# alphafox02/iridium-sniffer

Hardware: AMD Instinct MI355X
Metric: IQ Msamples/s end-to-end (detect->demod), 10 MHz cf32 (higher is better)
Workload: dtype f32

## Files before the change

### iridium-sniffer_amd/csrc/api.cpp

```cpp
#include <stdarg.h>
#include "pipeline.hpp"

namespace irdmh {

extern "C" int irdm_set_option(irdm_pipeline_t *p, const char *key, int value)
{
    if (!p || !key) return -1;
    if (!strcmp(key, "keep_frame_samples")) { p->keep_frame_samples = value; return 0; }
    if (!strcmp(key, "packed_records")) { p->packed_records = value; return 0; }
    if (!strcmp(key, "parsed_records")) { p->parsed_records = value; return 0; }
    if (!strcmp(key, "frame_records")) { p->frame_records = value; return 0; }
    if (!strcmp(key, "chunk_marks")) { p->chunk_marks = value ? 1 : 0; if (!value) p->q_marks.clear(); return 0; }
    if (!strcmp(key, "decode_frames")) { p->decode_frames = value; return 0; }
    if (!strcmp(key, "decode_ida")) { p->decode_ida = value; return 0; }
    if (!strcmp(key, "detect_only")) { p->detect_only = value; return 0; }
    if (!strcmp(key, "fir_order") || !strcmp(key, "simd_order")) { p->fir_order = value ? 1 : 0; return 0; }
    if (!strcmp(key, "host_cfo")) { p->dev_cfo = p->dev_cfo_ok && value == 0; return 0; }
    if (!strcmp(key, "scan_mode")) { p->scan_mode = value; return 0; }
    if (!strcmp(key, "kernel_clock")) { p->kernel_clock = value != 0; return 0; }
    if (!strcmp(key, "rot_prebuild")) {
        if (value) return p->rot_pre_runs ? 0 : rot_prebuild(p);
        return p->rot_pre_runs ? rot_arena_reset(p, (long long)std::min(p->P.n, 1024) * p->rot_runs) : 0;
    }
    if (!strcmp(key, "band_timeline")) { p->band_tune.timeline = value != 0; return 0; }
    if (!strcmp(key, "fir_generic")) { p->fir_generic = value != 0; return 0; }
    if (!strcmp(key, "post_generic")) { p->post_generic = value != 0; return 0; }
    if (!strcmp(key, "k1_lists")) { p->k1_lists = value; return 0; }
    if (!strcmp(key, "band_first")) { p->band_first = value < 0 ? 0 : value > kBandRounds ? kBandRounds : value; return 0; }
    if (!strcmp(key, "band_spec")) { p->band_spec_opt = value != 0; return 0; }
    if (!strcmp(key, "band_selfcheck")) { p->band_tune.selfcheck = value; return 0; }
    if (!strcmp(key, "rot_pool_rows")) {
        if (value < 1 || value > p->P.n) return -1;
        return rot_arena_reset(p, (long long)value * p->rot_runs);
    }
    if (!strcmp(key, "scratch_outputs")) {
        if (value < 16) return -1;
        for (int i = 0; i < p->n_bc; i++)
            if (p->bc[i].n != 0) return -1;
        IRDM_HIP_CHECK(hipDeviceSynchronize());
        for (int i = 0; i < p->n_bc; i++) {
            BatchCtx &b = p->bc[i];
            float2 *d2 = dev_alloc<float2>((size_t)value), *l2 = dev_alloc<float2>(lpf_alloc((size_t)value));
            if (!d2 || !l2) return -1;
            (void)hipFree(b.d_dec);
            (void)hipFree(b.d_lpf);
            b.d_dec = d2;
            b.d_lpf = l2;
            b.dec_cap = (size_t)value;
            if (!b.owns_buffers) { p->d_dec = d2; p->d_lpf = l2; }
        }
        return 0;
    }
    return -1;
}

extern "C" int64_t irdm_get_stat(const irdm_pipeline_t *p, const char *key)
{
    if (!p || !key) return -1;
    if (!strcmp(key, "scan_fast_chunks")) return (int64_t)p->stat_fast_chunks;
    if (!strcmp(key, "scan_fallbacks")) return (int64_t)p->stat_fallbacks;
    if (!strncmp(key, "host_us_", 8) && key[8] >= '0' && key[8] <= '9') return (int64_t)p->host_us[key[8] - '0'];
    if (!strcmp(key, "band_chunks")) return (int64_t)p->stat_band_chunks;
    if (!strcmp(key, "band_extra")) return (int64_t)p->stat_band_extra;
    if (!strcmp(key, "scan_chained")) return (int64_t)p->stat_chained;
    if (!strcmp(key, "scan_chain_undone")) return (int64_t)p->stat_chain_undone;
    if (!strcmp(key, "k1_lists")) return (int64_t)p->stat_k1_lists;
    if (!strcmp(key, "band_rounds")) return (int64_t)p->stat_band_rounds;
    if (!strcmp(key, "band_retries")) return (int64_t)p->stat_band_retries;
    if (!strcmp(key, "band_aborts")) return (int64_t)p->stat_band_aborts;
    if (!strncmp(key, "tl_dur_", 7)) { const int i = atoi(key + 7); return i >= 0 && i < 32 ? (int64_t)p->stat_tl_dur[i] : -1; }
    if (!strncmp(key, "tl_gap_", 7)) { const int i = atoi(key + 7); return i >= 0 && i < 32 ? (int64_t)p->stat_tl_gap[i] : -1; }
    if (!strncmp(key, "tl_n_", 5)) { const int i = atoi(key + 5); return i >= 0 && i < 32 ? (int64_t)p->stat_tl_n[i] : -1; }
    if (!strncmp(key, "plan_tp_", 8)) {
        const int i = atoi(key + 8);
        return i >= 0 && i < 16 ? (int64_t)p->stat_plan_tp[i] : -1;
    }
    if (!strcmp(key, "rot_rows")) return (int64_t)p->rot_rows_used;
    if (!strcmp(key, "rot_prebuilt_runs")) return (int64_t)p->rot_pre_runs;
    if (!strcmp(key, "rot_rows_cap")) return (int64_t)(p->rot_blocks_cap / p->rot_runs);
    if (!strcmp(key, "rot_blocks")) return (int64_t)p->rot_blocks_used;
    if (!strcmp(key, "rot_blocks_cap")) return (int64_t)p->rot_blocks_cap;
    if (!strcmp(key, "rot_grows")) return (int64_t)p->stat_rot_grows;
    if (!strcmp(key, "rot_builds")) return (int64_t)p->stat_rot_builds;
    if (!strcmp(key, "rot_runs")) return (int64_t)p->stat_rot_rows;
    if (!strcmp(key, "rot_ckpts")) return (int64_t)p->stat_rot_ckpts;
    if (!strcmp(key, "band_steps")) return (int64_t)p->stat_band_steps;
    if (!strcmp(key, "scratch_outputs")) return (int64_t)p->bc[0].dec_cap;
    if (!strcmp(key, "scratch_grows")) return (int64_t)p->stat_scratch_grows;
    if (!strcmp(key, "tiles_grows")) return (int64_t)p->stat_tiles_grows;
    if (!strcmp(key, "ring_waits")) return (int64_t)p->stat_ring_waits;
    if (!strcmp(key, "spec_passes")) return (int64_t)p->stat_spec_passes;
    if (!strcmp(key, "spec_scans")) return (int64_t)p->stat_spec_scans;
    if (!strcmp(key, "sum_restarts")) return (int64_t)p->stat_sum_restarts;
    if (!strcmp(key, "scratch_peak")) return (int64_t)p->stat_scratch_peak;
    if (!strcmp(key, "band_last_flags")) return (int64_t)p->last_band_flags;
    if (!strcmp(key, "scan_dense_frames")) return (int64_t)p->stat_dense_frames;
    return -1;
}

extern "C" int irdm_kernel_clock(irdm_pipeline_t *p, int which, double *sum_ms, uint64_t *launches, double *last_ms, int reset)
{
    if (!p || !p->d_kclk || which < 0 || which > 1) return -1;
    pipeline_enter(p);
    if (hipDeviceSynchronize() != hipSuccess) return -1;
    std::vector<unsigned long long> h((size_t)(6 + kMaxBc - 3) * kKClkWords);
    if (hipMemcpy(h.data(), p->d_kclk, sizeof(unsigned long long) * h.size(), hipMemcpyDeviceToHost) != hipSuccess) return -1;
    unsigned long long ticks = 0, n = 0, last = 0;
    std::vector<int> recs;
    if (which == 1) recs = { 3, 4, 5 };
    else
        for (int c = 0; c < kMaxBc; c++) recs.push_back(c < 3 ? c : 3 + c);
    for (int r : recs) {
        ticks += h[(size_t)r * kKClkWords + 128];
        n += h[(size_t)r * kKClkWords + 129];
        if (h[(size_t)r * kKClkWords + 130] > last) last = h[(size_t)r * kKClkWords + 130];
    }
    if (sum_ms) *sum_ms = (double)ticks * 1e-5;
    if (launches) *launches = n;
    if (last_ms) *last_ms = (double)last * 1e-5;
    if (reset) {
        for (int r : recs) {
            unsigned long long z[3] = { 0, 0, 0 };
            if (hipMemcpy(p->d_kclk + (size_t)r * kKClkWords + 128, z, sizeof(z), hipMemcpyHostToDevice) != hipSuccess) return -1;
        }
    }
    return 0;
}

extern "C" int irdm_last_timings(const irdm_pipeline_t *p, float *ms_out, int n)
{
    if (!p || !ms_out) return -1;
    for (int i = 0; i < n && i < 6; i++) ms_out[i] = p->last_ms[i];
    return n < 6 ? n : 6;
}

extern "C" int irdm_format_raw(const irdm_demod_t *f, const char *file_info, uint64_t *t0_io, char *buf,
                               size_t cap)
{
    if (!f || !t0_io || !buf) return -1;
    char auto_info[64];
    if (*t0_io == 0) *t0_io = (f->timestamp / 1000000000ULL) * 1000000000ULL;
    const uint64_t t0 = *t0_io;
    if (!file_info || !file_info[0]) {
        snprintf(auto_info, sizeof(auto_info), "i-%llu-t1", (unsigned long long)(t0 / 1000000000ULL));
        file_info = auto_info;
    }
    const double ts_ms = (double)(f->timestamp - t0) / 1000000.0;
    const int freq_hz = (int)(f->center_frequency + 0.5);
    const int payload = f->n_payload_symbols < 0 ? 0 : f->n_payload_symbols;
    int pos = snprintf(buf, cap, "RAW: %s %012.4f %010d N:%05.2f%+06.2f I:%011llu %3d%% %.5f %3d ", file_info,
                       ts_ms, freq_hz, f->magnitude, f->noise, (unsigned long long)f->id, f->confidence,
                       f->level, payload);
    if (pos < 0 || (size_t)pos + (size_t)f->n_bits + 2 > cap) return -1;
    for (int i = 0; i < f->n_bits; i++) buf[pos++] = (char)('0' + f->bits[i]);
    buf[pos++] = '\n';
    buf[pos] = 0;
    return pos;
}

extern "C" int irdm_format_raw_packed(const irdm_demod_packed_t *f, const char *file_info, uint64_t *t0_io, char *buf,
                                      size_t cap)
{
    if (!f || !t0_io || !buf) return -1;
    char auto_info[64];
    if (*t0_io == 0) *t0_io = (f->timestamp / 1000000000ULL) * 1000000000ULL;
    const uint64_t t0 = *t0_io;
    if (!file_info || !file_info[0]) {
        snprintf(auto_info, sizeof(auto_info), "i-%llu-t1", (unsigned long long)(t0 / 1000000000ULL));
        file_info = auto_info;
    }
    const double ts_ms = (double)(f->timestamp - t0) / 1000000.0;
    const int freq_hz = (int)(f->center_frequency + 0.5);
    const int payload = f->n_payload_symbols < 0 ? 0 : f->n_payload_symbols;
    int pos = snprintf(buf, cap, "RAW: %s %012.4f %010d N:%05.2f%+06.2f I:%011llu %3d%% %.5f %3d ", file_info,
                       ts_ms, freq_hz, f->magnitude, f->noise, (unsigned long long)f->id, f->confidence,
                       f->level, payload);
    const int nb = f->n_bits < 0 ? 0 : (f->n_bits > IRDM_MAX_BITS ? IRDM_MAX_BITS : f->n_bits);
    if (pos < 0 || (size_t)pos + (size_t)nb + 2 > cap) return -1;
    for (int i = 0; i < nb; i++) buf[pos++] = (char)('0' + ((f->bits[i >> 3] >> (7 - (i & 7))) & 1));
    buf[pos++] = '\n';
    buf[pos] = 0;
    return pos;
}

extern "C" long long irdm_format_raw_packed_batch(const irdm_demod_packed_t *f, int n, const char *file_info, uint64_t *t0_io,
                                                  char *buf, size_t cap)
{
    if (!f || n < 0 || !t0_io || !buf) return -1;
    size_t pos = 0;
    for (int i = 0; i < n; i++) {
        const int len = irdm_format_raw_packed(&f[i], file_info, t0_io, buf + pos, cap - pos);
        if (len < 0) return -1;
        pos += (size_t)len;
    }
    return (long long)pos;
}

extern "C" void irdm_ida_unpack(const irdm_ida_packed_t *ida, const irdm_demod_packed_t *f, irdm_ida_t *out)
{
    if (!ida || !f || !out) return;
    IdaOut d;
    memset(&d, 0, sizeof(d));
    d.ok = ida->ok;
    d.ft = ida->ft; d.lcw_ft = ida->lcw_ft; d.lcw_code = ida->lcw_code; d.ec_lcw = ida->ec_lcw;
    d.lcw3_val = ida->lcw3_val;
    d.da_ctr = ida->da_ctr; d.da_len = ida->da_len; d.cont = ida->cont; d.crc_ok = ida->crc_ok;
    d.stored_crc = ida->stored_crc; d.computed_crc = ida->computed_crc;
    d.fixederrs = ida->fixederrs; d.payload_len = ida->payload_len; d.bch_len = ida->bch_len;
    memcpy(d.payload, ida->payload, sizeof(d.payload));
    for (int i = 0; i < 256; i++) d.bch_stream[i] = (uint8_t)((ida->bch_stream[i >> 3] >> (7 - (i & 7))) & 1);
    irdm_demod_t fr;
    memset(&fr, 0, offsetof(irdm_demod_t, bits));
    fr.id = f->id;
    fr.direction = f->direction;
    fr.timestamp = f->timestamp;
    fr.center_frequency = f->center_frequency;
    fr.magnitude = f->magnitude;
    fr.noise = f->noise;
    fr.level = f->level;
    fr.confidence = f->confidence;
    fr.n_payload_symbols = f->n_payload_symbols;
    *out = finish_ida(d, fr);
}

extern "C" void irdm_frame_unpack(const irdm_frame_packed_t *fr, const irdm_demod_packed_t *f, irdm_decoded_t *out)
{
    if (!fr || !f || !out) return;
    DecodedOut d;
    memset(&d, 0, sizeof(d));
    d.type = fr->type;
    d.sat_id = fr->sat_id;
    d.beam_id = fr->beam_id;
    for (int k = 0; k < 3; k++) d.pos_xyz[k] = fr->pos_xyz[k];
    d.n_pages = fr->n_pages;
    for (int k = 0; k < 12; k++) { d.page_tmsi[k] = fr->page_tmsi[k]; d.page_msc[k] = fr->page_msc[k]; }
    d.timeslot = fr->timeslot;
    d.sv_blocking = fr->sv_blocking;
    d.bc_type = fr->bc_type;
    d.iri_time = fr->iri_time;
    d.bch_len = fr->bch_len;
    *out = finish_decoded(d, f->id, f->timestamp, f->center_frequency);
}

namespace {

struct LineBuf {
    char *buf;
    size_t cap, pos = 0;
    bool bad = false;
    void printf(const char *fmt, ...) __attribute__((format(printf, 2, 3)))
    {
        if (bad) return;
        va_list ap;
        va_start(ap, fmt);
        const int n = vsnprintf(buf + pos, cap - pos, fmt, ap);
        va_end(ap);
        if (n < 0 || (size_t)n >= cap - pos) bad = true;
        else pos += (size_t)n;
    }
    void put(char c)
    {
        if (bad || pos + 1 >= cap) { bad = true; return; }
        buf[pos++] = c;
        buf[pos] = 0;
    }
};

}

extern "C" int irdm_format_ida(const irdm_ida_t *b, uint64_t *t0_io, char *buf, size_t cap)
{
    if (!b || !t0_io || !buf || cap == 0) return -1;
    if (*t0_io == 0) *t0_io = (b->timestamp / 1000000000ULL) * 1000000000ULL;
    const uint64_t t0 = *t0_io;
    LineBuf o{ buf, cap };
    buf[0] = 0;
    char parsed_info[64];
    snprintf(parsed_info, sizeof(parsed_info), "p-%llu", (unsigned long long)(t0 / 1000000000ULL));
    const double ts_ms = (double)(b->timestamp - t0) / 1000000.0;
    const int freq_hz = (int)(b->frequency + 0.5);
    const double leveldb = (b->level > 0) ? 20.0 * log10(b->level) : -99.99;
    const double noise = b->noise, snr = b->magnitude;
    const char *dir = b->direction == 2 ? "UL" : "DL";
    const int syms = b->n_symbols < 0 ? 0 : b->n_symbols;
    o.printf("IDA: %s %014.4f %010d %3d%% %06.2f|%07.2f|%05.2f %3d %s ", parsed_info, ts_ms, freq_hz, b->confidence,
             leveldb, noise, snr, syms, dir);
    o.printf("%.*s", (int)sizeof(b->lcw_header), b->lcw_header);
    const uint8_t *bs = b->bch_stream;
    const int bch_len = b->bch_len;
    if (bch_len >= 20) {
        o.printf("%c%c%c", '0' + bs[0], '0' + bs[1], '0' + bs[2]);
        o.printf(" cont=%c", '0' + bs[3]);
        o.printf(" %c", '0' + bs[4]);
        o.printf(" ctr=%c%c%c", '0' + bs[5], '0' + bs[6], '0' + bs[7]);
        o.printf(" %c%c%c", '0' + bs[8], '0' + bs[9], '0' + bs[10]);
        o.printf(" len=%02d", b->da_len);
        o.printf(" 0:%c%c%c%c", '0' + bs[16], '0' + bs[17], '0' + bs[18], '0' + bs[19]);
        o.printf(" [");
        bool all_zero = true;
        if (b->da_len > 0)
            for (int i = b->da_len + 1; i < 20; i++)
                if (b->payload[i] != 0) { all_zero = false; break; }
        const int nbytes = b->da_len > 0 && all_zero ? b->da_len : 20;
        for (int i = 0; i < nbytes; i++) {
            if (i > 0) o.put(nbytes == 20 && i == b->da_len && b->da_len > 0 && b->da_len < 20 ? '!' : '.');
            o.printf("%02x", b->payload[i]);
        }
        o.printf("]");
        for (int i = nbytes * 3; i < 60; i++) o.put(' ');
        if (b->da_len > 0) {
            o.printf(" %04x/%04x", b->stored_crc, b->computed_crc);
            o.printf(b->crc_ok ? " CRC:OK" : " CRC:no");
        } else {
            o.printf("  ---   ");
        }
        const int shown = bch_len < 256 ? bch_len : 256;
        if (bch_len > 9 * 20 + 16) {
            o.put(' ');
            for (int i = 9 * 20 + 16; i < shown; i++) o.put((char)('0' + bs[i]));
        } else {
            o.printf(" 0000");
        }
        if (b->da_len > 0 && bch_len >= 9 * 20) {
            o.printf(" SBD: ");
            for (int i = 0; i < 20; i++) {
                int byte = 0;
                for (int k = 0; k < 8; k++) byte = (byte << 1) | bs[1 * 20 + i * 8 + k];
                o.put(byte >= 32 && byte < 127 ? (char)byte : '.');
            }
        }
    }
    o.put('\n');
    return o.bad ? -1 : (int)o.pos;
}

extern "C" long long irdm_format_parsed_packed_batch(const irdm_demod_packed_t *f, const irdm_ida_packed_t *idas, int n,
                                                     const char *file_info, uint64_t *t0_io, char *buf, size_t cap)
{
    if (!f || !idas || n < 0 || !t0_io || !buf) return -1;
    size_t pos = 0;
    for (int i = 0; i < n; i++) {
        int len;
        if (idas[i].ok) {
            irdm_ida_t b;
            irdm_ida_unpack(&idas[i], &f[i], &b);
            len = irdm_format_ida(&b, t0_io, buf + pos, cap - pos);
        } else {
            len = irdm_format_raw_packed(&f[i], file_info, t0_io, buf + pos, cap - pos);
        }
        if (len < 0) return -1;
        pos += (size_t)len;
    }
    return (long long)pos;
}

extern "C" int irdm_save_burst(const irdm_frame_info_t *info, const float *samples, const char *dir)
{
    if (!info || !samples || !dir || info->drop_reason != 0 || info->num_samples <= 0) return -1;
    struct stat st;
    memset(&st, 0, sizeof(st));
    if (stat(dir, &st) == -1) {
        if (mkdir(dir, 0755) == -1 && errno != EEXIST) {
            fprintf(stderr, "Warning: failed to create burst save directory: %s\n", strerror(errno));
            return -1;
        }
    }
    const char *dir_str = info->demod_direction == 1 ? "DL" : info->demod_direction == 2 ? "UL" : "UN";
    char base[512];
    snprintf(base, sizeof(base), "%s/%020lu_%011.0f_%lu_%s", dir, (unsigned long)info->timestamp,
             info->center_frequency, (unsigned long)info->id, dir_str);
    char path[520];
    snprintf(path, sizeof(path), "%s.cf32", base);
    FILE *f = fopen(path, "wb");
    if (!f) {
        fprintf(stderr, "Warning: failed to save burst IQ: %s\n", strerror(errno));
        return -1;
    }
    fwrite(samples, 2 * sizeof(float), (size_t)info->num_samples, f);
    fclose(f);
    snprintf(path, sizeof(path), "%s.meta", base);
    f = fopen(path, "w");
    if (!f) return -1;
    fprintf(f, "burst_id: %lu\n", (unsigned long)info->id);
    fprintf(f, "timestamp_ns: %lu\n", (unsigned long)info->timestamp);
    fprintf(f, "center_freq_hz: %.0f\n", info->center_frequency);
    fprintf(f, "sample_rate_hz: %.0f\n", info->sample_rate);
    fprintf(f, "samples_per_symbol: %.2f\n", info->samples_per_symbol);
    fprintf(f, "direction: %s\n", dir_str);
    fprintf(f, "magnitude_db: %.2f\n", info->magnitude);
    fprintf(f, "noise_dbfs_hz: %.2f\n", info->noise);
    fprintf(f, "num_samples: %zu\n", (size_t)info->num_samples);
    fprintf(f, "uw_start_offset: %.2f\n", info->uw_start);
    fclose(f);
    return 0;
}

extern "C" long long irdm_format_raw_batch(const irdm_demod_t *f, int n, const char *file_info, uint64_t *t0_io,
                                           char *buf, size_t cap)
{
    if (!f || n < 0 || !t0_io || !buf) return -1;
    size_t pos = 0;
    for (int i = 0; i < n; i++) {
        const int len = irdm_format_raw(&f[i], file_info, t0_io, buf + pos, cap - pos);
        if (len < 0) return -1;
        pos += (size_t)len;
    }
    return (long long)pos;
}

extern "C" const char *irdm_version(void) { return "irdm_hip 0.1 (gfx950)"; }

}
```

### iridium-sniffer_amd/csrc/band_core.hpp

```cpp
#pragma once
#include <stdint.h>
#include "types.hpp"

#if defined(__HIPCC__)
#define IRDM_HD __host__ __device__ __forceinline__
#else
#define IRDM_HD inline
#endif

namespace irdm {

constexpr int kBandSlots = 24;
constexpr int kBandRecCap = 1024;
constexpr int kBandMaxTotal = 8192;

enum : uint32_t {
    BAND_F_SLOTS = 1,
    BAND_F_RECS = 2,
    BAND_F_LIST = 4,
    BAND_F_STALE = 8,
    BAND_F_SQUELCH = 16,
    BAND_F_AGREE = 32,
    BAND_F_ITER = 64,
    BAND_F_TOTAL = 128,
    BAND_F_GONECAP = 256,
    BAND_F_SNAP = 512,
    BAND_F_CHAIN = 2048,
    BAND_F_CHECK = 4096,
    BAND_F_COOP = 1024,
};

struct BandParams {
    int32_t n, nw64;
    int32_t log_n;
    int32_t n_frames, occ_words;
    int32_t hw;
    int32_t pre_len, post_len, max_len, max_bursts;
    int32_t band_w, n_bands;
    int32_t gap;
    int32_t list_cap;
    float thr;
    uint64_t idx0;
    int32_t serial = 0;
    int32_t selfcheck = 0;
    int32_t tl_sel = -1;
    int32_t chained = 0;
    int32_t sum_restart = 1;
    int32_t spec_in = 0;
};

struct BandRec {
    int64_t start, last_active, stop;
    int32_t cf;
    int32_t cb;
    float rel, base;
    int32_t flags;
    int32_t seq;
};

IRDM_HD uint32_t band_float_bits(float v)
{
    uint32_t u;
    __builtin_memcpy(&u, &v, 4);
    return u;
}

IRDM_HD bool band_rec_same(const BandRec &a, const BandRec &b)
{
    return a.start == b.start && a.last_active == b.last_active && a.stop == b.stop && a.cf == b.cf &&
           a.cb == b.cb && a.seq == b.seq && (a.flags & 2) == (b.flags & 2) &&
           band_float_bits(a.rel) == band_float_bits(b.rel) && band_float_bits(a.base) == band_float_bits(b.base);
}

struct BandIO {
    const uint64_t *cross;
    const uint64_t *occ;
    const float *relq;
    const float *snap;
    const int32_t *slot_post;
    const ActiveBurst *act_in;
    int32_t n_act_in;
    BandRec *recs;
    uint32_t *rec_count;
    uint64_t *busy, *forced;
    uint32_t *conc;
    uint32_t *flags;
};

struct BandSlots {
    int64_t *start, *la;
    int32_t *cb, *cf, *seq;
    float *rel, *base;
    int stride;
};

#if defined(__HIP_DEVICE_COMPILE__)
IRDM_HD void band_or64(uint64_t *p, uint64_t v) { atomicOr(reinterpret_cast<unsigned long long *>(p), (unsigned long long)v); }
IRDM_HD void band_or32(uint32_t *p, uint32_t v) { atomicOr(p, v); }
IRDM_HD uint32_t band_add32(uint32_t *p, uint32_t v) { return atomicAdd(p, v); }
#else
IRDM_HD void band_or64(uint64_t *p, uint64_t v) { *p |= v; }
IRDM_HD void band_or32(uint32_t *p, uint32_t v) { *p |= v; }
IRDM_HD uint32_t band_add32(uint32_t *p, uint32_t v) { uint32_t o = *p; *p = o + v; return o; }
#endif

template <int NW>
IRDM_HD void bm_set_range(uint64_t (&m)[NW], int a, int b)
{
#pragma unroll
    for (int k = 0; k < NW; k++) {
        int lo = a - 64 * k, hi = b - 64 * k;
        if (lo < 0) lo = 0;
        if (hi > 63) hi = 63;
        if (lo <= hi) m[k] |= (~0ull >> (63 - hi)) & (~0ull << lo);
    }
}

template <int NW>
IRDM_HD int bm_test(const uint64_t (&m)[NW], int r)
{
    uint64_t w = 0;
#pragma unroll
    for (int k = 0; k < NW; k++)
        if (k == (r >> 6)) w = m[k];
    return (int)((w >> (r & 63)) & 1);
}

template <int NW>
IRDM_HD bool bm_any(const uint64_t (&m)[NW])
{
    uint64_t w = 0;
#pragma unroll
    for (int k = 0; k < NW; k++) w |= m[k];
    return w != 0;
}

IRDM_HD int band_next_occ(const uint64_t *occ, int a, int b, int n_frames)
{
    if (a < 0) a = 0;
    if (b >= n_frames) b = n_frames - 1;
    while (a <= b) {
        const int w = a >> 6;
        uint64_t v = occ[w] & (~0ull << (a & 63));
        if (v) {
            const int f = 64 * w + __builtin_ctzll(v);
            return f <= b ? f : 0x7fffffff;
        }
        a = 64 * (w + 1);
    }
    return 0x7fffffff;
}

IRDM_HD uint64_t band_segment_starts(const uint64_t *occ, int blk, int gap, bool carried)
{
    const uint64_t cur = occ[blk], prev = blk > 0 ? occ[blk - 1] : 0;
    uint64_t smear = 0;
    for (int d = 1; d <= gap; d++) smear |= (cur << d) | (prev >> (64 - d));
    if (blk == 0 && carried) smear |= gap >= 64 ? ~0ull : ((1ull << gap) - 1);
    return cur & ~smear;
}

template <int NW>
struct BandWalker {
    const BandParams &P;
    const BandIO &io;
    BandSlots S;
    int band, e0, word0;
    int own_lo, own_hi, rep_lo, rep_hi;
    uint64_t M[NW], elig[NW];
    uint32_t valid;
    int last_occ;
    int acc_blk;
    uint32_t acc_max;
    int n_events = 0;

    IRDM_HD BandWalker(const BandParams &p, const BandIO &i, BandSlots s, int b) : P(p), io(i), S(s), band(b)
    {
        const int H = P.band_w / 2;
        e0 = band * P.band_w - H;
        word0 = e0 >> 6;
        own_lo = H;
        own_hi = H + P.band_w;
        rep_lo = own_lo - P.hw;
        rep_hi = own_hi + P.hw;
#pragma unroll
        for (int k = 0; k < NW; k++) M[k] = elig[k] = 0;
        uint64_t dc[NW];
#pragma unroll
        for (int k = 0; k < NW; k++) dc[k] = 0;
        bm_set_range<NW>(elig, P.hw - e0, P.n - P.hw - 1 - e0);
        bm_set_range<NW>(dc, P.n / 2 - 3 - e0, P.n / 2 + 3 - e0);
#pragma unroll
        for (int k = 0; k < NW; k++) elig[k] &= ~dc[k];
        valid = 0;
        last_occ = -1;
        acc_blk = -1;
        acc_max = 0;
    }

    IRDM_HD void rebuild_mask()
    {
#pragma unroll
        for (int k = 0; k < NW; k++) M[k] = 0;
        for (uint32_t v = valid; v; v &= v - 1) {
            const int i = __builtin_ctz(v);
            const int r = S.cb[i * S.stride] - e0;
            bm_set_range<NW>(M, r - P.hw, r + P.hw);
        }
    }

    IRDM_HD void emit(int i, int64_t stop, int lng)
    {
        const int r = S.cb[i * S.stride] - e0;
        if (r < rep_lo || r >= rep_hi) return;
        const uint32_t at = band_add32(&io.rec_count[band], 1);
        if (at >= (uint32_t)kBandRecCap) {
            band_or32(io.flags, BAND_F_RECS);
            return;
        }
        BandRec g;
        g.start = S.start[i * S.stride];
        g.last_active = S.la[i * S.stride];
        g.stop = stop;
        g.cf = S.cf[i * S.stride];
        g.cb = S.cb[i * S.stride];
        g.rel = S.rel[i * S.stride];
        g.base = S.base[i * S.stride];
        g.flags = ((r >= own_lo && r < own_hi) ? 1 : 0) | (lng ? 2 : 0);
        g.seq = S.seq[i * S.stride];
        io.recs[(size_t)band * kBandRecCap + at] = g;
    }

    IRDM_HD uint32_t owned_count() const
    {
        uint32_t c = 0;
        for (uint32_t v = valid; v; v &= v - 1) {
            const int r = S.cb[__builtin_ctz(v) * S.stride] - e0;
            c += (r >= own_lo && r < own_hi) ? 1 : 0;
        }
        return c;
    }

    IRDM_HD void account(int a, int b, uint32_t c)
    {
        if (c == 0 || a > b) return;
        for (int blk = a >> 6; blk <= (b >> 6); blk++) {
            const int lo = blk == (a >> 6) ? (a & 63) : 0, hi = blk == (b >> 6) ? (b & 63) : 63;
            band_or64(&io.busy[blk], (~0ull >> (63 - hi)) & (~0ull << lo));
            if (blk != acc_blk) {
                flush_conc();
                acc_blk = blk;
                acc_max = c;
            } else if (c > acc_max) {
                acc_max = c;
            }
        }
    }

    IRDM_HD void flush_conc()
    {
        if (acc_blk >= 0 && acc_max > 0) band_add32(&io.conc[acc_blk], acc_max);
        acc_blk = -1;
        acc_max = 0;
    }

    IRDM_HD int load_carried()
    {
        int n = 0;
        for (int i = 0; i < io.n_act_in; i++) {
            const int r = io.act_in[i].center_bin - e0;
            if (r < 0 || r >= 64 * NW) continue;
            if (n >= kBandSlots) {
                band_or32(io.flags, BAND_F_SLOTS);
                break;
            }
            S.start[n * S.stride] = (int64_t)io.act_in[i].start;
            S.la[n * S.stride] = (int64_t)io.act_in[i].last_active;
            S.cb[n * S.stride] = io.act_in[i].center_bin;
            S.cf[n * S.stride] = -1;
            S.seq[n * S.stride] = i;
            S.rel[n * S.stride] = io.act_in[i].peak_rel;
            S.base[n * S.stride] = io.act_in[i].base_sum;
            valid |= 1u << n;
            n++;
        }
        rebuild_mask();
        return n;
    }

    IRDM_HD int min_expiry() const
    {
        int64_t best = 0x7fffffff;
        for (uint32_t v = valid; v; v &= v - 1) {
            const int i = __builtin_ctz(v);
            const int64_t num = S.la[i * S.stride] + (int64_t)P.post_len - (int64_t)P.idx0;
            const int64_t ef = num <= 0 ? 0 : (num + P.n - 1) >> P.log_n;
            if (ef < best) best = ef;
        }
        return (int)best;
    }

    IRDM_HD int next_event(int f)
    {
        const uint64_t *occ = io.occ + (size_t)band * P.occ_words;
        if (valid == 0) return band_next_occ(occ, f + 1, last_occ + P.gap, P.n_frames);
        const int ef = min_expiry();
        const int nf = band_next_occ(occ, f + 1, ef, P.n_frames);
        return nf < ef ? nf : ef;
    }

    IRDM_HD void process(int f)
    {
        const int64_t index = (int64_t)P.idx0 + (int64_t)f * P.n;
        const uint64_t *occ = io.occ + (size_t)band * P.occ_words;
        const bool occupied = (occ[f >> 6] >> (f & 63)) & 1;
        uint64_t cw[NW];
#pragma unroll
        for (int k = 0; k < NW; k++) {
            const int w = word0 + k;
            cw[k] = (occupied && w >= 0 && w < P.nw64) ? io.cross[(size_t)f * P.nw64 + w] : 0;
        }
        if (occupied) last_occ = f;

        if (valid && bm_any<NW>(cw)) {
            uint64_t hit[NW];
#pragma unroll
            for (int k = 0; k < NW; k++) {
                hit[k] = cw[k] | (cw[k] << 1) | (cw[k] >> 1);
                if (k > 0) hit[k] |= cw[k - 1] >> 63;
                if (k < NW - 1) hit[k] |= cw[k + 1] << 63;
            }
            for (uint32_t v = valid; v; v &= v - 1) {
                const int i = __builtin_ctz(v);
                if (bm_test<NW>(hit, S.cb[i * S.stride] - e0)) S.la[i * S.stride] = index;
            }
        }
        uint64_t pk[NW];
#pragma unroll
        for (int k = 0; k < NW; k++) pk[k] = cw[k] & ~M[k] & elig[k];

        bool deleted = false;
        for (uint32_t v = valid; v; v &= v - 1) {
            const int i = __builtin_ctz(v);
            const int64_t la = S.la[i * S.stride];
            const bool lng = P.max_len > 0 && (la - S.start[i * S.stride] > (int64_t)P.max_len);
            if (la + (int64_t)P.post_len <= index || lng) {
                const int r = S.cb[i * S.stride] - e0;
                if (lng && r >= own_lo && r < own_hi) band_or64(&io.forced[f >> 6], 1ull << (f & 63));
                emit(i, index, lng ? 1 : 0);
                valid &= ~(1u << i);
                deleted = true;
            }
        }
        if (deleted) rebuild_mask();

        while (bm_any<NW>(pk)) {
            float best = -1.0f;
            int best_r = -1;
#pragma unroll
            for (int k = 0; k < NW; k++) {
                uint64_t w = pk[k];
                const float *row = io.relq + (size_t)f * P.n + (e0 + 64 * k);
                while (w) {
                    const int j0 = __builtin_ctzll(w);
                    w &= w - 1;
                    const int j1 = w ? __builtin_ctzll(w) : j0;
                    w &= w ? w - 1 : 0;
                    const int j2 = w ? __builtin_ctzll(w) : j1;
                    w &= w ? w - 1 : 0;
                    const int j3 = w ? __builtin_ctzll(w) : j2;
                    w &= w ? w - 1 : 0;
                    const float v0 = row[j0], v1 = row[j1], v2 = row[j2], v3 = row[j3];
                    if (v0 > best) { best = v0; best_r = 64 * k + j0; }
                    if (v1 > best) { best = v1; best_r = 64 * k + j1; }
                    if (v2 > best) { best = v2; best_r = 64 * k + j2; }
                    if (v3 > best) { best = v3; best_r = 64 * k + j3; }
                }
            }
            if (best_r < 0) break;
            int slot = __builtin_ctz(~valid);
            if (slot >= kBandSlots) {
                band_or32(io.flags, BAND_F_SLOTS);
                break;
            }
            const int cbin = e0 + best_r;
            S.start[slot * S.stride] = index - (int64_t)P.pre_len;
            S.la[slot * S.stride] = index - (int64_t)P.pre_len;
            S.cb[slot * S.stride] = cbin;
            S.cf[slot * S.stride] = f;
            S.seq[slot * S.stride] = 0;
            S.rel[slot * S.stride] = best;
            S.base[slot * S.stride] = io.snap[(size_t)io.slot_post[f] * P.n + cbin];
            valid |= 1u << slot;
            bm_set_range<NW>(M, best_r - P.hw, best_r + P.hw);
#pragma unroll
            for (int k = 0; k < NW; k++) pk[k] &= ~M[k];
        }
    }

    IRDM_HD void run(int f_start, bool carried)
    {
        int f;
        if (carried) {
            last_occ = -1;
            const uint32_t c0 = owned_count();
            f = next_event(-1);
            account(0, (f < P.n_frames ? f : P.n_frames) - 1, c0);
        } else {
            f = f_start;
        }
        while (f < P.n_frames) {
            process(f);
            n_events++;
            const uint32_t c = owned_count();
            const int nf = next_event(f);
            account(f, (nf < P.n_frames ? nf : P.n_frames) - 1, c);
            if (valid == 0 && nf == 0x7fffffff) break;
            f = nf;
        }
        flush_conc();
        for (uint32_t v = valid; v; v &= v - 1) emit(__builtin_ctz(v), -1, 0);
    }
};

}
```

### iridium-sniffer_amd/csrc/create.cpp

```cpp
#include "pipeline.hpp"

namespace irdmh {

void pipeline_free(irdm_pipeline *p)
{
    if (!p) return;
    void *ptrs[] = { p->d_window, p->d_hist, p->d_sum, p->d_mag, p->d_tw, p->d_tw4096, p->d_tw2048,
                     p->d_dl_fft, p->d_ul_fft, p->d_rot_incr, p->d_state, p->d_gone,
                     p->d_cand_a, p->d_cand_b, p->d_ring, p->d_stage, p->d_in_taps, p->d_noise_taps,
                     p->d_start_taps, p->d_rrc_taps, p->d_cfo_window, p->d_work, p->d_tiles, p->d_dec,
                     p->d_lpf, p->d_rrc_ws, p->d_frames, p->d_demod_ws, p->d_probe, p->d_demod, p->d_decoded, p->d_syn_ra,
                     p->d_syn_hdr, p->d_nbits, p->d_ida, p->d_syn_da, p->d_syn_l1, p->d_syn_l2, p->d_syn_l3, p->d_dirs,
                     p->d_fir_off, p->d_mag2, p->d_mag3, p->k1_pre[1], p->k1_pre[2], p->k1_counts[1], p->k1_counts[2], p->k1_entries[1], p->k1_entries[2],
                     p->k1_pre[0] != p->d_pre ? p->k1_pre[0] : nullptr, p->k1_counts[0] != p->d_counts ? p->k1_counts[0] : nullptr,
                     p->k1_entries[0] != p->d_entries ? p->k1_entries[0] : nullptr, p->d_counts, p->d_entries, p->d_goff, p->d_compact, p->d_pre, p->d_sum_bak, p->d_hist_bak, p->d_state_bak,
                     p->d_status, p->d_mc_ops, p->d_mc_done, p->d_band, p->d_smin, p->d_kclk, p->d_state_spec };
    for (void *q : ptrs)
        if (q) (void)hipFree(q);
    for (int s = 0; s < 2; s++) {
        if (p->h_pin_set[s]) (void)hipHostFree(p->h_pin_set[s]);
        if (p->hp_gone_set[s]) (void)hipHostFree(p->hp_gone_set[s]);
        if (p->ev_end_set[s]) (void)hipEventDestroy(p->ev_end_set[s]);
        for (auto &e : p->ev_sk_set[s])
            if (e) (void)hipEventDestroy(e);
    }
    if (p->cfo_thread.joinable()) {
        {
            std::lock_guard<std::mutex> lk(p->cfo_mu);
            p->cfo_quit = true;
        }
        p->cfo_cv.notify_one();
        p->cfo_thread.join();
    }
    for (int i = 0; i < kMaxBc; i++) {
        BatchCtx &b = p->bc[i];
        if (b.ev_cfo) (void)hipEventDestroy(b.ev_cfo);
        if (b.ev_rot) (void)hipEventDestroy(b.ev_rot);
        for (auto &e : b.ev)
            if (e) (void)hipEventDestroy(e);
        if (b.hp_flag) (void)hipHostFree(b.hp_flag);
        if (b.hp_rot_new) (void)hipHostFree(b.hp_rot_new);
        if (b.d_rot_new) (void)hipFree(b.d_rot_new);
        if (b.hp_work) (void)hipHostFree(b.hp_work);
        if (b.hp_tiles) (void)hipHostFree(b.hp_tiles);
        if (b.hp_demod) (void)hipHostFree(b.hp_demod);
        if (b.hp_packed) (void)hipHostFree(b.hp_packed);
        if (b.hp_ida) (void)hipHostFree(b.hp_ida);
        if (b.hp_frame) (void)hipHostFree(b.hp_frame);
        if (b.owns_buffers) {
            void *own[] = { b.d_work, b.d_tiles, b.d_dec, b.d_lpf, b.d_rrc_ws, b.d_frames, b.d_demod_ws, b.d_demod,
                            b.d_decoded, b.d_ida };
            for (void *q : own)
                if (q) (void)hipFree(q);
            if (b.stream) (void)hipStreamDestroy(b.stream);
        }
    }
    if (p->ev_ring) (void)hipEventDestroy(p->ev_ring);
    for (auto &f : p->fs) {
        if (f.ev_start) (void)hipEventDestroy(f.ev_start);
        if (f.ev_k1) (void)hipEventDestroy(f.ev_k1);
        if (f.ev_copy) (void)hipEventDestroy(f.ev_copy);
    }
    if (p->hp_gate) (void)hipHostFree(p->hp_gate);
    if (p->d_rot_table) (void)hipFree(p->d_rot_table);
    for (float2 *q : p->rot_retired) (void)hipFree(q);
    for (float2 *q : p->scratch_retired) (void)hipFree(q);
    for (void *q : p->tiles_retired) (void)hipFree(q);
    for (void *q : p->tiles_host_retired) (void)hipHostFree(q);
    if (p->d_rot_slot) (void)hipFree(p->d_rot_slot);
    if (p->stream_rot_pre) { (void)hipStreamSynchronize(p->stream_rot_pre); (void)hipStreamDestroy(p->stream_rot_pre); }
    if (p->ev_rot_pre) (void)hipEventDestroy(p->ev_rot_pre);
    if (p->d_rot_pre_news) (void)hipFree(p->d_rot_pre_news);
    if (p->stream_spec) (void)hipStreamDestroy(p->stream_spec);
    if (p->ev_sums1) (void)hipEventDestroy(p->ev_sums1);
    if (p->ev_spec_done) (void)hipEventDestroy(p->ev_spec_done);
    if (p->d_band_spec) (void)hipFree(p->d_band_spec);
    for (auto &e : p->ev)
        if (e) (void)hipEventDestroy(e);
    if (p->sstream && p->sstream != p->stream) (void)hipStreamDestroy(p->sstream);
    if (p->ev_scan_in) (void)hipEventDestroy(p->ev_scan_in);
    if (p->ev_scan_out) (void)hipEventDestroy(p->ev_scan_out);
    if (p->fstream && p->fstream != p->stream) (void)hipStreamDestroy(p->fstream);
    if (p->stream2) (void)hipStreamDestroy(p->stream2);
    if (p->stream) (void)hipStreamDestroy(p->stream);
    delete p;
}

extern "C" void irdm_destroy(irdm_pipeline_t *p) { pipeline_free(p); }


bool chain_stream_create(irdm_pipeline *, hipStream_t *out, int prio)
{
    return hipStreamCreateWithPriority(out, hipStreamNonBlocking, prio) == hipSuccess;
}

extern "C" irdm_pipeline_t *irdm_create(const irdm_config_t *cfg)
{
    if (!cfg || cfg->sample_rate <= 0) return nullptr;
    int ndev = 0;
    if (hipGetDeviceCount(&ndev) != hipSuccess || ndev == 0) {
        fprintf(stderr, "irdm_hip: no HIP device -- there is no CPU fallback in this library\n");
        return nullptr;
    }
    if (hipSetDevice(cfg->device) != hipSuccess) return nullptr;
    const bool dbg = getenv("IRDM_CREATE_DEBUG") != nullptr;
    size_t mem_free0 = 0, mem_total = 0;
    if (dbg) (void)hipMemGetInfo(&mem_free0, &mem_total);
    auto t_now = [] {
        struct timespec ts;
        clock_gettime(CLOCK_MONOTONIC, &ts);
        return ts.tv_sec * 1e3 + ts.tv_nsec * 1e-6;
    };
    const double t_create0 = t_now();
    auto mark = [&](const char *what) {
        if (!dbg) return;
        size_t fr = 0, tot = 0;
        (void)hipMemGetInfo(&fr, &tot);
        fprintf(stderr, "irdm_create: %-28s %8.2f ms  %8.1f MB on the device\n", what, t_now() - t_create0,
                ((double)mem_free0 - (double)fr) / 1e6);
    };

    irdm_pipeline *p = new (std::nothrow) irdm_pipeline();
    if (!p) return nullptr;
    p->cfg = *cfg;
    const int fs = cfg->sample_rate;

    DetParams &P = p->P;
    P.log_n = (int)round(log2(fs / 1000.0));
    P.n = 1 << P.log_n;
    P.pre_len = 2 * P.n;
    P.post_len = (int)(fs * 16e-3);
    const int burst_width_hz = 40000;
    P.width = burst_width_hz / (fs / P.n);
    P.max_bursts = (int)((fs / (float)burst_width_hz) * 0.8f);
    P.max_len = (int)(fs * 0.09);
    const float tdb = cfg->threshold_db > 0 ? cfg->threshold_db : 16.0f;
    P.threshold = powf(10.0f, tdb / 10.0f) / kHistory / 1.72f;
    if (P.n < kScanThreads || P.n > 16384 || P.max_bursts + P.n / (P.width > 0 ? P.width : 1) + 8 > kMaxActive) {
        fprintf(stderr, "irdm_hip: unsupported sample rate %d (fft_size %d)\n", fs, P.n);
        delete p;
        return nullptr;
    }
    p->feed_block = cfg->feed_block > 0 ? cfg->feed_block : 32768;
    if (p->feed_block % P.n != 0) {
        fprintf(stderr, "irdm_hip: feed_block %d must be a multiple of fft_size %d\n", p->feed_block, P.n);
        delete p;
        return nullptr;
    }
    p->dev_fmt = cfg->format;
    p->bps = p->dev_fmt == 2 ? 8 : (p->dev_fmt == 1 ? 4 : 2);
    p->max_chunk = cfg->max_chunk_samples ? cfg->max_chunk_samples : ((size_t)64 << 20);
    p->max_chunk = (p->max_chunk + p->feed_block - 1) / p->feed_block * p->feed_block;
    p->burst_cap = cfg->max_bursts_per_chunk > 0 ? cfg->max_bursts_per_chunk : 4096;
    p->gone_cap = p->burst_cap;
    p->start_time_ns = cfg->start_time_ns;
    if (p->start_time_ns == 0) {
        struct timespec ts;
        clock_gettime(CLOCK_REALTIME, &ts);
        p->start_time_ns = ts.tv_sec * 1000000000ULL + ts.tv_nsec;
    }

    p->ref_ring = (uint64_t)P.max_len + P.pre_len + P.post_len + (uint64_t)P.n * 4;
    if (p->ref_ring < (uint64_t)2 * fs) p->ref_ring = (uint64_t)2 * fs;
    p->l_cap = (size_t)P.max_len + P.post_len + P.pre_len + 2 * (size_t)P.n;
    p->depth = cfg->pipeline_depth > 0 ? std::min(cfg->pipeline_depth, kMaxBc - 1) : 0;
    p->k1_first = 1;
    p->k1_lists = 1;
    p->band_first = 0;
    p->band_auto = kBandFirst;
    p->ring_len = p->ref_ring + p->l_cap + p->feed_block;
    if (p->depth) p->ring_len += (size_t)(p->depth + 2 + kLookAhead) * p->max_chunk;
    p->ring_len = (p->ring_len + 15) / 16 * 16;
    if (p->depth) p->ring_len = (p->ring_len + p->max_chunk - 1) / p->max_chunk * p->max_chunk;
    p->n_ckpt = (int)(p->l_cap / kRotSeg) + 2;

    p->out_rate = 10 * 25000;
    p->sps = (float)p->out_rate / 25000;
    p->search_depth = p->out_rate;
    p->pre_start = (int)(100 * 1e-6f * p->out_rate);
    p->decim = (int)roundf((float)fs / p->out_rate);
    if (p->decim < 1) p->decim = 1;
    p->dec_stride = (int)(p->l_cap / p->decim) + 8;

    std::vector<float> in_taps = design_lpf(1.0f, 10000000.0f, p->out_rate * 0.4f, p->out_rate * 0.2f);
    std::vector<float> noise_taps = design_lpf(1.0f, (float)p->out_rate, 40000.0f / 2.0f, 40000.0f);
    int box = (int)(p->sps * 2);
    if (box < 3) box = 3;
    std::vector<float> start_taps = design_box(box);
    std::vector<float> rrc = design_rrc(1.0f, (float)p->out_rate, 25000.0f, 0.4f, 51);
    std::vector<float> rc = design_rc((float)p->out_rate, 25000.0f, 0.4f, 51);
    std::vector<float> cfo_window = design_blackman(kCfoN);
    if ((int)in_taps.size() != kFirTaps) {
        delete p;
        return nullptr;
    }
    p->in_ntaps = (int)in_taps.size();
    p->noise_ntaps = (int)noise_taps.size();
    p->start_ntaps = (int)start_taps.size();
    p->rrc_ntaps = (int)rrc.size();
    std::vector<cfloat> dl = design_sync_template(rc, kCorrN, p->sps, false, &p->dl_len);
    std::vector<cfloat> ul = design_sync_template(rc, kCorrN, p->sps, true, &p->ul_len);

    std::vector<float> window = design_blackman(P.n);
    for (int i = 0; i < P.n; i++) window[i] /= 0.42f;
    std::vector<cfloat> tw = design_twiddles(P.n), tw4096 = design_twiddles(kCfoTotal),
                        tw2048 = design_twiddles(kCorrN);
    std::vector<cfloat> rot_incr = design_rotator_incr(P.n);

    mark("host designs");
    int prio_lo = 0, prio_hi = 0;
    (void)hipDeviceGetStreamPriorityRange(&prio_lo, &prio_hi);
    bool ok = true;
    p->stream2 = nullptr;
    if (p->depth) {
        int prio_k1 = prio_hi < prio_lo - 1 ? prio_hi + 1 : prio_hi;
        if (const char *e = getenv("IRDM_K1_PRIO")) prio_k1 = atoi(e);
        ok = hipStreamCreateWithPriority(&p->stream, hipStreamNonBlocking, prio_hi) == hipSuccess &&
             hipStreamCreateWithPriority(&p->fstream, hipStreamNonBlocking, prio_k1) == hipSuccess &&
             chain_stream_create(p, &p->stream2, prio_lo);
        p->bstream = p->stream2;
    } else {
        ok = hipStreamCreateWithFlags(&p->stream, hipStreamNonBlocking) == hipSuccess;
        p->bstream = p->stream;
        p->fstream = p->stream;
    }
    p->sstream = p->stream;
    p->bstream_prio = prio_lo;
    p->ev_scan_in = p->ev_scan_out = nullptr;
    p->has_pending = false;
    p->pend_c1 = 0;
    p->h_pin = nullptr;
    for (int s = 0; s < 2; s++) {
        p->h_pin_set[s] = nullptr;
        p->hp_gone_set[s] = nullptr;
        p->ev_end_set[s] = nullptr;
        for (auto &e : p->ev_sk_set[s]) ok = ok && hipEventCreate(&e) == hipSuccess;
        ok = ok && hipEventCreateWithFlags(&p->ev_end_set[s], hipEventDisableTiming) == hipSuccess;
        ok = ok && hipHostMalloc(reinterpret_cast<void **>(&p->h_pin_set[s]), sizeof(int) * 128, hipHostMallocDefault) == hipSuccess;
        if (ok) memset(p->h_pin_set[s], 0, sizeof(int) * 128);
    }
    p->out_sel = 0;
    p->chain_pending = false;
    p->settle_clean = true;
    p->h_pin = p->h_pin_set[0];
    p->ev_sk[0] = p->ev_sk_set[0][0];
    p->ev_sk[1] = p->ev_sk_set[0][1];
    p->ev_end = p->ev_end_set[0];
    for (auto &e : p->ev) ok = ok && hipEventCreate(&e) == hipSuccess;
#define UP(dst, vec) ok = ok && ((dst = reinterpret_cast<decltype(dst)>(dev_upload((vec).data(), (vec).size()))) != nullptr)
#define AL(dst, T, count) ok = ok && ((dst = dev_alloc<T>(count)) != nullptr)
    UP(p->d_window, window);
    UP(p->d_tw, tw);
    UP(p->d_tw4096, tw4096);
    UP(p->d_tw2048, tw2048);
    UP(p->d_dl_fft, dl);
    UP(p->d_ul_fft, ul);
    UP(p->d_rot_incr, rot_incr);
    UP(p->d_in_taps, in_taps);
    UP(p->d_noise_taps, noise_taps);
    UP(p->d_start_taps, start_taps);
    UP(p->d_rrc_taps, rrc);
    UP(p->d_cfo_window, cfo_window);
    {
        const int row = fir_tile_row(p->decim);
        std::vector<int> off(kFirTaps);
        for (int k = 0; k < kFirTaps; k++) off[k] = ((k % p->decim) * row + k / p->decim) * (int)sizeof(float2);
        UP(p->d_fir_off, off);
    }
    mark("streams, uploads");
    AL(p->d_hist, float, (size_t)kHistory * P.n);
    AL(p->d_sum, float, (size_t)P.n);
    AL(p->d_mag, float, p->max_chunk);
    if (p->depth) AL(p->d_mag2, float, p->max_chunk);
    if (p->depth) AL(p->d_mag3, float, p->max_chunk);
    AL(p->d_state, DetState, 1);
    AL(p->d_gone, GoneBurst, (size_t)p->gone_cap);
    AL(p->d_cand_a, PeakCand, (size_t)P.n);
    AL(p->d_cand_b, PeakCand, (size_t)P.n);
    mark("detector buffers");
    p->d_rot_table = nullptr;
    AL(p->d_work, BurstWork, (size_t)p->burst_cap);
    p->tiles_cap = (size_t)p->burst_cap * 64;
    AL(p->d_tiles, FirTile, (p->tiles_cap + 1) * kFirTileUnits);
    p->cfo_quit = false;
    p->scratch_init = std::max<size_t>((size_t)p->burst_cap * p->dec_stride / 16, (size_t)4 * p->dec_stride);
    AL(p->d_dec, float2, p->scratch_init);
    AL(p->d_lpf, float2, lpf_alloc(p->scratch_init));
    AL(p->d_rrc_ws, float2, (size_t)p->burst_cap * kFrameNeed);
    AL(p->d_frames, float2, (size_t)p->burst_cap * kMaxFrameSamples);
    AL(p->d_demod_ws, float2, (size_t)p->burst_cap * 2 * kMaxSymbols);
    AL(p->d_demod, DemodOut, (size_t)p->burst_cap);
    AL(p->d_decoded, DecodedOut, (size_t)p->burst_cap);
    AL(p->d_nbits, int, (size_t)p->burst_cap);
    {
        auto rem = [](unsigned poly, unsigned v) {
            if (!v) return 0u;
            const int pb = 32 - __builtin_clz(poly);
            for (int i = 31; i >= pb - 1; i--)
                if (v & (1u << i)) v ^= poly << (i - pb + 1);
            return v;
        };
        auto build = [&](unsigned poly, int nbits, int max_err, int size) {
            std::vector<int2> t((size_t)size, make_int2(-1, 0));
            for (int b1 = 0; b1 < nbits; b1++) {
                const unsigned v = 1u << b1, r = rem(poly, v);
                if (r < (unsigned)size) t[r] = make_int2(1, (int)v);
            }
            if (max_err >= 2)
                for (int b1 = 0; b1 < nbits; b1++)
                    for (int b2 = b1 + 1; b2 < nbits; b2++) {
                        const unsigned v = (1u << b1) | (1u << b2), r = rem(poly, v);
                        if (r < (unsigned)size && t[r].x < 0) t[r] = make_int2(2, (int)v);
                    }
            return t;
        };
        std::vector<int2> ra = build(1207u, 31, 2, 1024), hdr = build(29u, 7, 1, 16);
        UP(p->d_syn_ra, ra);
        UP(p->d_syn_hdr, hdr);
        std::vector<int2> da = build(3545u, 31, 2, 2048), l1 = build(29u, 7, 1, 16), l2 = build(465u, 14, 1, 256),
                          l3 = build(41u, 26, 2, 32);
        UP(p->d_syn_da, da);
        UP(p->d_syn_l1, l1);
        UP(p->d_syn_l2, l2);
        UP(p->d_syn_l3, l3);
        AL(p->d_ida, IdaOut, (size_t)p->burst_cap);
        AL(p->d_dirs, int, (size_t)p->burst_cap);
    }
    AL(p->d_probe, float2, p->l_cap);
    {
        const size_t max_frames = p->max_chunk / P.n;
        AL(p->d_counts, unsigned, max_frames);
        AL(p->d_entries, ListEntry, max_frames * (size_t)std::max(kListCap, band_list_cap(P.n)));
        AL(p->d_goff, unsigned, max_frames + 1);
        AL(p->d_compact, ListEntry, max_frames * kListCap);
        AL(p->d_pre, float, (size_t)P.n);
        p->k1_pre[0] = p->d_pre;
        p->k1_counts[0] = p->d_counts;
        p->k1_entries[0] = p->d_entries;
        for (int i = 0; i < kFeedSlots && p->depth; i++) {
            AL(p->k1_pre[i], float, (size_t)P.n);
            AL(p->k1_counts[i], unsigned, max_frames);
            AL(p->k1_entries[i], ListEntry, max_frames * (size_t)std::max(kListCap, band_list_cap(P.n)));
        }
        AL(p->d_sum_bak, float, (size_t)P.n);
        AL(p->d_hist_bak, float, (size_t)kHistory * P.n);
        AL(p->d_state_bak, DetState, 1);
        AL(p->d_status, int, 64);
        p->mc_ops_cap = (int)(4 * max_frames + 64);
        AL(p->d_mc_ops, unsigned long long, (size_t)p->mc_ops_cap);
        AL(p->d_mc_done, unsigned, 32 * 16);
    }
    mark("per-burst scratch, lists");
    ok = ok && hipHostMalloc(reinterpret_cast<void **>(&p->hp_gate), 64, hipHostMallocMapped | hipHostMallocCoherent) == hipSuccess &&
         hipHostGetDevicePointer(reinterpret_cast<void **>(&p->hp_gate_dev), p->hp_gate, 0) == hipSuccess;
    if (ok) memset(p->hp_gate, 0, 64);
    AL(p->d_kclk, unsigned long long, (size_t)(6 + kMaxBc - 3) * kKClkWords);
    if (ok) {
        std::vector<unsigned long long> init((size_t)(6 + kMaxBc - 3) * kKClkWords, 0ull);
        for (int r = 0; r < 6 + kMaxBc - 3; r++)
            for (int i = 0; i < 64; i++) init[(size_t)r * kKClkWords + i] = ~0ull;
        ok = hipMemcpy(p->d_kclk, init.data(), sizeof(unsigned long long) * init.size(), hipMemcpyHostToDevice) == hipSuccess;
    }
    p->band_ok = band_scan_supported(P, nullptr, 1, 0) != 0;
    if (p->band_ok) {
        AL(p->d_smin, float, (size_t)P.n);
        if (ok) ok = hipMalloc(&p->d_band, band_work_bytes(P.n, p->max_chunk)) == hipSuccess;
        if (ok) band_work_carve(&p->band, p->d_band, P.n, p->max_chunk);
        if (ok) ok = hipMemset(p->band.bar, 0, 256) == hipSuccess;
        if (ok && p->depth) {
            const size_t sb = band_work_bytes(P.n, p->max_chunk, true);
            ok = hipMalloc(&p->d_band_spec, sb) == hipSuccess;
            if (ok) band_work_carve(&p->band_spec, p->d_band_spec, P.n, p->max_chunk, true);
            if (ok) ok = hipMemset(p->band_spec.ctl, 0, sizeof(BandCtl)) == hipSuccess && hipMemset(p->band_spec.bar, 0, 256) == hipSuccess &&
                         hipMemset(p->band_spec.rec_count, 0, 4 * 64) == hipSuccess && hipMemset(p->band_spec.flags, 0, 256) == hipSuccess;
            AL(p->d_state_spec, DetState, 1);
            if (ok) ok = hipMemset(p->d_state_spec, 0, sizeof(DetState)) == hipSuccess;
            ok = ok && hipStreamCreateWithPriority(&p->stream_spec, hipStreamNonBlocking, prio_hi) == hipSuccess &&
                 hipEventCreateWithFlags(&p->ev_sums1, hipEventDisableTiming) == hipSuccess &&
                 hipEventCreateWithFlags(&p->ev_spec_done, hipEventDisableTiming) == hipSuccess;
        }
    }
    mark("band scan workspace");
    if (ok) ok = hipMalloc(&p->d_ring, p->ring_len * p->bps) == hipSuccess;
    mark("history ring");
    p->n_bc = p->depth ? std::min(p->depth + 1, kMaxBc) : 1;
    for (int i = 0; i < p->n_bc && ok; i++) {
        BatchCtx &b = p->bc[i];
        b.owner = p;
        b.n = 0;
        b.cfo_seq = 0;
        b.owns_buffers = i > 0;
        b.tiles_cap = p->tiles_cap;
        b.dec_cap = p->scratch_init;
        if (i == 0) {
            b.stream = p->bstream;
            b.d_work = p->d_work; b.d_tiles = p->d_tiles; b.d_dec = p->d_dec; b.d_lpf = p->d_lpf;
            b.d_rrc_ws = p->d_rrc_ws; b.d_frames = p->d_frames; b.d_demod_ws = p->d_demod_ws; b.d_demod = p->d_demod;
            b.d_decoded = p->d_decoded; b.d_ida = p->d_ida;
        } else {
            ok = ok && chain_stream_create(p, &b.stream, p->bstream_prio);
            AL(b.d_work, BurstWork, (size_t)p->burst_cap);
            AL(b.d_tiles, FirTile, (b.tiles_cap + 1) * kFirTileUnits);
            AL(b.d_dec, float2, p->scratch_init);
            AL(b.d_lpf, float2, lpf_alloc(p->scratch_init));
            AL(b.d_rrc_ws, float2, (size_t)p->burst_cap * kFrameNeed);
            AL(b.d_frames, float2, (size_t)p->burst_cap * kMaxFrameSamples);
            AL(b.d_demod_ws, float2, (size_t)p->burst_cap * 2 * kMaxSymbols);
            AL(b.d_demod, DemodOut, (size_t)p->burst_cap);
            AL(b.d_decoded, DecodedOut, (size_t)p->burst_cap);
            AL(b.d_ida, IdaOut, (size_t)p->burst_cap);
        }
        ok = ok && hipHostMalloc(reinterpret_cast<void **>(&b.hp_work), sizeof(BurstWork) * (size_t)p->burst_cap,
                                 hipHostMallocMapped | hipHostMallocCoherent) == hipSuccess &&
             hipHostGetDevicePointer(reinterpret_cast<void **>(&b.hp_work_dev), b.hp_work, 0) == hipSuccess;
        ok = ok && hipHostMalloc(reinterpret_cast<void **>(&b.hp_tiles), sizeof(FirTile) * b.tiles_cap, hipHostMallocDefault) == hipSuccess;
        ok = ok && hipHostMalloc(reinterpret_cast<void **>(&b.hp_demod), sizeof(DemodOut) * (size_t)p->burst_cap, hipHostMallocDefault) == hipSuccess;
        ok = ok && hipHostMalloc(reinterpret_cast<void **>(&b.hp_packed), sizeof(DemodPacked) * (size_t)p->burst_cap, hipHostMallocDefault) == hipSuccess;
        ok = ok && hipHostMalloc(reinterpret_cast<void **>(&b.hp_ida), sizeof(IdaPacked) * (size_t)p->burst_cap, hipHostMallocDefault) == hipSuccess;
        ok = ok && hipHostMalloc(reinterpret_cast<void **>(&b.hp_frame), sizeof(FramePacked) * (size_t)p->burst_cap, hipHostMallocDefault) == hipSuccess;
        ok = ok && hipHostMalloc(reinterpret_cast<void **>(&b.hp_flag), 64, hipHostMallocMapped | hipHostMallocCoherent) == hipSuccess &&
             hipHostGetDevicePointer(reinterpret_cast<void **>(&b.hp_flag_dev), b.hp_flag, 0) == hipSuccess;
        if (ok) memset(b.hp_flag, 0, 64);
        ok = ok && hipHostMalloc(reinterpret_cast<void **>(&b.hp_rot_new), sizeof(int4) * (size_t)p->burst_cap, hipHostMallocMapped) == hipSuccess &&
             hipHostGetDevicePointer(reinterpret_cast<void **>(&b.hp_rot_new_dev), b.hp_rot_new, 0) == hipSuccess;
        AL(b.d_rot_new, int4, (size_t)p->burst_cap);
        ok = ok && hipEventCreateWithFlags(&b.ev_cfo, hipEventDisableTiming) == hipSuccess;
        ok = ok && hipEventCreateWithFlags(&b.ev_rot, hipEventDisableTiming) == hipSuccess;
        for (auto &e : b.ev) ok = ok && hipEventCreate(&e) == hipSuccess;
        b.h_cfreq.assign((size_t)p->burst_cap, 0.0);
    }
    p->hp_gone_cap = p->gone_cap;
    for (int s = 0; s < 2; s++)
        ok = ok && hipHostMalloc(reinterpret_cast<void **>(&p->hp_gone_set[s]), sizeof(GoneBurst) * (size_t)p->hp_gone_cap, hipHostMallocDefault) == hipSuccess;
    p->hp_gone = p->hp_gone_set[0];
    ok = ok && hipEventCreateWithFlags(&p->ev_ring, hipEventDisableTiming) == hipSuccess;
    for (auto &f : p->fs)
        ok = ok && hipEventCreate(&f.ev_start) == hipSuccess && hipEventCreate(&f.ev_k1) == hipSuccess &&
             hipEventCreateWithFlags(&f.ev_copy, hipEventDisableTiming) == hipSuccess;
    p->chunk_no = 0;
#undef UP
#undef AL
    if (!ok) {
        fprintf(stderr, "irdm_hip: device allocation failed\n");
        pipeline_free(p);
        return nullptr;
    }
    mark("batch contexts");
    ok = hipMemset(p->d_hist, 0, sizeof(float) * (size_t)kHistory * P.n) == hipSuccess &&
         hipMemset(p->d_sum, 0, sizeof(float) * P.n) == hipSuccess &&
         hipMemset(p->d_state, 0, sizeof(DetState)) == hipSuccess &&
         hipMemset(p->d_ring, 0, p->ring_len * p->bps) == hipSuccess;
    ok = ok && hipDeviceSynchronize() == hipSuccess;
    mark("memsets, sync");
    p->rot_runs = (p->n_ckpt + kRotRun - 1) / kRotRun;
    p->rot_blocks_cap = std::min(P.n, 1024) * p->rot_runs;
    p->rot_blocks_used = 0;
    p->rot_rows_used = 0;
    p->rot_len_h.assign((size_t)P.n, 0);
    p->rot_want.assign((size_t)P.n, 0);
    ok = ok && (p->d_rot_table = dev_alloc<float2>((size_t)p->rot_blocks_cap * kRotRun)) != nullptr;
    ok = ok && (p->d_rot_slot = dev_alloc<int>((size_t)P.n * p->rot_runs)) != nullptr;
    ok = ok && hipMemset(p->d_rot_slot, 0xff, sizeof(int) * (size_t)P.n * p->rot_runs) == hipSuccess;
    p->rot_build_ctx.assign((size_t)P.n, -1);
    p->rot_build_gen.assign((size_t)P.n, 0);
#ifndef IRDM_HIP_EMULATED
    if (ok && p->depth >= 1 && !getenv("IRDM_NO_ROT_PREBUILD")) (void)rot_prebuild(p);
#endif
    mark("rotator row pool");
    if (!ok) {
        fprintf(stderr, "irdm_hip: device initialisation failed\n");
        pipeline_free(p);
        return nullptr;
    }
    p->h_gone.resize(p->gone_cap);
    p->total_samples = p->begun_samples = 0;
    p->begin_no = p->end_no = 0;
    p->tagged = 0;
    p->stream_closed = false;
    p->last_frames = 0;
    p->last_chunk = nullptr;
    p->keep_frame_samples = 0;
    p->chunk_marks = 0;
    p->scan_mode = 0;
    p->mc_updaters = 7;
    {
        hipDeviceProp_t prop;
        const bool have = hipGetDeviceProperties(&prop, cfg->device) == hipSuccess;
        p->mc_auto = have && prop.multiProcessorCount >= 64;
        if (p->scan_cus == 0) p->scan_cus = have ? prop.multiProcessorCount : 1;
    }
    p->stat_fast_chunks = p->stat_fallbacks = p->stat_dense_frames = 0;
    p->stat_band_chunks = p->stat_band_rounds = p->stat_band_retries = p->stat_band_aborts = 0;
    p->last_band_flags = 0;
    p->fl_mode = 0;
    p->fl_done = 0;
    p->host_primed = 0;
    p->host_hist_idx = 0;
    p->dev_cfo = true;
    {
        auto same = [](float off) {
            const cfloat h = fine_rotator_incr(off);
            const float phase_inc = -2.0f * (float)M_PI * off;
            float re, im;
            if (libm_cexpf_i<true>(phase_inc, &re, &im) != 0) return false;
            const float hr = h.real(), hi = h.imag();
            return memcmp(&re, &hr, 4) == 0 && memcmp(&im, &hi, 4) == 0;
        };
        bool all = true;
        for (int i = 0; i < (1 << 18) && all; i++) all = same(-0.26f + 0.52f * (float)i / (float)(1 << 18));
        const float edges[] = { 0.0f, -0.0f, 1e-45f, -1e-45f, 1e-39f, 3e-5f, -3e-5f, 0.125f, -0.125f, 0.25f, -0.25f, 0.2499999f, 0.1250001f };
        for (float e : edges) all = all && same(e);
        if (!all) {
            fprintf(stderr, "irdm_hip: this host's cexpf differs from the restated glibc routine: the fine-CFO step stays on the host\n");
            p->dev_cfo = false;
        }
    }
    p->dev_cfo_ok = p->dev_cfo;
    mark("libm self-check");
    p->cfo_thread = std::thread(cfo_helper_main, p);
    mark("done");
    return p;
}

extern "C" int irdm_sincosf_probe(int device, const float *x, size_t n, float *re, float *im)
{
    if (!x || !re || !im) return -1;
    if (!n) return 0;
    IRDM_HIP_CHECK(hipSetDevice(device));
    float *d = nullptr;
    IRDM_HIP_CHECK(hipMalloc(&d, 3 * n * sizeof(float)));
    int rc = hipMemcpy(d, x, n * sizeof(float), hipMemcpyHostToDevice) == hipSuccess ? 0 : -1;
    if (!rc) rc = launch_sincosf_probe(d, n, d + n, d + 2 * n, nullptr);
    if (!rc) rc = hipMemcpy(re, d + n, n * sizeof(float), hipMemcpyDeviceToHost) == hipSuccess ? 0 : -1;
    if (!rc) rc = hipMemcpy(im, d + 2 * n, n * sizeof(float), hipMemcpyDeviceToHost) == hipSuccess ? 0 : -1;
    (void)hipFree(d);
    return rc;
}

extern "C" uint64_t irdm_tagged_bursts(const irdm_pipeline_t *p) { return p ? p->tagged : 0; }
extern "C" size_t irdm_max_chunk_samples(const irdm_pipeline_t *p) { return p ? p->max_chunk : 0; }
extern "C" size_t irdm_bytes_per_sample(const irdm_pipeline_t *p) { return p ? p->bps : 0; }
extern "C" size_t irdm_required_overlap(const irdm_pipeline_t *p)
{
    if (!p) return 0;
    return (size_t)(p->ref_ring + (uint64_t)p->P.max_len + (uint64_t)p->P.post_len + (uint64_t)p->P.pre_len + 2 * (uint64_t)p->P.n);
}
extern "C" int irdm_wait_ingest(irdm_pipeline_t *p)
{
    if (!p) return -1;
    pipeline_enter(p);
    IRDM_HIP_CHECK(hipStreamSynchronize(p->fstream));
    return 0;
}
extern "C" uint64_t irdm_sample_count(const irdm_pipeline_t *p) { return p ? p->total_samples : 0; }
extern "C" int irdm_fft_size(const irdm_pipeline_t *p) { return p ? p->P.n : -1; }
extern "C" uint64_t irdm_start_time_ns(const irdm_pipeline_t *p) { return p ? p->start_time_ns : 0; }

extern "C" int irdm_set_stream_origin(irdm_pipeline_t *p, double center_frequency, uint64_t start_time_ns)
{
    if (!p || p->begin_no != p->end_no) return -1;
    p->cfg.center_frequency = center_frequency;
    if (start_time_ns) p->start_time_ns = start_time_ns;
    return 0;
}

}
```

### iridium-sniffer_amd/csrc/kernels.hpp

```cpp
#pragma once
#include <hip/hip_runtime.h>
#include "types.hpp"

namespace irdm {

int launch_fft_mag_lists(int log_n, int fmt, const void *iq, const float *window, const float2 *tw, float *mag,
                         int n_frames, const float *pre, unsigned *counts, ListEntry *entries, int cap,
                         hipStream_t stream, unsigned long long *kclk, int order);
int launch_prefilter_threshold(const float *sum, float thr, float *pre, int n, hipStream_t stream);
int launch_fft_mag(int log_n, int fmt, const void *iq, const float *window, const float2 *tw,
                   float *mag, int n_frames, hipStream_t stream, unsigned long long *kclk, int order);
int launch_detect_scan(const DetParams &P, DetState *st, float *sum, float *hist, const float *mag,
                       int n_frames, GoneBurst *gone, int gone_cap, PeakCand *cand_a,
                       PeakCand *cand_b, hipStream_t stream);

int launch_prefilter(const float *sum, float thr, float *pre, const float *mag, int n,
                     unsigned *counts, ListEntry *entries, unsigned *goff, ListEntry *compact,
                     int n_frames, hipStream_t stream);
int launch_detect_scan_fast(const DetParams &P, DetState *st, float *sum, float *hist, const float *mag,
                            int n_frames, const unsigned *counts, const unsigned *goff,
                            const ListEntry *compact, const float *pre, GoneBurst *gone, int gone_cap,
                            int *status, unsigned long long *mc_ops, int mc_ops_cap, unsigned *mc_done,
                            int mc_updaters, hipStream_t stream);

constexpr int kBandRounds = 5;
constexpr int kBandFirst = 3;
struct BandRec;
struct BandParams;
struct BandCtl {
    int32_t status;
    int32_t rounds;
    uint32_t flags;
    int32_t n_upd, n_snap, agree_fail, mismatch, first_mismatch;
    int32_t n_gone, n_total, committed, h0;
    int32_t k_restart, restart_slot;
    int32_t n_restarts, pad1;
    uint32_t tp[16];
};
struct SumStep {
    uint32_t nw_off;
    uint32_t ol_off;
    uint32_t snap_off;
    uint32_t pad;
};
struct BandWork {
    BandCtl *ctl;
    uint8_t *uq, *uf;
    int32_t *cnt_before, *tmp, *upd_frame, *old_row, *snap_after, *need, *snap_slot, *slot_pre, *slot_post;
    SumStep *steps;
    uint64_t *cross;
    float *relq, *snap;
    int snap_cap;
    uint64_t *occ, *busy, *forced;
    uint32_t *conc;
    BandRec *recs;
    uint32_t *rec_count;
    float *sum_new;
    uint32_t *tot;
    uint64_t *ids;
    uint32_t *flags;
    uint32_t *rank;
    unsigned long long *tl;
    unsigned *bar;
};
struct BandTune {
    int selfcheck = 0;
    int timeline = 0;
    int sum_restart = 1;
};
int band_list_cap(int n);
int band_scan_supported(const DetParams &D, BandParams *out, int n_frames, uint64_t idx0);
size_t band_work_bytes(int n, size_t max_chunk, bool spec = false);
int band_work_carve(BandWork *W, void *base, int n, size_t max_chunk, bool spec = false);
int launch_band_spec(const DetParams &D, BandWork S, DetState *st_spec, const float *sum_src, int n_frames, uint64_t idx0,
                     const unsigned *counts, const ListEntry *entries, int have_prev, hipStream_t stream, const BandTune &tune);
int launch_band_scan(const DetParams &D, BandWork W, DetState *st, float *sum, float *hist, const float *mag,
                     int n_frames, uint64_t idx0, const unsigned *counts, const ListEntry *entries, const float *pre,
                     float *smin, GoneBurst *gone, int gone_cap, int round_begin, int round_end, GoneBurst *hp_gone,
                     uint32_t *hp_hdr, void *hp_ctl, int hp_cap, int chained, int tl_sel, hipStream_t stream,
                     const BandTune &tune, const uint32_t *gate_flag = nullptr, uint32_t gate_seq = 0, uint32_t *gate_err = nullptr,
                     const void *gate_src = nullptr, size_t gate_bytes = 0,
                     const BandWork *spec = nullptr, hipEvent_t sums_done = nullptr);
constexpr int kBandTlSlots = 32;
int launch_prefilter_lists(const float *sum, float thr, float *pre, const float *smin, const float *mag, int n,
                           unsigned *counts, ListEntry *entries, int n_frames, int cap, hipStream_t stream);

struct SampleSource {
    const void *chunk;
    uint64_t chunk_start;
    uint64_t chunk_end;
    const void *ring;
    uint64_t ring_len;
    uint64_t ref_ring;
    int fmt;
};

int launch_rotator_rows(const float2 *incr, float2 *table, int n_runs, const int4 *news, int n_new, int *runs, hipStream_t stream);
int fir_tile_row(int decim);
int fir_reg_supported(int decim);
int fir_fma_tile_out(int decim);
int fir_reg_tile_out(int decim);
int launch_fir_fma(const SampleSource &src, const FirGeom *geom, int n_tiles, int decim, const float *taps,
                   const float2 *rot_table, float2 *dec, hipStream_t stream, unsigned long long *kclk = nullptr);
int launch_fir_reg(const SampleSource &src, const FirGeom *geom, int n_tiles, int decim, const float *taps,
                   const float2 *rot_table, float2 *dec, hipStream_t stream, unsigned long long *kclk = nullptr);
int fir_tile_out(int decim, int aligned, int generic, int order);
int fir_needs_tile_list(int decim, int aligned, int generic);
int launch_fir_decimate(const SampleSource &src, const BurstWork *work, int n_bursts, FirTile *tiles, size_t tiles_cap,
                        int n_tiles, int decim, const float *taps, const int *tap_off, const float2 *rot_incr,
                        const float2 *rot_table, int n_ckpt, float2 *dec,
                        hipStream_t stream, unsigned long long *kclk,
                        const int *rot_slot, int order, int generic);
int launch_kclk_fold(unsigned long long *kclk, hipStream_t stream);
int launch_gone_export(const DetState *st, const GoneBurst *gone, int cap, GoneBurst *hp_gone, uint32_t *hp_hdr,
                       const void *ctl, void *hp_ctl, int ctl_bytes, hipStream_t stream);
int launch_copy_to_host(void *dst, const void *src, size_t bytes, hipStream_t stream);
int launch_copy2_to_host(void *dst_a, const void *src_a, size_t bytes_a, void *dst_b, const void *src_b, size_t bytes_b,
                         hipStream_t stream);
int launch_copy_words(void *dst, const void *src, size_t bytes, hipStream_t stream);
int launch_wait_host_flag(const uint32_t *flag, uint32_t seq, uint32_t *err, hipStream_t stream);
int launch_gather_burst(const SampleSource &src, uint64_t start, uint64_t avail_end, int n,
                        float2 *out, hipStream_t stream);
int launch_downmix_post1(BurstWork *work, int n_bursts, int max_dec_len, float2 *dec,
                         float2 *lpf, float *box, const float *noise_taps, int noise_ntaps,
                         const float *start_taps, int start_ntaps, int search_depth, int pre_start,
                         const float *cfo_window, const float2 *tw4096, BurstWork *hp_work, hipStream_t stream,
                         unsigned long long *kclk,
                         int order, int generic);
struct CfoStep {
    int on_device;
    int n_fft, sample_rate, out_rate;
    double center_frequency;
};
int launch_downmix_post2(BurstWork *work, int n_bursts, const float2 *lpf,
                         const float *rrc_taps, int rrc_ntaps, const float2 *tw2048,
                         const float2 *dl_fft, const float2 *ul_fft, int dl_len, int ul_len,
                         float sps, float2 *rrc_ws, float2 *frames, const BurstWork *hp_work, const CfoStep &cfo,
                         hipStream_t stream, int order, int generic);
int launch_sincosf_probe(const float *x, size_t n, float *re, float *im, hipStream_t stream);

int launch_ida_decode(const DemodOut *frames, int n_frames, const int2 *syn_da, const int2 *syn_l1, const int2 *syn_l2,
                      const int2 *syn_l3, int use_llr, const int *n_bits, const int *direction, IdaOut *out,
                      hipStream_t stream);
int launch_frame_decode(const DemodOut *frames, int n_frames, const int2 *syn_ra, const int2 *syn_hdr, int use_llr,
                        const int *n_bits, DecodedOut *out, hipStream_t stream);
int launch_ida_packed(const DemodOut *frames, int n_frames, const int2 *syn_da, const int2 *syn_l1, const int2 *syn_l2,
                      const int2 *syn_l3, IdaPacked *hp_ida, hipStream_t stream);
int launch_frame_packed(const DemodOut *frames, int n_frames, const int2 *syn_ra, const int2 *syn_hdr, FramePacked *hp_frame,
                        hipStream_t stream);
int launch_demod(const BurstWork *work, int n_bursts, const float2 *frames, int use_gardner,
                 float sps, float2 *ws, DemodOut *out, hipStream_t stream, DemodPacked *hp_packed = nullptr,
                 BurstWork *hp_work = nullptr, int keep_bits = 0);

}
```

### iridium-sniffer_amd/csrc/pipeline.hpp

```cpp
#pragma once
#include <math.h>
#include <stdlib.h>
#include <string.h>
#include <time.h>
#include <errno.h>
#include <sys/stat.h>
#include <algorithm>
#include <deque>
#include <new>
#include <vector>
#include <thread>
#include <mutex>
#include <condition_variable>
#include "../../include/irdm_hip.h"
#include "common.hpp"
#include "host_design.hpp"
#include "kernels.hpp"
#include "libm_port.hpp"
#include "band_core.hpp"
#include "types.hpp"

using namespace irdm;

namespace irdmh {

template <typename T>
inline T *dev_alloc(size_t count)
{
    void *p = nullptr;
    if (hipMalloc(&p, count * sizeof(T)) != hipSuccess) return nullptr;
    return static_cast<T *>(p);
}

template <typename T>
inline T *dev_upload(const T *src, size_t count)
{
    T *p = dev_alloc<T>(count);
    if (!p) return nullptr;
    if (hipMemcpy(p, src, count * sizeof(T), hipMemcpyHostToDevice) != hipSuccess) {
        (void)hipFree(p);
        return nullptr;
    }
    return p;
}

inline int ilog2(int n)
{
    int l = 0;
    while ((1 << l) < n) l++;
    return (1 << l) == n ? l : -1;
}

}


struct irdm_pipeline;

constexpr int kMaxBc = 6;
static inline size_t lpf_alloc(size_t cap) { return cap + cap / 2 + 8; }
static inline float *box_of(float2 *lpf, size_t cap) { return reinterpret_cast<float *>(lpf + cap); }
constexpr int kFeedSlots = 3;
constexpr unsigned kLookAhead = 1;

struct BatchCtx {
    irdm_pipeline *owner;
    hipStream_t stream;
    hipEvent_t ev[4];
    hipEvent_t ev_cfo;
    hipEvent_t ev_rot;
    BurstWork *d_work;
    FirTile *d_tiles;
    size_t tiles_cap;
    float2 *d_dec, *d_lpf, *d_rrc_ws, *d_frames, *d_demod_ws;
    size_t dec_cap;
    DemodOut *d_demod;
    DecodedOut *d_decoded;
    IdaOut *d_ida;
    BurstWork *hp_work, *hp_work_dev;
    FirTile *hp_tiles;
    DemodOut *hp_demod;
    DemodPacked *hp_packed;
    IdaPacked *hp_ida;
    FramePacked *hp_frame;
    uint32_t *hp_flag, *hp_flag_dev;
    int4 *hp_rot_new, *hp_rot_new_dev, *d_rot_new;
    uint32_t cfo_seq;
    bool packed;
    bool parsed;
    bool framed;
    bool cfo_on_device;
    std::vector<double> h_cfreq;
    std::vector<irdm_burst_t> recs;
    int n;
    uint64_t chunk_no;
    uint64_t ring_lo = 0, ring_hi = 0;
    bool owns_buffers;
    float ms[3];
};

struct irdm_pipeline {
    irdm_config_t cfg;
    DetParams P;
    int dev_fmt;
    size_t bps;
    int feed_block, decim, out_rate;
    float peak_signal_db;
    bool dev_cfo;
    bool dev_cfo_ok;
    float sps;
    uint64_t ref_ring, ring_len;
    size_t l_cap;
    int n_ckpt, dec_stride, burst_cap, gone_cap;
    size_t max_chunk;
    int search_depth, pre_start;
    int in_ntaps, noise_ntaps, start_ntaps, rrc_ntaps, dl_len, ul_len;

    hipStream_t stream;
    hipStream_t bstream;
    hipStream_t stream2;
    int bstream_prio;
    hipStream_t sstream;
    hipEvent_t ev_scan_in, ev_scan_out;
    int band_spec_opt = 1;
    void *d_band_spec = nullptr;
    BandWork band_spec = {};
    DetState *d_state_spec = nullptr;
    hipStream_t stream_spec = nullptr;
    hipEvent_t ev_sums1 = nullptr;
    hipEvent_t ev_spec_done = nullptr;
    uint64_t spec_for_no = ~0ull;
    int spec_frames = 0;
    uint64_t stat_spec_passes = 0, stat_spec_scans = 0, stat_sum_restarts = 0;
    uint32_t seq_counter = 0;
    uint32_t fl_seq = 0;
    uint32_t chain_seq = 0;
    uint64_t chain_no = 0;
    int fir_order = 1;
    int fir_generic = 0;
    int post_generic = 0;
    irdm::BandTune band_tune;
    hipEvent_t ev_sk[2];
    hipEvent_t ev[10];

    float *d_window, *d_hist, *d_sum, *d_mag;
    float2 *d_tw, *d_tw4096, *d_tw2048, *d_dl_fft, *d_ul_fft, *d_rot_incr, *d_rot_table;
    DetState *d_state;
    GoneBurst *d_gone;
    PeakCand *d_cand_a, *d_cand_b;
    void *d_ring, *d_stage;
    float *d_in_taps, *d_noise_taps, *d_start_taps, *d_rrc_taps, *d_cfo_window;
    int *d_fir_off;
    BurstWork *d_work;
    FirTile *d_tiles;
    size_t tiles_cap;
    float2 *d_dec, *d_lpf, *d_rrc_ws, *d_frames, *d_demod_ws, *d_probe;
    DemodOut *d_demod;
    DecodedOut *d_decoded;
    int2 *d_syn_ra, *d_syn_hdr;
    int *d_nbits;
    int decode_frames, decode_ida, detect_only;
    IdaOut *d_ida;
    int2 *d_syn_da, *d_syn_l1, *d_syn_l2, *d_syn_l3;
    int *d_dirs;
    std::vector<IdaOut> h_ida;
    std::deque<irdm_ida_t> q_ida;
    std::vector<DecodedOut> h_decoded;
    std::deque<irdm_decoded_t> q_decoded;
    unsigned *d_counts, *d_goff;
    ListEntry *d_entries, *d_compact;
    float *d_pre, *d_sum_bak, *d_hist_bak;
    DetState *d_state_bak;
    int *d_status;
    unsigned long long *d_mc_ops;
    unsigned *d_mc_done;
    int mc_ops_cap, mc_updaters, mc_auto;
    int scan_cus;
    int scan_mode;
    uint64_t stat_fast_chunks, stat_fallbacks, stat_dense_frames;
    int host_primed, host_hist_idx;
    void *d_band;
    BandWork band;
    float *d_smin;
    bool band_ok;
    int fl_mode;
    int fl_done;
    uint64_t stat_plan_tp[16] = {};
    uint64_t stat_tl_dur[32] = {}, stat_tl_gap[32] = {}, stat_tl_n[32] = {};
    uint64_t stat_band_chunks, stat_band_rounds, stat_band_retries, stat_band_aborts, stat_band_extra, stat_chain_undone, stat_chained;
    uint32_t last_band_flags;

    std::vector<GoneBurst> h_gone;
    std::vector<GoneBurst> pend_gone;
    bool has_pending;
    uint64_t pend_c1, pend_no, fl_no;
    int depth;
    int *h_pin;
    int deferred_emitted;
    bool caller_ordered;
    int k1_first;
    bool fl_active, fl_sparse;
    bool fl_band_ran;
    const float *fl_mag, *d_mag_last;
    int fl_frames;
    uint64_t fl_c1, fl_c0;
    hipStream_t fstream;
    float *d_mag2;
    std::vector<BurstWork> h_work;
    BatchCtx bc[kMaxBc];
    int n_bc;
    std::thread cfo_thread;
    std::mutex cfo_mu;
    std::condition_variable cfo_cv;
    std::deque<BatchCtx *> cfo_jobs;
    bool cfo_quit;
    GoneBurst *hp_gone;
    int hp_gone_cap;
    int *h_pin_set[2];
    GoneBurst *hp_gone_set[2];
    hipEvent_t ev_sk_set[2][2], ev_end_set[2], ev_end;
    int out_sel;
    bool chain_pending;
    int chain_sel, chain_band_first;
    bool settle_clean;
    hipEvent_t ev_ring;
    uint64_t chunk_no;
    struct FeedSlot {
        const void *iq;
        uint64_t c0, c1;
        float *mag;
        int frames;
        bool in_ring;
        bool lists;
        hipEvent_t ev_start, ev_k1, ev_copy;
    } fs[kFeedSlots];
    float *k1_pre[kFeedSlots];
    unsigned *k1_counts[kFeedSlots];
    ListEntry *k1_entries[kFeedSlots];
    int k1_lists;
    int band_first;
    int band_auto, fl_band_first;
    const FeedSlot *fl_feed;
    uint64_t stat_k1_lists;
    uint64_t begin_no, end_no;
    uint64_t begun_samples;
    float *d_mag3;
    double host_us[10];
    std::vector<FirTile> h_tiles;
    std::vector<DemodOut> h_demod;
    std::vector<float> h_frames;

    std::deque<irdm_burst_t> q_bursts;
    std::deque<irdm_frame_info_t> q_frames;
    std::deque<std::vector<float>> q_frame_samples;
    std::deque<irdm_demod_t> q_demods;
    std::deque<irdm_demod_packed_t> q_packed;
    int packed_records;
    int parsed_records;
    std::deque<irdm_ida_packed_t> q_ida_packed;
    int frame_records;
    std::deque<irdm_frame_packed_t> q_frame_packed;
    std::deque<irdm_chunk_mark_t> q_marks;
    int chunk_marks;

    uint64_t total_samples, tagged, start_time_ns;
    bool stream_closed;
    int last_frames;
    const void *last_chunk;
    uint64_t last_chunk_start, last_chunk_end;
    std::vector<irdm_burst_t> last_bursts;
    float last_ms[6];
    int keep_frame_samples;
    int *d_rot_slot = nullptr;
    int rot_runs = 0;
    int rot_rows_used = 0;
    int rot_blocks_used = 0, rot_blocks_cap = 0;
    std::vector<int> rot_len_h, rot_want, rot_touched;
    std::vector<int> rot_build_ctx;
    std::vector<uint32_t> rot_build_gen;
    uint32_t rot_gen[kMaxBc] = {}, rot_done_gen[kMaxBc] = {};
    std::vector<float2 *> rot_retired;
    uint64_t stat_rot_builds = 0, stat_rot_rows = 0, stat_rot_ckpts = 0, stat_rot_grows = 0, stat_band_steps = 0;
    hipStream_t stream_rot_pre = nullptr;
    hipEvent_t ev_rot_pre = nullptr;
    int4 *d_rot_pre_news = nullptr;
    bool rot_pre_pending = false;
    int rot_pre_runs = 0;
    size_t scratch_init = 0;
    std::vector<float2 *> scratch_retired;
    std::vector<void *> tiles_retired, tiles_host_retired;
    uint64_t stat_scratch_grows = 0, stat_scratch_peak = 0, stat_tiles_grows = 0, stat_ring_waits = 0;
    uint32_t *hp_gate = nullptr, *hp_gate_dev = nullptr;
    uint32_t gate_seq = 0;
    bool gate_armed = false;
    bool gate_open_pending = false;
    const void *gate_src = nullptr;
    unsigned long long *d_kclk = nullptr;
    int kernel_clock = 0;
    unsigned long long *kclk_rec(int i) const { return kernel_clock && d_kclk ? d_kclk + (size_t)i * kKClkWords : nullptr; }
    unsigned long long *kclk_fir(int c) const { return kclk_rec(c < 3 ? c : 3 + c); }
};


static inline void pipeline_enter(const irdm_pipeline *p) { (void)hipSetDevice(p->cfg.device); }

namespace irdmh {

template <typename T>
static int drain(std::deque<T> &q, T *out, int max)
{
    int n = 0;
    while (n < max && !q.empty()) {
        out[n++] = q.front();
        q.pop_front();
    }
    return n;
}

void pipeline_free(irdm_pipeline *p);
bool chain_stream_create(irdm_pipeline *, hipStream_t *out, int prio);

SampleSource make_source(const irdm_pipeline *p, const void *chunk, uint64_t c0, uint64_t c1);
int ring_guard(irdm_pipeline *p, uint64_t a0, uint64_t a1, hipStream_t st);
int ring_update(irdm_pipeline *p, const void *d_iq, uint64_t c0, uint64_t c1, hipStream_t st);
irdm_decoded_t finish_decoded(const DecodedOut &d, uint64_t id, uint64_t timestamp, double frequency);
int lcw_field(const char *b, int from, int to);
void format_lcw_header(int ft, int lcw_ft, int lcw_code, uint32_t lcw3_val, char *out, size_t outsz);
irdm_ida_t finish_ida(const IdaOut &d, const irdm_demod_t &f);
void cfreq_from_records(BatchCtx &b);
void fine_cfo_host(BatchCtx &b);
void cfo_helper_main(irdm_pipeline *p);
int rot_arena_reset(irdm_pipeline *p, long long blocks);
int rot_prebuild(irdm_pipeline *p);
int rot_rows_prepare(irdm_pipeline *p, BatchCtx &b, int nb, hipStream_t st);
int bursts_enqueue(irdm_pipeline *p, BatchCtx &b, const SampleSource &src, const GoneBurst *gone_list, int nb);
int bursts_finish(irdm_pipeline *p, BatchCtx &b);
int bursts_finish_records(irdm_pipeline *p, BatchCtx &b);
int process_bursts(irdm_pipeline *p, BatchCtx &b, const SampleSource &src, const GoneBurst *gone_list, int n_gone);

int hist_fence(irdm_pipeline *);
uint32_t next_scan_seq(irdm_pipeline *p);
int scan_hop_in(irdm_pipeline *p);
int scan_hop_out(irdm_pipeline *p);
int scan_dense(irdm_pipeline *p, const float *mag, int n_frames, bool timed);
int scan_pick(const irdm_pipeline *p);
int scan_snapshot(irdm_pipeline *p);
int scan_restore(irdm_pipeline *p);
int scan_band_enqueue_at(irdm_pipeline *p, const float *mag, int n_frames, int done, int retry, bool more_rounds,
                                uint64_t c0, const irdm_pipeline::FeedSlot *feed, int sel, int first, int chained,
                                uint32_t seq, uint64_t chunk_no, bool use_spec = false);
int scan_band_enqueue(irdm_pipeline *p, const float *mag, int n_frames, int done, int retry, bool more_rounds = false);
int scan_legacy_enqueue(irdm_pipeline *p, const float *mag, int n_frames, int done, bool sparse);
int scan_export(irdm_pipeline *p);
void scan_select_outputs(irdm_pipeline *p, int sel);
int scan_chain_try(irdm_pipeline *p, irdm_pipeline::FeedSlot &f, uint64_t no);
int spec_enqueue(irdm_pipeline *p, irdm_pipeline::FeedSlot &nx, uint64_t no);
int scan_launch(irdm_pipeline *p, const float *mag, int n_frames, uint64_t c1);
int scan_finish(irdm_pipeline *p, int *n_gone_out);
int settle(irdm_pipeline *p);
int quiesce(irdm_pipeline *p);
int deferred_enqueue(irdm_pipeline *p);
int deferred_finish(irdm_pipeline *p, BatchCtx &b);

}
```

### iridium-sniffer_amd/csrc/scan_band.hip

```cpp
#include <atomic>
#include <mutex>
#include "common.hpp"
#include "types.hpp"
#include "kernels.hpp"
#include "band_core.hpp"
#include "band_wave.hpp"

namespace irdm {

namespace {

__device__ __forceinline__ bool band_void(const BandParams &P, const BandWork &W)
{
    return __hip_atomic_load(W.bar + 5, __ATOMIC_RELAXED, __HIP_MEMORY_SCOPE_AGENT) == (unsigned)P.serial;
}

struct TlScope {
    unsigned long long *lo, *hi;
    __device__ __forceinline__ TlScope(const BandParams &P, const BandWork &W, int slot) : lo(nullptr), hi(nullptr)
    {
        if (P.tl_sel >= 0 && (threadIdx.x & 63) == 0 && slot >= 0 && slot < kBandTlSlots) {
            lo = W.tl + (size_t)P.tl_sel * 2 * kBandTlSlots + slot;
            hi = lo + kBandTlSlots;
            atomicMin(lo, (unsigned long long)wall_clock64());
        }
    }
    __device__ __forceinline__ void leave()
    {
        if (hi) atomicMax(hi, (unsigned long long)wall_clock64());
        hi = nullptr;
    }
    __device__ __forceinline__ ~TlScope() { leave(); }
};

constexpr int kPlanThreads = 1024;
constexpr int kSumDepth = 32;

template <int NT>
__device__ int block_scan(const int32_t *in, int32_t *out, int len, int32_t *s_part)
{
    const int tid = threadIdx.x, lane = tid & 63, wave = tid >> 6;
    const int per = (len + NT - 1) / NT;
    const int lo = tid * per, hi = min(lo + per, len);
    int s = 0;
    for (int i = lo; i < hi; i++) s += in[i];
    int incl = s;
    for (int d = 1; d < 64; d <<= 1) {
        const int v = __shfl_up(incl, d);
        if (lane >= d) incl += v;
    }
    if (lane == 63) s_part[wave] = incl;
    __syncthreads();
    int wave_base = 0, total = 0;
    for (int w = 0; w < NT / 64; w++) {
        const int v = s_part[w];
        if (w < wave) wave_base += v;
        total += v;
    }
    int run = wave_base + incl - s;
    for (int i = lo; i < hi; i++) {
        const int v = in[i];
        out[i] = run;
        run += v;
    }
    __syncthreads();
    return total;
}

__device__ bool boundary_agrees(const BandParams &P, const BandWork &W, int i, int lane)
{
    const int X = (i + 1) * P.band_w;
    const BandRec *A = W.recs + (size_t)i * kBandRecCap, *B = W.recs + (size_t)(i + 1) * kBandRecCap;
    const int na = min((int)W.rec_count[i], kBandRecCap), nb = min((int)W.rec_count[i + 1], kBandRecCap);
    int bad = 0, ca = 0, cb = 0;
    for (int a = lane; a < na; a += 64) {
        if (A[a].cb < X - P.hw || A[a].cb >= X + P.hw) continue;
        ca++;
        bool found = false;
        for (int b = 0; b < nb && !found; b++) found = B[b].cb == A[a].cb && band_rec_same(A[a], B[b]);
        if (!found) bad = 1;
    }
    for (int b = lane; b < nb; b += 64)
        if (B[b].cb >= X - P.hw && B[b].cb < X + P.hw) cb++;
    for (int d = 32; d; d >>= 1) {
        ca += __shfl_xor(ca, d);
        cb += __shfl_xor(cb, d);
        bad |= __shfl_xor(bad, d);
    }
    return !(bad || ca != cb);
}

struct ZoneEnt {
    uint32_t cb, start_lo, idx;
};
constexpr int kZoneCap = 32;
constexpr size_t kZoneLdsBytes = 64 * kZoneCap * (sizeof(ZoneEnt) + sizeof(uint32_t)) + 128 * sizeof(uint32_t);

__device__ void boundaries_agree_lds(const BandParams &P, const BandWork &W, uint8_t *lds, int *s_fail, int nt)
{
    ZoneEnt *zb = reinterpret_cast<ZoneEnt *>(lds);
    uint32_t *za = reinterpret_cast<uint32_t *>(zb + 64 * kZoneCap);
    uint32_t *zc = za + 64 * kZoneCap;
    const int tid = threadIdx.x, gl = tid & 15;
    for (int t = tid; t < 128; t += nt) zc[t] = 0;
    __syncthreads();
    for (int i = tid >> 4; i + 1 < P.n_bands; i += nt >> 4) {
        const int X = (i + 1) * P.band_w;
        const BandRec *A = W.recs + (size_t)i * kBandRecCap, *B = W.recs + (size_t)(i + 1) * kBandRecCap;
        const int na = min((int)W.rec_count[i], kBandRecCap), nb = min((int)W.rec_count[i + 1], kBandRecCap);
        const int nmax = max(na, nb);
        for (int k = gl; k < nmax; k += 16) {
            const int cba = k < na ? A[k].cb : -0x40000000;
            const int cbb = k < nb ? B[k].cb : -0x40000000;
            const uint32_t stb = k < nb ? (uint32_t)B[k].start : 0u;
            if (cba >= X - P.hw && cba < X + P.hw) {
                const uint32_t at = atomicAdd(&zc[2 * i], 1u);
                if (at < (uint32_t)kZoneCap) za[i * kZoneCap + at] = (uint32_t)k;
            }
            if (cbb >= X - P.hw && cbb < X + P.hw) {
                const uint32_t at = atomicAdd(&zc[2 * i + 1], 1u);
                if (at < (uint32_t)kZoneCap) zb[i * kZoneCap + at] = ZoneEnt{ (uint32_t)cbb, stb, (uint32_t)k };
            }
        }
    }
    __syncthreads();
    int bad = 0;
    for (int i = tid >> 4; i + 1 < P.n_bands; i += nt >> 4) {
        const int X = (i + 1) * P.band_w;
        const BandRec *A = W.recs + (size_t)i * kBandRecCap, *B = W.recs + (size_t)(i + 1) * kBandRecCap;
        const int na = min((int)W.rec_count[i], kBandRecCap), nb = min((int)W.rec_count[i + 1], kBandRecCap);
        const int ca = (int)zc[2 * i], cb = (int)zc[2 * i + 1];
        if (ca != cb) {
            bad = 1;
        } else if (ca > kZoneCap) {
            for (int a = gl; a < na; a += 16) {
                if (A[a].cb < X - P.hw || A[a].cb >= X + P.hw) continue;
                bool found = false;
                for (int b = 0; b < nb && !found; b++) found = B[b].cb == A[a].cb && band_rec_same(A[a], B[b]);
                if (!found) bad = 1;
            }
        } else {
            for (int k = gl; k < ca; k += 16) {
                const BandRec ra = A[za[i * kZoneCap + k]];
                bool found = false;
                for (int j = 0; j < cb && !found; j++) {
                    const ZoneEnt e = zb[i * kZoneCap + j];
                    if (e.cb == (uint32_t)ra.cb && e.start_lo == (uint32_t)ra.start) found = band_rec_same(ra, B[e.idx]);
                }
                if (!found) bad = 1;
            }
        }
    }
    if (bad) atomicOr(s_fail, 1);
}

__device__ __forceinline__ SumStep make_step(const BandParams &P, int uf, int old, int slot)
{
    SumStep s;
    const uint32_t row = (uint32_t)P.n * 4u;
    s.nw_off = (uint32_t)uf * row;
    s.ol_off = (uint32_t)(old < 0 ? -old - 1 : old) * row;
    s.snap_off = slot >= 0 ? (uint32_t)slot * row : ~0u;
    s.pad = 0;
    return s;
}
__device__ __forceinline__ SumStep noop_step()
{
    SumStep s;
    s.nw_off = 0;
    s.ol_off = 0;
    s.snap_off = ~0u;
    s.pad = 0;
    return s;
}

struct PlanShared {
    int32_t part[kPlanThreads / 64 + 1];
    int mismatch, first, status, agree_fail;
    unsigned flags;
    int kstar;
};

constexpr int kPlanLdsFrames = 8192;
constexpr size_t kPlanLdsBytes = ((2 * kPlanLdsFrames + 2 + 15) & ~15) + sizeof(int32_t) * (2 * kPlanLdsFrames + 2);
static_assert(kZoneLdsBytes <= kPlanLdsBytes, "the boundary test's lists live in the plan's LDS before the plan needs it");

template <int NT>
__device__ void band_plan_body(const BandParams &P, const BandWork &W, const unsigned *__restrict__ counts,
                               DetState *__restrict__ st, int round, PlanShared &sh, uint8_t *lds,
                               const uint64_t *u_busy = nullptr, const uint64_t *u_forced = nullptr)
{
    const bool first = round == 0 || (P.spec_in && round == 1);
    if (!(P.spec_in && round == 1) || u_busy == nullptr) {
        u_busy = W.busy;
        u_forced = W.forced;
    }
    constexpr int kPlanThreads = NT;
    int32_t *s_part = sh.part;
    int &s_mismatch = sh.mismatch, &s_first = sh.first, &s_status = sh.status, &s_agree_fail = sh.agree_fail;
    unsigned &s_flags = sh.flags;
    const int tid = threadIdx.x;
    BandCtl *ctl = W.ctl;
    if (first) {
        if (tid == 0) {
            const unsigned prev = W.bar[4];
            s_status = (P.chained && prev != 1u) ? 1 : 0;
            if (s_status) __hip_atomic_store(W.bar + 5, (unsigned)P.serial, __ATOMIC_RELAXED, __HIP_MEMORY_SCOPE_AGENT);
            else W.bar[4] = 0;
        }
        __syncthreads();
        if (s_status) return;
        __syncthreads();
    } else if (band_void(P, W)) {
        return;
    }
    if (first) {
        if (tid < (int)(sizeof(BandCtl) / 4)) reinterpret_cast<uint32_t *>(ctl)[tid] = 0;
        if (tid == 0) {
            *W.flags = 0;
            st->n_gone = 0;
        }
        __syncthreads();
        if (round != 0 && tid == 0) ctl->h0 = st->hist_idx;
    }
    if (ctl->status != 0) return;
    const int F = P.n_frames;
    const uint64_t t_begin = wall_clock64();
    uint32_t *tp = ctl->tp + (round == 1 ? 0 : 8);
    auto stamp = [&](int i) {
        if (tid == 0 && round >= 1) tp[i] = (uint32_t)(wall_clock64() - t_begin);
    };

    if (tid == 0) {
        s_mismatch = 0;
        s_first = 0x7fffffff;
        s_flags = 0;
        s_status = 0;
        s_agree_fail = 0;
    }
    __syncthreads();
    if (round == 0) {
        int any = 0;
        for (int f = tid; f < F; f += kPlanThreads) {
            const unsigned c = counts[f];
            W.uq[f] = 0;
            W.uf[f] = 0;
            W.cnt_before[f] = 0;
            const int slot = c > 0 ? 0 : -1;
            W.slot_pre[f] = slot;
            W.slot_post[f] = slot;
            any |= c > 0 ? 1 : 0;
            if (c > (unsigned)P.list_cap) atomicOr(&s_flags, BAND_F_LIST);
        }
        if (any) atomicOr(&s_mismatch, 1);
        for (int i = tid; i < P.n_bands * P.occ_words; i += kPlanThreads) W.occ[i] = 0;
        for (int i = tid; i < P.occ_words; i += kPlanThreads) {
            W.busy[i] = 0;
            W.forced[i] = 0;
            W.conc[i] = 0;
        }
        for (int i = tid; i < P.n_bands; i += kPlanThreads) W.rec_count[i] = 0;
        for (int k = tid; k < 2 * kSumDepth + 1; k += kPlanThreads) W.steps[k] = noop_step();
        __syncthreads();
        if (tid == 0) {
            const int some = s_mismatch;
            ctl->h0 = st->hist_idx;
            W.need[0] = some;
            W.snap_slot[0] = some ? 0 : -1;
            ctl->n_upd = 0;
            ctl->n_snap = some;
            ctl->rounds = 1;
            if (s_flags) {
                ctl->flags = s_flags;
                ctl->status = 2;
            }
        }
        return;
    } else if (first) {
        for (int f = tid; f < F; f += kPlanThreads)
            if (counts[f] > (unsigned)P.list_cap) atomicOr(&s_flags, BAND_F_LIST);
        __syncthreads();
        if (s_flags) {
            if (tid == 0) {
                ctl->flags = s_flags;
                ctl->rounds = 1;
                ctl->status = 2;
            }
            return;
        }
        for (int f = tid; f < F; f += kPlanThreads) {
            W.uq[f] = ((u_busy[f >> 6] >> (f & 63)) & 1) ? 0 : 1;
            W.uf[f] = (uint8_t)((u_forced[f >> 6] >> (f & 63)) & 1);
        }
        if (P.selfcheck & 32) {
            __syncthreads();
            if (tid == 0 && F >= 8) W.uq[(3 * F) / 4] ^= 1;
            __syncthreads();
        }
    } else {
        for (int f = tid; f < F; f += kPlanThreads) {
            const int q = ((W.busy[f >> 6] >> (f & 63)) & 1) ? 0 : 1;
            const int fc = (int)((W.forced[f >> 6] >> (f & 63)) & 1);
            if (q != W.uq[f] || fc != W.uf[f]) {
                atomicAdd(&s_mismatch, 1);
                atomicMin(&s_first, f);
            }
        }
        for (int b = tid; b < P.occ_words; b += kPlanThreads)
            if (W.conc[b] >= (unsigned)P.max_bursts) atomicOr(&s_flags, BAND_F_SQUELCH);
        __syncthreads();
        stamp(0);
        if (P.selfcheck & 2) {
            for (int i = 1; i < P.n_bands; i++) {
                BandRec *B = W.recs + (size_t)i * kBandRecCap;
                const int X = i * P.band_w, nb = min((int)W.rec_count[i], kBandRecCap);
                for (int k = tid; k < nb; k += kPlanThreads)
                    if (B[k].cb >= X - P.hw && B[k].cb < X + P.hw) B[k].last_active += 1;
            }
            __syncthreads();
        }
        if (lds != nullptr) {
            boundaries_agree_lds(P, W, lds, &s_agree_fail, NT);
            if (P.selfcheck & 1) {
                __shared__ int s_other;
                if (tid == 0) s_other = 0;
                __syncthreads();
                for (int i = tid >> 6; i + 1 < P.n_bands; i += kPlanThreads / 64)
                    if (!boundary_agrees(P, W, i, tid & 63) && (tid & 63) == 0) atomicOr(&s_other, 1);
                __syncthreads();
                if (tid == 0 && s_other != s_agree_fail) atomicOr(&s_flags, BAND_F_CHECK);
            }
        } else {
            for (int i = tid >> 6; i + 1 < P.n_bands; i += kPlanThreads / 64)
                if (!boundary_agrees(P, W, i, tid & 63) && (tid & 63) == 0) atomicOr(&s_agree_fail, 1);
        }
        __syncthreads();
        stamp(1);
        if (tid == 0) {
            unsigned fl = s_flags | *W.flags;
            int status = 0;
            if (fl) {
                status = 2;
            } else if (s_mismatch == 0) {
                if (s_agree_fail) {
                    fl |= BAND_F_AGREE;
                    status = 2;
                } else {
                    status = 1;
                }
            } else if (round >= kBandRounds) {
                fl |= BAND_F_ITER;
                status = 2;
            }
            ctl->flags = fl;
            ctl->mismatch = s_mismatch;
            ctl->first_mismatch = s_first;
            ctl->rounds = round;
            ctl->status = status;
            s_status = status;
        }
        __syncthreads();
        if (s_status != 0) return;
        for (int f = tid; f < F; f += kPlanThreads) {
            W.uq[f] = ((W.busy[f >> 6] >> (f & 63)) & 1) ? 0 : 1;
            W.uf[f] = (uint8_t)((W.forced[f >> 6] >> (f & 63)) & 1);
        }
    }
    __syncthreads();
    if (round == 0 && s_flags) {
        if (tid == 0) {
            ctl->flags = s_flags;
            ctl->status = 2;
        }
        return;
    }

    if (lds != nullptr && F <= kPlanLdsFrames) {
        constexpr int FPT = kPlanLdsFrames / NT;
        uint8_t *s_need = lds;
        int32_t *s_slot = reinterpret_cast<int32_t *>(lds + ((2 * kPlanLdsFrames + 2 + 15) & ~15));
        const int f0 = tid * FPT;
        int uqb = 0, ufb = 0, cnz = 0, c_t = 0;
#pragma unroll
        for (int j = 0; j < FPT; j++) {
            const int f = f0 + j;
            if (f < F) {
                int q = ((u_busy[f >> 6] >> (f & 63)) & 1) ? 0 : 1;
                const int fc = (int)((u_forced[f >> 6] >> (f & 63)) & 1);
                if ((P.selfcheck & 32) && first && round == 1 && F >= 8 && f == (3 * F) / 4) q ^= 1;
                uqb |= q << j;
                ufb |= fc << j;
                cnz |= (counts[f] > 0 ? 1 : 0) << j;
                c_t += q + fc;
            }
        }
        __syncthreads();
        stamp(2);
        for (int i = tid; i < P.n_bands * P.occ_words; i += kPlanThreads) W.occ[i] = 0;
        for (int i = tid; i < P.occ_words; i += kPlanThreads) {
            W.busy[i] = 0;
            W.forced[i] = 0;
            W.conc[i] = 0;
        }
        for (int i = tid; i < P.n_bands; i += kPlanThreads) W.rec_count[i] = 0;
        const int lane = tid & 63, wave = tid >> 6;
        auto scan1 = [&](int v, int &total) {
            int incl = v;
            for (int d = 1; d < 64; d <<= 1) {
                const int o = __shfl_up(incl, d);
                if (lane >= d) incl += o;
            }
            if (lane == 63) s_part[wave] = incl;
            __syncthreads();
            int wb = 0, tot = 0;
            for (int w = 0; w < NT / 64; w++) {
                const int o = s_part[w];
                if (w < wave) wb += o;
                tot += o;
            }
            __syncthreads();
            total = tot;
            return wb + incl - v;
        };
        int n_upd = 0;
        const int base = scan1(c_t, n_upd);
        stamp(3);
        for (int k = tid; k <= n_upd + 1; k += kPlanThreads) s_need[k] = (P.sum_restart && k > 0 && (k & 63) == 0) ? 1 : 0;
        __syncthreads();
        {
            int k = base;
#pragma unroll
            for (int j = 0; j < FPT; j++) {
                const int f = f0 + j;
                if (f < F) {
                    const int q = (uqb >> j) & 1, fc = (ufb >> j) & 1;
                    if (f == s_first) sh.kstar = k;
                    if ((cnz >> j) & 1) {
                        s_need[k] = 1;
                        if (fc) s_need[k + 1] = 1;
                    }
                    if (fc) W.upd_frame[k++] = f;
                    if (q) W.upd_frame[k++] = f;
                }
            }
        }
        __syncthreads();
        stamp(4);
        const int kpt = (n_upd + 1 + NT - 1) / NT;
        const int k0 = tid * kpt, k1 = min(k0 + kpt, n_upd + 1);
        int nn = 0;
        for (int k = k0; k < k1; k++) nn += s_need[k];
        int n_snap = 0;
        int run = scan1(nn, n_snap);
        for (int k = k0; k < k1; k++) {
            const int nd = s_need[k];
            s_slot[k] = nd ? run : -1;
            run += nd;
        }
        if (tid == 0) W.snap_slot[0] = s_need[0] ? 0 : -1;
        __syncthreads();
        stamp(5);
        const int h0 = ctl->h0;
        for (int k = n_upd + tid; k < n_upd + 2 * kSumDepth + 1; k += kPlanThreads) W.steps[k] = noop_step();
        for (int k = tid; k < n_upd; k += kPlanThreads) {
            const int uf_k = W.upd_frame[k];
            const int old = k < kHistory ? -(((h0 + k) % kHistory) + 1) : W.upd_frame[k - kHistory];
            W.steps[k] = make_step(P, uf_k, old, s_slot[k + 1]);
        }
        {
            int k = base;
#pragma unroll
            for (int j = 0; j < FPT; j++) {
                const int f = f0 + j;
                if (f < F) {
                    const int q = (uqb >> j) & 1, fc = (ufb >> j) & 1, has = (cnz >> j) & 1;
                    const int pre = has ? s_slot[k] : -1;
                    W.slot_pre[f] = pre;
                    W.slot_post[f] = (has && fc) ? s_slot[k + 1] : pre;
                    k += q + fc;
                }
            }
        }
        __syncthreads();
        stamp(6);
        if (tid == 0) {
            ctl->n_upd = n_upd;
            ctl->n_snap = n_snap;
            ctl->rounds = round + 1;
            if (n_snap > W.snap_cap) {
                ctl->flags = BAND_F_SNAP;
                ctl->status = 2;
            }
            int kr = 0;
            if (P.sum_restart && !first && round >= 2 && s_first != 0x7fffffff && s_first < F) kr = (sh.kstar / 64) * 64;
            if (kr > n_upd) kr = (n_upd / 64) * 64;
            if (kr >= 64 && s_slot[kr] >= 0) {
                ctl->k_restart = kr;
                ctl->restart_slot = s_slot[kr];
                ctl->n_restarts++;
            } else {
                ctl->k_restart = 0;
                ctl->restart_slot = -1;
            }
        }
        return;
    }

    for (int i = tid; i < P.n_bands * P.occ_words; i += kPlanThreads) W.occ[i] = 0;
    for (int i = tid; i < P.occ_words; i += kPlanThreads) {
        W.busy[i] = 0;
        W.forced[i] = 0;
        W.conc[i] = 0;
    }
    for (int i = tid; i < P.n_bands; i += kPlanThreads) W.rec_count[i] = 0;

    for (int f = tid; f < F; f += kPlanThreads) W.tmp[f] = W.uq[f] + W.uf[f];
    __syncthreads();
    const int n_upd = block_scan<NT>(W.tmp, W.cnt_before, F, s_part);
    for (int k = tid; k <= n_upd; k += kPlanThreads) W.need[k] = 0;
    __syncthreads();
    for (int f = tid; f < F; f += kPlanThreads) {
        int k = W.cnt_before[f];
        if (counts[f] > 0) {
            W.need[k] = 1;
            if (W.uf[f]) W.need[k + 1] = 1;
        }
        if (W.uf[f]) W.upd_frame[k++] = f;
        if (W.uq[f]) W.upd_frame[k] = f;
    }
    __syncthreads();
    const int n_snap = block_scan<NT>(W.need, W.tmp, n_upd + 1, s_part);
    for (int k = tid; k <= n_upd; k += kPlanThreads) W.snap_slot[k] = W.need[k] ? W.tmp[k] : -1;
    __syncthreads();
    const int h0 = ctl->h0;
    for (int k = n_upd + tid; k < n_upd + 2 * kSumDepth + 1; k += kPlanThreads) W.steps[k] = noop_step();
    for (int k = tid; k < n_upd; k += kPlanThreads) {
        W.snap_after[k] = W.snap_slot[k + 1];
        W.old_row[k] = k < kHistory ? -(((h0 + k) % kHistory) + 1) : W.upd_frame[k - kHistory];
        W.steps[k] = make_step(P, W.upd_frame[k], W.old_row[k], W.snap_after[k]);
    }
    for (int f = tid; f < F; f += kPlanThreads) {
        const int k = W.cnt_before[f];
        const int pre = counts[f] > 0 ? W.snap_slot[k] : -1;
        W.slot_pre[f] = pre;
        W.slot_post[f] = (counts[f] > 0 && W.uf[f]) ? W.snap_slot[k + 1] : pre;
    }
    if (tid == 0) {
        ctl->n_upd = n_upd;
        ctl->n_snap = n_snap;
        ctl->rounds = round + 1;
        if (n_snap > W.snap_cap) {
            ctl->flags = BAND_F_SNAP;
            ctl->status = 2;
        }
    }
}

__device__ void band_commit_body(const BandParams &P, const BandWork &W, DetState *__restrict__ st,
                                 float *__restrict__ sum, GoneBurst *__restrict__ gone, int gone_cap,
                                 unsigned char *smem_raw);
template <int NT>
__global__ __launch_bounds__(NT) void band_plan_kernel(BandParams P, BandWork W, const unsigned *__restrict__ counts,
                                                       DetState *__restrict__ st, int round, float *__restrict__ sum,
                                                       GoneBurst *__restrict__ gone, int gone_cap, const float *__restrict__ pre,
                                                       float *__restrict__ smin_out, const uint64_t *u_busy,
                                                       const uint64_t *u_forced)
{
    IRDM_DETECTOR_PRIO();
    TlScope tl(P, W, 4 * round);
    __shared__ PlanShared sh;
    extern __shared__ __attribute__((aligned(16))) unsigned char plan_lds[];
    static_assert(kPlanLdsBytes >= (size_t)kBandMaxTotal * 10, "the fused commit sorts in the plan pass's LDS");
    band_plan_body<NT>(P, W, counts, st, round, sh, (P.selfcheck & 16) ? nullptr : plan_lds, u_busy, u_forced);
    if (round == 0 && pre != nullptr) {
        __syncthreads();
        if (!band_void(P, W) && W.ctl->status == 0) {
            const int slot0 = W.snap_slot[0];
            for (int b = (int)threadIdx.x; b < P.n; b += NT) {
                const float sv = sum[b];
                if (slot0 >= 0) W.snap[(size_t)slot0 * P.n + b] = sv;
                W.sum_new[b] = sv;
                smin_out[b] = sv;
                if (!(pre[b] <= 0.9f * P.thr * sv)) atomicOr(W.flags, BAND_F_STALE);
            }
        }
    }
    if (round >= 1 && !(P.selfcheck & 16)) {
        __syncthreads();
        if (!band_void(P, W) && W.ctl->status == 1) band_commit_body(P, W, st, sum, gone, gone_cap, plan_lds);
    }
}


__device__ __forceinline__ __amdgpu_buffer_rsrc_t band_rsrc(const void *p, size_t bytes)
{
    return __builtin_amdgcn_make_buffer_rsrc(const_cast<void *>(p), 0, (int)(bytes > 0x7fffffffu ? 0x7fffffffu : bytes), 0x00020000);
}

__device__ __forceinline__ void band_sum_body(const BandParams &P, const BandWork &W, const float *__restrict__ mag,
                                              const float *__restrict__ hist, const float *__restrict__ sum,
                                              const float *__restrict__ pre, float *__restrict__ smin_out,
                                              const SumStep *steps, float *snap, int b)
{
    const BandCtl *ctl = W.ctl;
    const int N = P.n;
    const int n = ctl->n_upd;
    const int k_begin = ctl->k_restart;
    float s = sum[b], smin = s;
    const int slot0 = W.snap_slot[0];
    if (k_begin > 0) {
        s = snap[(size_t)ctl->restart_slot * N + b];
        smin = __builtin_fminf(smin_out[b], s);
    } else if (slot0 >= 0) {
        snap[(size_t)slot0 * N + b] = s;
    }
    const size_t row = (size_t)N * 4;
    const __amdgpu_buffer_rsrc_t r_mag = band_rsrc(mag, (size_t)P.n_frames * row);
    const __amdgpu_buffer_rsrc_t r_hist = band_rsrc(hist, (size_t)kHistory * row);
    const __amdgpu_buffer_rsrc_t r_snap = band_rsrc(snap, (size_t)W.snap_cap * row);
    const int boff = b * 4;

    static_assert(kHistory % kSumDepth == 0, "a batch of steps must not straddle the history ring's length");
    static_assert(kSumDepth == 32, "two batches per 64 descriptors");
    static_assert(sizeof(SumStep) == 16, "a descriptor is one 16-byte load");
    const int lane = (int)(threadIdx.x & 63);
    const uint4 *steps4 = reinterpret_cast<const uint4 *>(steps);
    float nwA[kSumDepth], olA[kSumDepth], nwB[kSumDepth], olB[kSumDepth];
#define IRDM_SUM_LOAD(NWv, OLv, D, half, k0)                                                            \
    {                                                                                                   \
        const __amdgpu_buffer_rsrc_t r_old = (k0) < kHistory ? r_hist : r_mag;                          \
        _Pragma("unroll") for (int j = 0; j < kSumDepth; j++) {                                         \
            const int o_nw = __builtin_amdgcn_readlane((int)D.x, (half) * kSumDepth + j);               \
            const int o_ol = __builtin_amdgcn_readlane((int)D.y, (half) * kSumDepth + j);               \
            NWv[j] = __builtin_bit_cast(float, __builtin_amdgcn_raw_buffer_load_b32(r_mag, boff, o_nw, 0)); \
            OLv[j] = __builtin_bit_cast(float, __builtin_amdgcn_raw_buffer_load_b32(r_old, boff, o_ol, 0)); \
        }                                                                                               \
    }
#define IRDM_SUM_STEP(NWv, OLv, D, half)                                                                \
    {                                                                                                   \
        const float dd = s - OLv[j];       \
        s = dd + NWv[j];                                                                                \
        smin = __builtin_fminf(smin, s);                                                                      \
        if ((snaps >> ((half) * kSumDepth + j)) & 1)                                                    \
            __builtin_amdgcn_raw_buffer_store_b32(__builtin_bit_cast(int, s), r_snap, boff,             \
                                                  __builtin_amdgcn_readlane((int)D.z, (half) * kSumDepth + j), 0); \
    }
#define IRDM_SUM_CONSUME(NWv, OLv, D, half, k0)                                                         \
    {                                                                                                   \
        const unsigned long long snaps = __builtin_amdgcn_ballot_w64(D.z != ~0u);                       \
        if ((k0) + kSumDepth <= n) {                                                                    \
            _Pragma("unroll") for (int j = 0; j < kSumDepth; j++) IRDM_SUM_STEP(NWv, OLv, D, half)      \
        } else {                                                                                        \
            _Pragma("unroll") for (int j = 0; j < kSumDepth; j++)                                       \
                if ((k0) + j < n) IRDM_SUM_STEP(NWv, OLv, D, half)                                      \
        }                                                                                               \
    }
    uint4 d = steps4[k_begin + lane], dn = steps4[k_begin + 2 * kSumDepth + lane];
    IRDM_SUM_LOAD(nwA, olA, d, 0, k_begin)
    for (int k0 = k_begin; k0 < n; k0 += 2 * kSumDepth) {
        const bool more = k0 + 2 * kSumDepth < n;
        const uint4 dnn = steps4[k0 + 4 * kSumDepth + lane];
        IRDM_SUM_LOAD(nwB, olB, d, 1, k0 + kSumDepth)
        IRDM_SUM_CONSUME(nwA, olA, d, 0, k0)
        if (more) { IRDM_SUM_LOAD(nwA, olA, dn, 0, k0 + 2 * kSumDepth) }
        IRDM_SUM_CONSUME(nwB, olB, d, 1, k0 + kSumDepth)
        d = dn;
        dn = dnn;
    }
#undef IRDM_SUM_LOAD
#undef IRDM_SUM_CONSUME
#undef IRDM_SUM_STEP
    W.sum_new[b] = s;
    smin_out[b] = smin;
    if (!(pre[b] <= 0.9f * P.thr * smin)) atomicOr(W.flags, BAND_F_STALE);
}

__global__ __launch_bounds__(64) void band_sum_kernel(BandParams P, BandWork W, const float *__restrict__ mag,
                                                      const float *__restrict__ hist, const float *__restrict__ sum,
                                                      const float *__restrict__ pre, float *__restrict__ smin_out,
                                                      const SumStep *__restrict__ steps, float *__restrict__ snap)
{
    IRDM_DETECTOR_PRIO();
    TlScope tl(P, W, 4 * (W.ctl->rounds - 1) + 1);
    if (band_void(P, W) || W.ctl->status != 0) return;
    band_sum_body(P, W, mag, hist, sum, pre, smin_out, steps, snap, (int)blockIdx.x * 64 + (int)threadIdx.x);
}

constexpr int kWalkWaveGroups = 256;

template <int NW>
__global__ __launch_bounds__(256) void band_walk_wave_kernel(BandParams P, BandWork W, BandIO io, const DetState *__restrict__ st)
{
    IRDM_DETECTOR_PRIO();
    TlScope tl(P, W, 4 * (W.ctl->rounds - 1) + 3);
    if (band_void(P, W) || W.ctl->status != 0) return;
    io.act_in = st->act;
    io.n_act_in = (int32_t)wv_first((uint32_t)st->n_act);
    const int lane = threadIdx.x & 63;
    const int gw = (int)wv_first((uint32_t)(blockIdx.x * 4 + (threadIdx.x >> 6))), n_waves = (int)gridDim.x * 4;
    const int n_pairs = P.n_bands * P.occ_words;
    unsigned long long *tl_stat = nullptr;
    if (P.tl_sel >= 0)
        tl_stat = W.tl + (size_t)P.tl_sel * 2 * kBandTlSlots + kBandTlSlots + (W.ctl->rounds - 1 == 0 ? 26 : 28);
    int wave_events = 0;
    const unsigned long long t_wave = tl_stat ? wall_clock64() : 0;
    for (int p0 = gw; p0 < n_pairs; p0 += 64 * n_waves) {
        const int pl = p0 + lane * n_waves;
        bool work = false;
        if (pl < n_pairs) {
            const int band = pl / P.occ_words, blk = pl % P.occ_words;
            work = blk == 0 || band_segment_starts(io.occ + (size_t)band * P.occ_words, blk, P.gap, false) != 0;
        }
        uint64_t todo = __builtin_amdgcn_ballot_w64(work);
        while (todo) {
            const int j = __builtin_ctzll(todo);
            todo &= todo - 1;
            const int p = p0 + j * n_waves;
            const int band = p / P.occ_words, blk = p % P.occ_words;
            bool carried = false;
            int events = 0;
            if (blk == 0) {
                WaveWalker<NW> w(P, io, band, lane);
                if (w.load_carried() > 0) {
                    carried = true;
                    w.run(0, true);
                    events += w.n_events;
                }
            }
            uint64_t starts = wv_first64(band_segment_starts(io.occ + (size_t)band * P.occ_words, blk, P.gap, carried));
            while (starts) {
                const int q = __builtin_ctzll(starts);
                starts &= starts - 1;
                WaveWalker<NW> w(P, io, band, lane);
                w.run(64 * blk + q, false);
                events += w.n_events;
            }
            wave_events += events;
            if (tl_stat && lane == 0) {
                atomicMax(tl_stat, (unsigned long long)events);
                atomicAdd(tl_stat + 1, (unsigned long long)events);
            }
        }
    }
    if (tl_stat && lane == 0 && W.ctl->rounds - 1 != 0) {
        unsigned long long *x = W.tl + (size_t)P.tl_sel * 2 * kBandTlSlots + kBandTlSlots + 30;
        atomicMax(x, (unsigned long long)wave_events);
        atomicMax(x + 1, wall_clock64() - t_wave);
    }
}

__device__ __forceinline__ void band_cross_wave(const BandParams &P, const BandWork &W, unsigned c,
                                                const ListEntry *__restrict__ entries, int f, uint32_t *s_bits, int lane)
{
    const int N = P.n;
    for (int w = lane; w < N / 32; w += 64) s_bits[w] = 0;
    __builtin_amdgcn_fence(__ATOMIC_RELEASE, "wavefront");
    __builtin_amdgcn_wave_barrier();
    const float *srow = W.snap + (size_t)W.slot_pre[f] * N;
    const ListEntry *e = entries + (size_t)f * P.list_cap;
    float *rq = W.relq + (size_t)f * N;
    for (unsigned i = lane; i < c; i += 64) {
        const int bin = e[i].bin;
        const float base = srow[bin];
        const float rel = base > 0 ? e[i].mag / base : 0.0f;
        if (rel > P.thr) {
            atomicOr(&s_bits[bin >> 5], 1u << (bin & 31));
            rq[bin] = rel;
        }
    }
    __builtin_amdgcn_fence(__ATOMIC_ACQ_REL, "wavefront");
    __builtin_amdgcn_wave_barrier();
    uint32_t *out = reinterpret_cast<uint32_t *>(W.cross) + (size_t)f * (N / 32);
    for (int w = lane; w < N / 32; w += 64) out[w] = s_bits[w];
    if (lane < P.n_bands) {
        const int w0 = (lane * P.band_w - P.band_w / 2) / 32, nw = 2 * P.band_w / 32;
        uint32_t any = 0;
        for (int k = 0; k < nw; k++) {
            const int w = w0 + k;
            if (w >= 0 && w < N / 32) any |= s_bits[w];
        }
        if (any) atomicOr(reinterpret_cast<unsigned long long *>(&W.occ[(size_t)lane * P.occ_words + (f >> 6)]), 1ull << (f & 63));
    }
    __builtin_amdgcn_fence(__ATOMIC_ACQ_REL, "wavefront");
    __builtin_amdgcn_wave_barrier();
}

constexpr int kCrossGroups = 256;

__global__ __launch_bounds__(256) void band_cross_w_kernel(BandParams P, BandWork W, const unsigned *__restrict__ counts,
                                                           const ListEntry *__restrict__ entries)
{
    IRDM_DETECTOR_PRIO();
    TlScope tl(P, W, 4 * (W.ctl->rounds - 1) + 2);
    __shared__ uint32_t s_bits_all[4][16384 / 32];
    if (band_void(P, W) || W.ctl->status != 0) return;
    const int lane = threadIdx.x & 63, wave = threadIdx.x >> 6;
    const int gw = (int)blockIdx.x * 4 + wave, n_waves = (int)gridDim.x * 4;
    uint32_t *s_bits = s_bits_all[wave];
    for (int f0 = gw; f0 < P.n_frames; f0 += 64 * n_waves) {
        const int fl = f0 + lane * n_waves;
        const unsigned cl = fl < P.n_frames ? counts[fl] : 0u;
        uint64_t todo = __builtin_amdgcn_ballot_w64(cl != 0 && cl <= (unsigned)P.list_cap);
        while (todo) {
            const int j = __builtin_ctzll(todo);
            todo &= todo - 1;
            const unsigned c = (unsigned)__builtin_amdgcn_readlane((int)cl, j);
            band_cross_wave(P, W, c, entries, f0 + j * n_waves, s_bits, lane);
        }
    }
}


__global__ __launch_bounds__(256) void band_spec_prep_kernel(BandParams P, BandWork S, const unsigned *__restrict__ counts,
                                                              const float *__restrict__ sum_src, DetState *__restrict__ st_spec,
                                                              int have_prev)
{
    IRDM_DETECTOR_PRIO();
    const int tid = threadIdx.x, F = P.n_frames;
    __shared__ unsigned s_n;
    if (tid == 0) s_n = 0;
    __syncthreads();
    if (have_prev)
        for (int band = tid >> 4; band < P.n_bands; band += 256 / 16) {
            const int cnt = min((int)S.rec_count[band], kBandRecCap);
            for (int j = tid & 15; j < cnt; j += 16) {
                const BandRec &r = S.recs[(size_t)band * kBandRecCap + j];
                if (!(r.flags & 1) || r.stop >= 0) continue;
                const unsigned at = atomicAdd(&s_n, 1u);
                if (at < (unsigned)kMaxActive) {
                    ActiveBurst a;
                    a.id = 0; a.start = (uint64_t)r.start; a.last_active = (uint64_t)r.last_active;
                    a.center_bin = r.cb; a.peak_rel = r.rel; a.base_sum = r.base; a.pad = 0;
                    st_spec->act[at] = a;
                }
            }
        }
    __syncthreads();
    if (tid == 0) st_spec->n_act = (uint32_t)min(s_n, (unsigned)kMaxActive);
    if (tid < (int)(sizeof(BandCtl) / 4)) reinterpret_cast<uint32_t *>(S.ctl)[tid] = 0;
    for (int f = tid; f < F; f += 256) {
        const int slot = counts[f] > 0 ? 0 : -1;
        S.slot_pre[f] = slot;
        S.slot_post[f] = slot;
    }
    for (int i = tid; i < P.n_bands * P.occ_words; i += 256) S.occ[i] = 0;
    for (int i = tid; i < P.occ_words; i += 256) {
        S.busy[i] = 0;
        S.forced[i] = 0;
        S.conc[i] = 0;
    }
    for (int i = tid; i < P.n_bands; i += 256) S.rec_count[i] = 0;
    for (int b = tid; b < P.n; b += 256) S.snap[b] = sum_src[b];
    __syncthreads();
    if (tid == 0) {
        *S.flags = 0;
        S.ctl->rounds = 1;
        S.snap_slot[0] = 0;
    }
}

__device__ void lds_bitonic_sort(uint64_t *key, uint16_t *val, int np)
{
    for (int k = 2; k <= np; k <<= 1) {
        for (int j = k >> 1; j > 0; j >>= 1) {
            for (int i = threadIdx.x; i < np / 2; i += blockDim.x) {
                const int lo = ((i & ~(j - 1)) << 1) | (i & (j - 1)), hi = lo | j;
                const uint64_t a = key[lo], b = key[hi];
                if ((a > b) == ((lo & k) == 0)) {
                    key[lo] = b;
                    key[hi] = a;
                    const uint16_t va = val[lo];
                    val[lo] = val[hi];
                    val[hi] = va;
                }
            }
            __syncthreads();
        }
    }
}

__device__ void band_commit_body(const BandParams &P, const BandWork &W, DetState *__restrict__ st,
                                 float *__restrict__ sum, GoneBurst *__restrict__ gone, int gone_cap,
                                 unsigned char *smem_raw)
{
    const int kPlanThreads = (int)blockDim.x;
    uint64_t *s_key = reinterpret_cast<uint64_t *>(smem_raw);
    uint16_t *s_val = reinterpret_cast<uint16_t *>(s_key + kBandMaxTotal);
    uint32_t *rank_of = W.rank;
    __shared__ unsigned s_n, s_carried, s_gone;
    BandCtl *ctl = W.ctl;
    if (band_void(P, W) || ctl->status != 1 || ctl->committed) return;
    const int tid = threadIdx.x;
    if (tid == 0) {
        s_n = 0;
        s_carried = 0;
        s_gone = 0;
    }
    __syncthreads();
    for (int band = tid >> 4; band < P.n_bands; band += kPlanThreads / 16) {
        {
            const int cnt = min((int)W.rec_count[band], kBandRecCap);
            for (int j = tid & 15; j < cnt; j += 16) {
                const int i = band * kBandRecCap + j;
                const BandRec &r = W.recs[i];
                if (!(r.flags & 1)) continue;
                const unsigned at = atomicAdd(&s_n, 1u);
                if (at < (unsigned)kBandMaxTotal) W.tot[at] = i;
                if (r.cf < 0) atomicAdd(&s_carried, 1u);
                if (r.stop >= 0) atomicAdd(&s_gone, 1u);
            }
        }
    }
    __syncthreads();
    const int n = (int)s_n, n_carried = (int)s_carried, n_gone = (int)s_gone;
    if (n > kBandMaxTotal || n_gone > gone_cap) {
        if (tid == 0) {
            ctl->flags |= n > kBandMaxTotal ? BAND_F_TOTAL : BAND_F_GONECAP;
            ctl->n_gone = n_gone;
            ctl->status = 2;
        }
        return;
    }
    for (int t = tid; t < n; t += kPlanThreads) {
        const BandRec &r = W.recs[W.tot[t]];
        uint64_t key;
        if (r.cf < 0) {
            key = (uint64_t)r.seq;
        } else {
            uint32_t rb;
            __builtin_memcpy(&rb, &r.rel, 4);
            key = (1ull << 63) | ((uint64_t)r.cf << 46) | ((uint64_t)(0xffffffffu - rb) << 14) | (uint64_t)r.cb;
        }
        s_key[t] = key;
        s_val[t] = (uint16_t)t;
    }
    int np = 2;
    while (np < n) np <<= 1;
    for (int t = n + tid; t < np; t += kPlanThreads) {
        s_key[t] = ~0ull;
        s_val[t] = 0xffff;
    }
    __syncthreads();
    lds_bitonic_sort(s_key, s_val, np);
    for (int q = tid; q < n; q += kPlanThreads) rank_of[s_val[q]] = (uint32_t)q;
    __syncthreads();
    const uint64_t id0 = st->burst_id;
    for (int t = tid; t < n; t += kPlanThreads) {
        const BandRec &r = W.recs[W.tot[t]];
        W.ids[t] = r.cf < 0 ? st->act[r.seq].id : id0 + 10ull * (uint64_t)((int)rank_of[t] - n_carried);
    }
    for (int t = tid; t < n; t += kPlanThreads) {
        const BandRec &r = W.recs[W.tot[t]];
        s_key[t] = r.stop >= 0 ? (((uint64_t)((r.stop - (int64_t)P.idx0) >> P.log_n)) << 32) | rank_of[t]
                               : (1ull << 63) | rank_of[t];
        s_val[t] = (uint16_t)t;
    }
    for (int t = n + tid; t < np; t += kPlanThreads) {
        s_key[t] = ~0ull;
        s_val[t] = 0xffff;
    }
    __syncthreads();
    lds_bitonic_sort(s_key, s_val, np);
    for (int pos = tid; pos < n; pos += kPlanThreads) {
        const int t = s_val[pos];
        const BandRec &r = W.recs[W.tot[t]];
        const uint64_t id = W.ids[t];
        if (r.stop >= 0) {
            GoneBurst g;
            g.id = id; g.start = (uint64_t)r.start; g.stop = (uint64_t)r.stop; g.last_active = (uint64_t)r.last_active;
            g.center_bin = r.cb; g.peak_rel = r.rel; g.base_sum = r.base; g.pad = 0;
            gone[pos] = g;
        } else {
            ActiveBurst a;
            a.id = id; a.start = (uint64_t)r.start; a.last_active = (uint64_t)r.last_active;
            a.center_bin = r.cb; a.peak_rel = r.rel; a.base_sum = r.base; a.pad = 0;
            st->act[pos - n_gone] = a;
        }
    }
    for (int b = tid; b < P.n; b += kPlanThreads) sum[b] = W.sum_new[b];
    if (tid == 0) {
        const int F = P.n_frames;
        st->index += (uint64_t)F * (uint64_t)P.n;
        st->burst_id = id0 + 10ull * (uint64_t)(n - n_carried);
        st->hist_idx = (ctl->h0 + ctl->n_upd) % kHistory;
        st->squelch = st->squelch > F ? st->squelch - F : 0;
        st->n_act = n - n_gone;
        st->n_gone = (uint32_t)n_gone;
        ctl->n_gone = n_gone;
        ctl->n_total = n;
        ctl->committed = 1;
        W.bar[4] = 1;
    }
}

__global__ __launch_bounds__(kPlanThreads) void band_commit_kernel(BandParams P, BandWork W, DetState *__restrict__ st,
                                                                   float *__restrict__ sum, GoneBurst *__restrict__ gone,
                                                                   int gone_cap)
{
    IRDM_DETECTOR_PRIO();
    TlScope tl(P, W, 24);
    extern __shared__ __attribute__((aligned(16))) unsigned char smem_raw[];
    band_commit_body(P, W, st, sum, gone, gone_cap, smem_raw);
}

constexpr int kExportBlocks = 32;

__global__ __launch_bounds__(256) void band_history_kernel(BandParams P, BandWork W, const float *__restrict__ mag,
                                                           float *__restrict__ hist, const DetState *__restrict__ st,
                                                           const uint32_t *__restrict__ gone, int gone_cap,
                                                           uint32_t *__restrict__ hp_gone, uint32_t *__restrict__ hp_hdr,
                                                           uint32_t *__restrict__ hp_ctl)
{
    IRDM_DETECTOR_PRIO();
    TlScope tl(P, W, 25);
    const BandCtl *ctl = W.ctl;
    if (band_void(P, W)) {
        if (hp_ctl && blockIdx.x == 0 && threadIdx.x == 0) {
            __hip_atomic_store(hp_ctl + 2, (uint32_t)BAND_F_CHAIN, __ATOMIC_RELAXED, __HIP_MEMORY_SCOPE_SYSTEM);
            __hip_atomic_store(hp_ctl + 0, 2u, __ATOMIC_RELAXED, __HIP_MEMORY_SCOPE_SYSTEM);
            __threadfence_system();
        }
        return;
    }
    if (hp_hdr && blockIdx.x < kExportBlocks)
        gone_export_body(st, gone, gone_cap, hp_gone, hp_hdr, reinterpret_cast<const uint32_t *>(ctl), hp_ctl,
                         (int)(sizeof(BandCtl) / 4), kExportBlocks);
    if (ctl->status != 1 || !ctl->committed) return;
    const int k = ctl->n_upd - 1 - (int)blockIdx.x;
    if (k < 0) return;
    const float4 *src = reinterpret_cast<const float4 *>(mag + (size_t)W.upd_frame[k] * P.n);
    float4 *dst = reinterpret_cast<float4 *>(hist + (size_t)((ctl->h0 + k) % kHistory) * P.n);
    for (int i0 = threadIdx.x; i0 < P.n / 4; i0 += 8 * 256) {
        float4 v[8];
#pragma unroll
        for (int u = 0; u < 8; u++)
            if (i0 + 256 * u < P.n / 4) v[u] = src[i0 + 256 * u];
#pragma unroll
        for (int u = 0; u < 8; u++)
            if (i0 + 256 * u < P.n / 4) dst[i0 + 256 * u] = v[u];
    }
}

}

int band_list_cap(int n) { return n < kBandListCap ? n : kBandListCap; }

int band_scan_supported(const DetParams &D, BandParams *out, int n_frames, uint64_t idx0)
{
    BandParams P;
    P.n = D.n;
    P.log_n = 31 - __builtin_clz((unsigned)(D.n > 0 ? D.n : 1));
    P.nw64 = D.n / 64;
    P.n_frames = n_frames;
    P.occ_words = (n_frames + 63) / 64;
    P.hw = D.width / 2;
    P.pre_len = D.pre_len;
    P.post_len = D.post_len;
    P.max_len = D.max_len;
    P.max_bursts = D.max_bursts;
    P.band_w = P.hw <= 20 ? 128 : 256;
    P.n_bands = D.n / P.band_w;
    P.gap = (D.post_len + D.n - 1) / D.n;
    P.thr = D.threshold;
    P.idx0 = idx0;
    P.list_cap = band_list_cap(D.n);
    if (out) *out = P;
    if (D.n < 2048 || D.n > 16384 || D.n != (1 << P.log_n) || P.n_bands < 1 || P.n_bands > 64) return 0;
    if (P.hw < 1 || 2 * P.hw + 8 > P.band_w / 2) return 0;
    if (P.gap < 1 || P.gap >= 64) return 0;
    if (D.max_bursts <= 0 || D.max_bursts > kMaxActive - 64) return 0;
    return 1;
}

size_t band_work_bytes(int n, size_t max_chunk, bool spec)
{
    const size_t F = max_chunk / (size_t)n + 2;
    size_t b = 0;
    auto add = [&](size_t x) { b += (x + 255) & ~(size_t)255; };
    add(sizeof(BandCtl));
    add(F); add(F);
    add(4 * (F + 2)); add(4 * (2 * F + 4));
    add(4 * (2 * F + 4)); add(4 * (2 * F + 4)); add(4 * (2 * F + 4));
    add(sizeof(SumStep) * (2 * F + 4 + 3 * kSumDepth + 6 * kSumDepth));
    add(4 * (2 * F + 4)); add(4 * (2 * F + 4));
    add(4 * F); add(4 * F);
    add(F * (size_t)n / 8);
    add(F * (size_t)n * 4);
    add((spec ? 2 : F + 2 + F / 32 + 4) * (size_t)n * 4);
    add(64 * ((F + 63) / 64) * 8);
    add(((F + 63) / 64) * 8); add(((F + 63) / 64) * 8); add(((F + 63) / 64) * 4);
    add(sizeof(BandRec) * 64 * kBandRecCap); add(4 * 64);
    add(4 * (size_t)n); add(4 * kBandMaxTotal); add(8 * kBandMaxTotal); add(256);
    add(256); add(4 * kBandMaxTotal);
    add(8 * 4 * kBandTlSlots);
    return b;
}

int band_work_carve(BandWork *W, void *base, int n, size_t max_chunk, bool spec)
{
    const size_t F = max_chunk / (size_t)n + 2;
    unsigned char *p = static_cast<unsigned char *>(base);
    auto take = [&](size_t x) { void *q = p; p += (x + 255) & ~(size_t)255; return q; };
    W->ctl = static_cast<BandCtl *>(take(sizeof(BandCtl)));
    W->uq = static_cast<uint8_t *>(take(F));
    W->uf = static_cast<uint8_t *>(take(F));
    W->cnt_before = static_cast<int32_t *>(take(4 * (F + 2)));
    W->tmp = static_cast<int32_t *>(take(4 * (2 * F + 4)));
    W->upd_frame = static_cast<int32_t *>(take(4 * (2 * F + 4)));
    W->old_row = static_cast<int32_t *>(take(4 * (2 * F + 4)));
    W->snap_after = static_cast<int32_t *>(take(4 * (2 * F + 4)));
    W->steps = static_cast<SumStep *>(take(sizeof(SumStep) * (2 * F + 4 + 3 * kSumDepth + 6 * kSumDepth)));
    W->need = static_cast<int32_t *>(take(4 * (2 * F + 4)));
    W->snap_slot = static_cast<int32_t *>(take(4 * (2 * F + 4)));
    W->slot_pre = static_cast<int32_t *>(take(4 * F));
    W->slot_post = static_cast<int32_t *>(take(4 * F));
    W->cross = static_cast<uint64_t *>(take(F * (size_t)n / 8));
    W->relq = static_cast<float *>(take(F * (size_t)n * 4));
    W->snap = static_cast<float *>(take((spec ? 2 : F + 2 + F / 32 + 4) * (size_t)n * 4));
    W->snap_cap = (int)(spec ? 2 : F + 2 + F / 32 + 4);
    W->occ = static_cast<uint64_t *>(take(64 * ((F + 63) / 64) * 8));
    W->busy = static_cast<uint64_t *>(take(((F + 63) / 64) * 8));
    W->forced = static_cast<uint64_t *>(take(((F + 63) / 64) * 8));
    W->conc = static_cast<uint32_t *>(take(((F + 63) / 64) * 4));
    W->recs = static_cast<BandRec *>(take(sizeof(BandRec) * 64 * kBandRecCap));
    W->rec_count = static_cast<uint32_t *>(take(4 * 64));
    W->sum_new = static_cast<float *>(take(4 * (size_t)n));
    W->tot = static_cast<uint32_t *>(take(4 * kBandMaxTotal));
    W->ids = static_cast<uint64_t *>(take(8 * kBandMaxTotal));
    W->flags = static_cast<uint32_t *>(take(256));
    W->bar = static_cast<unsigned *>(take(256));
    W->rank = static_cast<uint32_t *>(take(4 * kBandMaxTotal));
    W->tl = static_cast<unsigned long long *>(take(8 * 4 * kBandTlSlots));
    return 0;
}

static unsigned next_launch_serial()
{
    static std::atomic<unsigned> launch_serial{ 0 };
    unsigned serial = launch_serial.fetch_add(1) + 1;
    if (serial == 0) serial = launch_serial.fetch_add(1) + 1;
    return serial;
}

int launch_band_spec(const DetParams &D, BandWork S, DetState *st_spec, const float *sum_src, int n_frames, uint64_t idx0,
                     const unsigned *counts, const ListEntry *entries, int have_prev, hipStream_t stream, const BandTune &tune)
{
    BandParams P;
    if (!band_scan_supported(D, &P, n_frames, idx0) || n_frames < 1) return -1;
    P.serial = (int32_t)next_launch_serial();
    P.selfcheck = tune.selfcheck & 8;
    BandIO io;
    io.cross = S.cross;
    io.occ = S.occ;
    io.relq = S.relq;
    io.snap = S.snap;
    io.slot_post = S.slot_post;
    io.act_in = nullptr;
    io.n_act_in = 0;
    io.recs = S.recs;
    io.rec_count = S.rec_count;
    io.busy = S.busy;
    io.forced = S.forced;
    io.conc = S.conc;
    io.flags = S.flags;
    hipLaunchKernelGGL(band_spec_prep_kernel, dim3(1), dim3(256), 0, stream, P, S, counts, sum_src, st_spec, have_prev);
    hipLaunchKernelGGL(band_cross_w_kernel, dim3(kCrossGroups), dim3(256), 0, stream, P, S, counts, entries);
    if (P.band_w == 128)
        hipLaunchKernelGGL((band_walk_wave_kernel<4>), dim3(kWalkWaveGroups), dim3(256), 0, stream, P, S, io, st_spec);
    else
        hipLaunchKernelGGL((band_walk_wave_kernel<8>), dim3(kWalkWaveGroups), dim3(256), 0, stream, P, S, io, st_spec);
    return hipGetLastError() == hipSuccess ? 0 : -1;
}

int launch_band_scan(const DetParams &D, BandWork W, DetState *st, float *sum, float *hist, const float *mag,
                     int n_frames, uint64_t idx0, const unsigned *counts, const ListEntry *entries, const float *pre,
                     float *smin, GoneBurst *gone, int gone_cap, int round_begin, int round_end, GoneBurst *hp_gone,
                     uint32_t *hp_hdr, void *hp_ctl, int hp_cap, int chained, int tl_sel, hipStream_t stream,
                     const BandTune &tune, const uint32_t *gate_flag, uint32_t gate_seq, uint32_t *gate_err, const void *gate_src,
                     size_t gate_bytes, const BandWork *spec, hipEvent_t sums_done)
{
    if (spec && round_begin != 1) return -1;
    const uint64_t *ub = spec ? spec->busy : nullptr, *uf = spec ? spec->forced : nullptr;
    bool sums_noted = sums_done == nullptr;
    BandParams P;
    if (!band_scan_supported(D, &P, n_frames, idx0) || n_frames < 1) return -1;
    P.serial = (int32_t)next_launch_serial();
    P.chained = chained;
    P.spec_in = spec ? 1 : 0;
    P.sum_restart = tune.sum_restart;
    P.selfcheck = tune.selfcheck;
    P.tl_sel = tune.timeline && tl_sel >= 0 && tl_sel < 2 ? tl_sel : -1;
    if (P.tl_sel >= 0 && (round_begin == 0 || spec)) {
        unsigned long long *half = W.tl + (size_t)P.tl_sel * 2 * kBandTlSlots;
        (void)hipMemsetAsync(half, 0xff, 8 * kBandTlSlots, stream);
        (void)hipMemsetAsync(half + kBandTlSlots, 0, 8 * kBandTlSlots, stream);
    }
    BandIO io;
    io.cross = W.cross;
    io.occ = W.occ;
    io.relq = W.relq;
    io.snap = W.snap;
    io.slot_post = W.slot_post;
    io.act_in = nullptr;
    io.n_act_in = 0;
    io.recs = W.recs;
    io.rec_count = W.rec_count;
    io.busy = W.busy;
    io.forced = W.forced;
    io.conc = W.conc;
    io.flags = W.flags;
    const size_t commit_lds = (size_t)kBandMaxTotal * (8 + 2);
    (void)hipFuncSetAttribute((const void *)band_commit_kernel, hipFuncAttributeMaxDynamicSharedMemorySize, (int)commit_lds);
    (void)hipFuncSetAttribute((const void *)band_plan_kernel<kPlanThreads>, hipFuncAttributeMaxDynamicSharedMemorySize, (int)kPlanLdsBytes);
    for (int round = round_begin; round <= round_end; round++) {
        if (round > round_begin || round_begin == 0 || spec) {
            const size_t plan_lds = (P.selfcheck & 16) ? 0 : kPlanLdsBytes;
            const float *pre0 = round == 0 ? pre : nullptr;
            hipLaunchKernelGGL(band_plan_kernel<kPlanThreads>, dim3(1), dim3(kPlanThreads), plan_lds, stream, P, W, counts, st, round, sum,
                               gone, gone_cap, pre0, smin, ub, uf);
        }
        if (round == round_end) break;
        if (gate_flag && round == (round_begin > 1 ? round_begin : 1)) {
            if (launch_wait_host_flag(gate_flag, gate_seq, gate_err, stream) != 0) return -1;
            if (hipMemcpyAsync(hist, gate_src, gate_bytes, hipMemcpyDeviceToDevice, stream) != hipSuccess) return -1;
        }
        if (round >= 1)
            hipLaunchKernelGGL(band_sum_kernel, dim3(P.n / 64), dim3(64), 0, stream, P, W, mag, hist, sum, pre, smin, W.steps, W.snap);
        if (!sums_noted && round >= 1) {
            if (hipEventRecord(sums_done, stream) != hipSuccess) return -1;
            sums_noted = true;
        }
        hipLaunchKernelGGL(band_cross_w_kernel, dim3(kCrossGroups), dim3(256), 0, stream, P, W, counts, entries);
        if (P.band_w == 128)
            hipLaunchKernelGGL((band_walk_wave_kernel<4>), dim3(kWalkWaveGroups), dim3(256), 0, stream, P, W, io, st);
        else
            hipLaunchKernelGGL((band_walk_wave_kernel<8>), dim3(kWalkWaveGroups), dim3(256), 0, stream, P, W, io, st);
    }
    if (P.selfcheck & 16)
        hipLaunchKernelGGL(band_commit_kernel, dim3(1), dim3(kPlanThreads), commit_lds, stream, P, W, st, sum, gone, gone_cap);
    static_assert(kHistory >= kExportBlocks, "the export rides on the history pass's first workgroups");
    hipLaunchKernelGGL(band_history_kernel, dim3(kHistory), dim3(256), 0, stream, P, W, mag, hist, st,
                       reinterpret_cast<const uint32_t *>(gone), hp_cap < gone_cap ? hp_cap : gone_cap,
                       reinterpret_cast<uint32_t *>(hp_gone), hp_hdr, static_cast<uint32_t *>(hp_ctl));
    return hipGetLastError() == hipSuccess ? 0 : -1;
}

}
```

### iridium-sniffer_amd/csrc/scan_host.cpp

```cpp
#include "pipeline.hpp"

namespace irdmh {

int hist_fence(irdm_pipeline *) { return 0; }

uint32_t next_scan_seq(irdm_pipeline *p)
{
    if (++p->seq_counter == 0) ++p->seq_counter;
    return p->seq_counter;
}

int scan_hop_in(irdm_pipeline *p)
{
    if (p->sstream == p->stream) return 0;
    IRDM_HIP_CHECK(hipEventRecord(p->ev_scan_in, p->stream));
    IRDM_HIP_CHECK(hipStreamWaitEvent(p->sstream, p->ev_scan_in, 0));
    return 0;
}

int scan_hop_out(irdm_pipeline *p)
{
    if (p->sstream == p->stream) return 0;
    IRDM_HIP_CHECK(hipEventRecord(p->ev_scan_out, p->sstream));
    IRDM_HIP_CHECK(hipStreamWaitEvent(p->stream, p->ev_scan_out, 0));
    return 0;
}

int scan_dense(irdm_pipeline *p, const float *mag, int n_frames, bool timed)
{
    if (hist_fence(p) != 0 || scan_hop_in(p) != 0) return -1;
    if (timed) IRDM_HIP_CHECK(hipEventRecord(p->ev_sk[0], p->sstream));
    if (launch_detect_scan(p->P, p->d_state, p->d_sum, p->d_hist, mag, n_frames, p->d_gone, p->gone_cap,
                           p->d_cand_a, p->d_cand_b, p->sstream) != 0)
        return -1;
    if (timed) IRDM_HIP_CHECK(hipEventRecord(p->ev_sk[1], p->sstream));
    if (scan_hop_out(p) != 0) return -1;
    p->stat_dense_frames += n_frames;
    return 0;
}

int scan_pick(const irdm_pipeline *p)
{
    if (p->scan_mode == 1) return 0;
    if ((p->scan_mode == 0 || p->scan_mode == 4) && p->band_ok) return 2;
    return p->P.n >= 2048 ? 1 : 0;
}

int scan_snapshot(irdm_pipeline *p)
{
    const DetParams &P = p->P;
    if (hist_fence(p) != 0) return -1;
    IRDM_HIP_CHECK(hipMemcpyAsync(p->d_sum_bak, p->d_sum, sizeof(float) * P.n, hipMemcpyDeviceToDevice, p->stream));
    IRDM_HIP_CHECK(hipMemcpyAsync(p->d_hist_bak, p->d_hist, sizeof(float) * (size_t)kHistory * P.n,
                                  hipMemcpyDeviceToDevice, p->stream));
    IRDM_HIP_CHECK(hipMemcpyAsync(p->d_state_bak, p->d_state, sizeof(DetState), hipMemcpyDeviceToDevice, p->stream));
    return 0;
}

int scan_restore(irdm_pipeline *p)
{
    const DetParams &P = p->P;
    if (hist_fence(p) != 0) return -1;
    IRDM_HIP_CHECK(hipMemcpyAsync(p->d_sum, p->d_sum_bak, sizeof(float) * P.n, hipMemcpyDeviceToDevice, p->stream));
    IRDM_HIP_CHECK(hipMemcpyAsync(p->d_hist, p->d_hist_bak, sizeof(float) * (size_t)kHistory * P.n,
                                  hipMemcpyDeviceToDevice, p->stream));
    IRDM_HIP_CHECK(hipMemcpyAsync(p->d_state, p->d_state_bak, sizeof(DetState), hipMemcpyDeviceToDevice, p->stream));
    return 0;
}

int scan_band_enqueue_at(irdm_pipeline *p, const float *mag, int n_frames, int done, int retry, bool more_rounds,
                                uint64_t c0, const irdm_pipeline::FeedSlot *feed, int sel, int first, int chained,
                                uint32_t seq, uint64_t chunk_no, bool use_spec)
{
    (void)seq; (void)chunk_no;
    const DetParams &P = p->P;
    const float *mag_rest = mag + (size_t)done * P.n;
    const uint64_t idx0 = c0 + (uint64_t)done * (uint64_t)P.n;
    const bool from_k1 = feed && feed->lists && done == 0;
    const int ls = from_k1 && p->depth ? (int)(feed - p->fs) : 0;
    float *pre = from_k1 ? p->k1_pre[ls] : p->d_pre;
    unsigned *counts = from_k1 ? p->k1_counts[ls] : p->d_counts;
    ListEntry *entries = from_k1 ? p->k1_entries[ls] : p->d_entries;
    int *pin = p->h_pin_set[sel];
    GoneBurst *hpg = p->hp_gone_set[sel];
    if (more_rounds) {
        return launch_band_scan(P, p->band, p->d_state, p->d_sum, p->d_hist, mag_rest, n_frames - done, idx0, counts, entries, pre,
                                p->d_smin, p->d_gone, p->gone_cap, first, kBandRounds, hpg,
                                reinterpret_cast<uint32_t *>(pin + 64), pin + 96, p->hp_gone_cap, 0, sel, p->stream, p->band_tune);
    }
    if (!from_k1 || retry) {
        if (launch_prefilter_lists(p->d_sum, P.threshold, pre, retry ? p->d_smin : nullptr, mag_rest, P.n, counts,
                                   entries, n_frames - done, band_list_cap(P.n), p->stream) != 0)
            return -1;
    } else {
        p->stat_k1_lists++;
    }
    IRDM_HIP_CHECK(hipEventRecord(p->ev_sk_set[sel][0], p->stream));
    const bool gate = p->gate_armed && !retry && p->hp_gate_dev;
    if (gate) {
        p->gate_armed = false;
        p->gate_open_pending = true;
    }
    if (launch_band_scan(P, p->band, p->d_state, p->d_sum, p->d_hist, mag_rest, n_frames - done, idx0, counts,
                         entries, pre, p->d_smin, p->d_gone, p->gone_cap, use_spec ? 1 : 0, first, hpg,
                         reinterpret_cast<uint32_t *>(pin + 64), pin + 96, p->hp_gone_cap, chained, sel, p->stream, p->band_tune,
                         gate ? p->hp_gate_dev : nullptr, p->gate_seq, gate ? p->hp_gate_dev + 1 : nullptr,
                         p->gate_src, sizeof(float) * (size_t)kHistory * P.n,
                         use_spec ? &p->band_spec : nullptr, p->ev_sums1) != 0)
        return -1;
    if (use_spec) p->stat_spec_scans++;
    IRDM_HIP_CHECK(hipEventRecord(p->ev_sk_set[sel][1], p->stream));
    return 0;
}

int scan_band_enqueue(irdm_pipeline *p, const float *mag, int n_frames, int done, int retry, bool more_rounds)
{
    if (!more_rounds && !retry) p->fl_band_first = p->band_first ? p->band_first : p->band_auto;
    return scan_band_enqueue_at(p, mag, n_frames, done, retry, more_rounds, p->fl_c0, p->fl_feed, p->out_sel, p->fl_band_first, 0,
                                p->fl_seq, p->fl_no);
}

int scan_legacy_enqueue(irdm_pipeline *p, const float *mag, int n_frames, int done, bool sparse)
{
    const DetParams &P = p->P;
    if (hist_fence(p) != 0) return -1;
    if (sparse) {
        IRDM_HIP_CHECK(hipMemsetAsync(p->d_status, 0, sizeof(int) * 64, p->stream));
        if (done < n_frames) {
            const float *mag_rest = mag + (size_t)done * P.n;
            if (launch_prefilter(p->d_sum, P.threshold, p->d_pre, mag_rest, P.n, p->d_counts, p->d_entries,
                                 p->d_goff, p->d_compact, n_frames - done, p->stream) != 0)
                return -1;
            const int upd = (p->scan_mode == 3 || (p->scan_mode != 2 && p->mc_auto))
                                ? std::min(p->mc_updaters, p->scan_cus - 1) : 0;
            const int mc_words = (int)std::min<size_t>((size_t)p->mc_ops_cap, 3 * (size_t)(n_frames - done) + 64);
            if (upd > 0) {
                IRDM_HIP_CHECK(hipMemsetAsync(p->d_mc_ops, 0, sizeof(unsigned long long) * (size_t)mc_words, p->stream));
                IRDM_HIP_CHECK(hipMemsetAsync(p->d_mc_done, 0, sizeof(unsigned) * 32 * 16, p->stream));
            }
            if (scan_hop_in(p) != 0) return -1;
            IRDM_HIP_CHECK(hipEventRecord(p->ev_sk[0], p->sstream));
            if (launch_detect_scan_fast(P, p->d_state, p->d_sum, p->d_hist, mag_rest, n_frames - done,
                                        p->d_counts, p->d_goff, p->d_compact, p->d_pre, p->d_gone,
                                        p->gone_cap, p->d_status, p->d_mc_ops, mc_words, p->d_mc_done, upd, p->sstream) != 0)
                return -1;
            IRDM_HIP_CHECK(hipEventRecord(p->ev_sk[1], p->sstream));
            if (scan_hop_out(p) != 0) return -1;
        }
        IRDM_HIP_CHECK(hipMemcpyAsync(p->h_pin, p->d_status, sizeof(int) * 64, hipMemcpyDeviceToHost, p->stream));
    } else if (done < n_frames) {
        if (scan_dense(p, mag + (size_t)done * P.n, n_frames - done, true) != 0) return -1;
    }
    return 0;
}

int scan_export(irdm_pipeline *p)
{
    const bool band = p->fl_mode == 2 && p->fl_band_ran;
    return launch_gone_export(p->d_state, p->d_gone, std::min(p->gone_cap, p->hp_gone_cap), p->hp_gone,
                              reinterpret_cast<uint32_t *>(p->h_pin + 64), band ? p->band.ctl : nullptr, p->h_pin + 96,
                              (int)sizeof(BandCtl), p->stream);
}

void scan_select_outputs(irdm_pipeline *p, int sel)
{
    p->out_sel = sel;
    p->h_pin = p->h_pin_set[sel];
    p->hp_gone = p->hp_gone_set[sel];
    p->ev_sk[0] = p->ev_sk_set[sel][0];
    p->ev_sk[1] = p->ev_sk_set[sel][1];
    p->ev_end = p->ev_end_set[sel];
}

int scan_chain_try(irdm_pipeline *p, irdm_pipeline::FeedSlot &f, uint64_t no)
{
    p->chain_pending = false;
    if (!p->fl_active || p->fl_mode != 2 || !p->fl_band_ran || !p->host_primed || scan_pick(p) != 2 ||
        f.frames < 1 || !f.lists)
        return 0;
    const int sel = p->out_sel ^ 1;
    IRDM_HIP_CHECK(hipStreamWaitEvent(p->stream, f.ev_k1, 0));
    memset(p->h_pin_set[sel] + 96, 0, sizeof(BandCtl));
    p->chain_band_first = p->band_first ? p->band_first : p->band_auto;
    p->chain_seq = next_scan_seq(p);
    const bool use_spec = p->band_spec_opt && p->d_band_spec && p->spec_for_no == no && p->chain_band_first >= 2 &&
                          f.frames == p->spec_frames && !p->gate_armed;
    if (use_spec) IRDM_HIP_CHECK(hipStreamWaitEvent(p->stream, p->ev_spec_done, 0));
    if (scan_band_enqueue_at(p, f.mag, f.frames, 0, 0, false, f.c0, &f, sel, p->chain_band_first, 1, p->chain_seq, no, use_spec) != 0) return -1;
    IRDM_HIP_CHECK(hipEventRecord(p->ev_end_set[sel], p->stream));
    p->chain_pending = true;
    p->chain_no = no;
    p->chain_sel = sel;
    p->stat_chained++;
    return 0;
}

int spec_enqueue(irdm_pipeline *p, irdm_pipeline::FeedSlot &nx, uint64_t no)
{
    if (!p->band_spec_opt || !p->d_band_spec || !p->host_primed || scan_pick(p) != 2 || nx.frames < 1 || !nx.lists) return 0;
    const int ls = (int)(&nx - p->fs);
    IRDM_HIP_CHECK(hipStreamWaitEvent(p->stream_spec, nx.ev_k1, 0));
    IRDM_HIP_CHECK(hipStreamWaitEvent(p->stream_spec, p->ev_sums1, 0));
    const int have_prev = p->spec_for_no != ~0ull && p->spec_for_no + 1 == no;
    if (launch_band_spec(p->P, p->band_spec, p->d_state_spec, p->band.sum_new, nx.frames, nx.c0, p->k1_counts[ls], p->k1_entries[ls],
                         have_prev, p->stream_spec, p->band_tune) != 0)
        return -1;
    IRDM_HIP_CHECK(hipEventRecord(p->ev_spec_done, p->stream_spec));
    p->spec_for_no = no;
    p->spec_frames = nx.frames;
    p->stat_spec_passes++;
    return 0;
}

int scan_launch(irdm_pipeline *p, const float *mag, int n_frames, uint64_t c1)
{
    if (p->chain_pending) {
        p->chain_pending = false;
        p->fl_mode = 2;
        p->fl_sparse = false;
        p->fl_mag = mag;
        p->fl_frames = n_frames;
        p->fl_c1 = c1;
        p->fl_c0 = p->total_samples;
        p->fl_no = p->chunk_no;
        p->fl_done = 0;
        p->fl_band_ran = true;
        p->fl_band_first = p->chain_band_first;
        p->fl_seq = p->chain_seq;
        scan_select_outputs(p, p->chain_sel);
        p->fl_active = true;
        return 0;
    }
    p->fl_mode = scan_pick(p);
    if (p->fl_mode != 2 || !p->host_primed) IRDM_HIP_CHECK(hipMemsetAsync(&p->d_state->n_gone, 0, sizeof(uint32_t), p->stream));
    p->fl_sparse = p->fl_mode == 1;
    p->fl_mag = mag;
    p->fl_frames = n_frames;
    p->fl_c1 = c1;
    p->fl_c0 = p->total_samples;
    p->fl_no = p->chunk_no;
    p->fl_seq = next_scan_seq(p);
    int done = 0;
    if (!p->host_primed && p->fl_mode != 0) {
        done = std::min(n_frames, kHistory - p->host_hist_idx);
        if (scan_dense(p, mag, done, done == n_frames) != 0) return -1;
    }
    p->fl_done = done;
    if (p->fl_mode == 2) {
        memset(p->h_pin + 96, 0, sizeof(BandCtl));
        p->fl_band_ran = done < n_frames;
        if (done < n_frames) {
            if (scan_band_enqueue(p, mag, n_frames, done, 0) != 0) return -1;
        } else {
            reinterpret_cast<BandCtl *>(p->h_pin + 96)->status = 1;
        }
    } else {
        if (scan_snapshot(p) != 0) return -1;
        if (scan_legacy_enqueue(p, mag, n_frames, done, p->fl_mode == 1) != 0) return -1;
    }
    if (!(p->fl_mode == 2 && p->fl_band_ran) && scan_export(p) != 0) return -1;
    IRDM_HIP_CHECK(hipEventRecord(p->ev_end, p->stream));
    p->fl_active = true;
    return 0;
}

int scan_finish(irdm_pipeline *p, int *n_gone_out)
{
    *n_gone_out = 0;
    if (!p->fl_active) return 0;
    p->fl_active = false;
    auto now_us = [] {
        struct timespec ts;
        clock_gettime(CLOCK_MONOTONIC, &ts);
        return ts.tv_sec * 1e6 + ts.tv_nsec * 1e-3;
    };
    double tq0 = now_us(), tq1;
    IRDM_HIP_CHECK(hipEventSynchronize(p->ev_end));
    if (p->gate_open_pending) {
        p->gate_open_pending = false;
        if (p->hp_gate[1]) {
            fprintf(stderr, "irdm_hip: the detector scan waited for a history import that never came (irdm_expect_history)\n");
            p->hp_gate[1] = 0;
            return -1;
        }
    }
    tq1 = now_us(); p->host_us[6] += tq1 - tq0; tq0 = tq1;
    int redo_from = p->fl_done;
    bool redone = false;
    if (p->fl_mode == 2) {
        const BandCtl *ctl = reinterpret_cast<const BandCtl *>(p->h_pin + 96);
        int tries = 0;
        auto more_rounds = [&]() -> int {
            if (ctl->status != 0 || ctl->flags != 0 || !p->fl_band_ran) return 0;
            redone = true;
            p->stat_band_extra++;
            if (scan_band_enqueue(p, p->fl_mag, p->fl_frames, p->fl_done, 0, true) != 0) return -1;
            if (scan_export(p) != 0) return -1;
            IRDM_HIP_CHECK(hipStreamSynchronize(p->stream));
            return 0;
        };
        if (more_rounds() != 0) return -1;
        while (ctl->status != 1 && ctl->flags == BAND_F_STALE && tries < 2) {
            tries++;
            redone = true;
            p->stat_band_retries++;
            if (scan_band_enqueue(p, p->fl_mag, p->fl_frames, p->fl_done, 1) != 0) return -1;
            if (scan_export(p) != 0) return -1;
            IRDM_HIP_CHECK(hipStreamSynchronize(p->stream));
            if (more_rounds() != 0) return -1;
        }
        p->stat_band_rounds += (uint64_t)ctl->rounds;
        p->stat_band_steps += (uint64_t)(ctl->n_upd > 0 ? ctl->n_upd : 0);
        if (p->band_tune.timeline && p->fl_band_ran) {
            unsigned long long tl[2 * kBandTlSlots];
            IRDM_HIP_CHECK(hipMemcpy(tl, p->band.tl + (size_t)p->out_sel * 2 * kBandTlSlots, sizeof(tl), hipMemcpyDeviceToHost));
            for (int i = 26; i < 32; i++) p->stat_tl_dur[i] += tl[kBandTlSlots + i];
            unsigned long long prev_end = 0;
            for (int i = 0; i < 26; i++) {
                const unsigned long long lo = tl[i], hi = tl[kBandTlSlots + i];
                if (lo == ~0ull || hi == 0 || hi < lo) continue;
                p->stat_tl_dur[i] += hi - lo;
                if (prev_end && lo > prev_end) p->stat_tl_gap[i] += lo - prev_end;
                p->stat_tl_n[i]++;
                prev_end = hi;
            }
        }
        for (int i = 0; i < 16; i++) p->stat_plan_tp[i] += ctl->tp[i];
        p->stat_sum_restarts += (uint64_t)(ctl->n_restarts > 0 ? ctl->n_restarts : 0);
        if (ctl->status == 1) {
            p->band_auto = std::min(std::max(ctl->rounds, 2), kBandRounds);
            p->stat_band_chunks++;
            p->stat_fast_chunks++;
        } else {
            p->stat_band_aborts++;
            p->stat_fallbacks++;
            redone = true;
            p->last_band_flags = ctl->flags;
            if (getenv("IRDM_SCAN_DEBUG"))
                fprintf(stderr, "irdm_hip: band scan declined the chunk (flags 0x%x, %d rounds, %d mismatches from frame %d) -> sequential scan\n",
                        ctl->flags, ctl->rounds, ctl->mismatch, ctl->first_mismatch);
            p->fl_mode = p->P.n >= 2048 && p->scan_mode != 4 ? 1 : 0;
            p->fl_sparse = p->fl_mode == 1;
            IRDM_HIP_CHECK(hipMemsetAsync(&p->d_state->n_gone, 0, sizeof(uint32_t), p->stream));
            if (scan_snapshot(p) != 0) return -1;
            if (scan_legacy_enqueue(p, p->fl_mag, p->fl_frames, p->fl_done, p->fl_mode == 1) != 0) return -1;
            IRDM_HIP_CHECK(hipEventRecord(p->ev[2], p->stream));
            IRDM_HIP_CHECK(hipStreamSynchronize(p->stream));
        }
    }
    if (p->fl_mode == 1) {
        const int status = p->h_pin[0];
        if (getenv("IRDM_SCAN_DEBUG")) {
            const long long *d = reinterpret_cast<const long long *>(p->h_pin + 4);
            fprintf(stderr, "scan dbg (10ns ticks): all=%lld leader=%lld | stage=%lld(%lld) cross=%lld(%lld) hc=%lld(%lld) find=%lld(%lld) "
                            "partA=%lld(%lld) partB=%lld(%lld) | publish=%lld(nbulk %lld) frame_end=%lld(%lld) | cmdcross=%lld(%lld) cmdbulk=%lld(%lld) busytop_total=%lld(%lld) fast1=%lld(%lld) fast2=%lld(%lld) bulk_frames=%lld\n",
                    d[0], d[7], d[1], d[13], d[2], d[14], d[3], d[15], d[4], d[16], d[5], d[17], d[6], d[18], d[8], d[20], d[9], d[21],
                    d[10], d[22], d[11], d[23], d[12], d[24], d[25], d[26], d[27], d[28], d[29]);
        }
        if (status != 0) {
            p->stat_fallbacks++;
            redone = true;
            if (getenv("IRDM_SCAN_DEBUG")) fprintf(stderr, "irdm_hip: sparse scan aborted with status 0x%x -> dense scan\n", status);
            if (scan_restore(p) != 0) return -1;
            if (scan_dense(p, p->fl_mag + (size_t)redo_from * p->P.n, p->fl_frames - redo_from, true) != 0) return -1;
            IRDM_HIP_CHECK(hipEventRecord(p->ev[2], p->stream));
        } else {
            p->stat_fast_chunks++;
        }
    }
    volatile uint32_t *counters = reinterpret_cast<volatile uint32_t *>(p->h_pin + 64);
    volatile int32_t *hdr = p->h_pin + 66;
    p->settle_clean = !redone;
    if (redone) {
        if (scan_export(p) != 0) return -1;
        IRDM_HIP_CHECK(hipStreamSynchronize(p->stream));
    }
    tq1 = now_us(); p->host_us[7] += tq1 - tq0; tq0 = tq1;
    p->host_hist_idx = hdr[0];
    p->host_primed = hdr[1];
    int n_gone = (int)counters[0];
    if (counters[1] || n_gone > p->gone_cap) {
        p->settle_clean = false;
        const int want = std::max(n_gone, p->gone_cap) + 4096;
        GoneBurst *bigger = dev_alloc<GoneBurst>((size_t)want);
        if (!bigger) {
            fprintf(stderr, "irdm_hip: %d bursts in one chunk and no memory for their records\n", n_gone);
            return -1;
        }
        (void)hipFree(p->d_gone);
        p->d_gone = bigger;
        p->gone_cap = want;
        p->h_gone.resize(want);
        p->stat_fallbacks++;
        if (p->gone_cap > p->hp_gone_cap) {
            p->hp_gone_cap = p->gone_cap;
            for (int s = 0; s < 2; s++) {
                (void)hipHostFree(p->hp_gone_set[s]);
                p->hp_gone_set[s] = nullptr;
                if (hipHostMalloc(reinterpret_cast<void **>(&p->hp_gone_set[s]), sizeof(GoneBurst) * (size_t)p->hp_gone_cap, hipHostMallocDefault) != hipSuccess)
                    return -1;
            }
            p->hp_gone = p->hp_gone_set[p->out_sel];
        }
        if (scan_restore(p) != 0) return -1;
        if (scan_dense(p, p->fl_mag + (size_t)redo_from * p->P.n, p->fl_frames - redo_from, true) != 0) return -1;
        if (scan_export(p) != 0) return -1;
        IRDM_HIP_CHECK(hipStreamSynchronize(p->stream));
        p->host_hist_idx = hdr[0];
        p->host_primed = hdr[1];
        n_gone = (int)counters[0];
        if (counters[1] || n_gone > p->gone_cap) {
            fprintf(stderr, "irdm_hip: detector capacity exceeded (%d bursts in one chunk, cap %d)\n", n_gone, p->gone_cap);
            return -1;
        }
    }
    if (n_gone > 0) memcpy(p->h_gone.data(), p->hp_gone, sizeof(GoneBurst) * n_gone);
    tq1 = now_us(); p->host_us[8] += tq1 - tq0; tq0 = tq1;
    float ms = 0;
    p->last_ms[1] = hipEventElapsedTime(&ms, p->ev_sk[0], p->ev_sk[1]) == hipSuccess ? ms : -1.0f;
    p->last_frames = p->fl_frames;
    p->d_mag_last = p->fl_mag;
    p->tagged += (uint64_t)n_gone;
    *n_gone_out = n_gone;
    return 0;
}

int settle(irdm_pipeline *p)
{
    if (!p->fl_active) return 0;
    pipeline_enter(p);
    const uint64_t c1 = p->fl_c1;
    int n_gone = 0;
    if (scan_finish(p, &n_gone) != 0) return -1;
    p->pend_gone.assign(p->h_gone.begin(), p->h_gone.begin() + n_gone);
    p->has_pending = true;
    p->pend_c1 = c1;
    p->pend_no = p->fl_no;
    return 0;
}

int quiesce(irdm_pipeline *p)
{
    pipeline_enter(p);
    if (settle(p) != 0) return -1;
    IRDM_HIP_CHECK(hipDeviceSynchronize());
    return 0;
}

int deferred_enqueue(irdm_pipeline *p)
{
    if (!p->has_pending) return 0;
    BatchCtx &b = p->bc[p->pend_no % p->n_bc];
    b.chunk_no = p->pend_no;
    const SampleSource src = make_source(p, nullptr, 0, p->pend_c1);
    const int n = (int)p->pend_gone.size();
    int base = 0;
    IRDM_HIP_CHECK(hipStreamWaitEvent(b.stream, p->ev_ring, 0));
    IRDM_HIP_CHECK(hipStreamWaitEvent(b.stream, p->fs[p->pend_no % kFeedSlots].ev_copy, 0));
    if (p->begin_no > 0) {
        const irdm_pipeline::FeedSlot &newest = p->fs[(p->begin_no - 1) % kFeedSlots];
        if (p->k1_first >= 2) IRDM_HIP_CHECK(hipStreamWaitEvent(b.stream, newest.ev_copy, 0));
        else if (p->k1_first == 1) IRDM_HIP_CHECK(hipStreamWaitEvent(b.stream, newest.ev_k1, 0));
    }
    while (n - base > p->burst_cap) {
        if (process_bursts(p, b, src, p->pend_gone.data() + base, p->burst_cap) != 0) return -1;
        base += p->burst_cap;
    }
    if (bursts_enqueue(p, b, src, p->pend_gone.data() + base, n - base) != 0) return -1;
    p->has_pending = false;
    return 0;
}

int deferred_finish(irdm_pipeline *p, BatchCtx &b)
{
    return bursts_finish(p, b);
}

}
```

Baseline: 75940.

## Speculatively run next chunk's band round-1 plan and sums ahead on spec stream

Adds a second band workspace and a speculative 'ahead' pass that runs the next chunk's round-1 plan and window-sum update on the spec stream. It uses the previous chunk's update list to predict the history-ring state. The main scan then consumes the precomputed round, and if the serial check fails it refuses with BAND_F_AHEAD and the host reruns the chunk. The aim is to overlap round-1 work with the current chunk's tail. The cost is extra memory, double-buffered workspace bookkeeping, and a redo path when the speculation mismatches.

```diff
diff --git a/iridium-sniffer_amd/csrc/api.cpp b/iridium-sniffer_amd/csrc/api.cpp
--- a/iridium-sniffer_amd/csrc/api.cpp
+++ b/iridium-sniffer_amd/csrc/api.cpp
@@ -28,6 +28,11 @@
     if (!strcmp(key, "k1_lists")) { p->k1_lists = value; return 0; }
     if (!strcmp(key, "band_first")) { p->band_first = value < 0 ? 0 : value > kBandRounds ? kBandRounds : value; return 0; }
     if (!strcmp(key, "band_spec")) { p->band_spec_opt = value != 0; return 0; }
+    if (!strcmp(key, "spec_round1")) {
+        if (value && band_ws_b_alloc(p) != 0) return -1;
+        p->spec_round1_opt = value != 0;
+        return 0;
+    }
     if (!strcmp(key, "band_selfcheck")) { p->band_tune.selfcheck = value; return 0; }
     if (!strcmp(key, "rot_pool_rows")) {
         if (value < 1 || value > p->P.n) return -1;
@@ -91,6 +96,9 @@
     if (!strcmp(key, "ring_waits")) return (int64_t)p->stat_ring_waits;
     if (!strcmp(key, "spec_passes")) return (int64_t)p->stat_spec_passes;
     if (!strcmp(key, "spec_scans")) return (int64_t)p->stat_spec_scans;
+    if (!strcmp(key, "spec_round1_passes")) return (int64_t)p->stat_ahead_passes;
+    if (!strcmp(key, "spec_round1_used")) return (int64_t)p->stat_ahead_used;
+    if (!strcmp(key, "spec_round1_refused")) return (int64_t)p->stat_ahead_refused;
     if (!strcmp(key, "sum_restarts")) return (int64_t)p->stat_sum_restarts;
     if (!strcmp(key, "scratch_peak")) return (int64_t)p->stat_scratch_peak;
     if (!strcmp(key, "band_last_flags")) return (int64_t)p->last_band_flags;
diff --git a/iridium-sniffer_amd/csrc/band_core.hpp b/iridium-sniffer_amd/csrc/band_core.hpp
--- a/iridium-sniffer_amd/csrc/band_core.hpp
+++ b/iridium-sniffer_amd/csrc/band_core.hpp
@@ -28,6 +28,7 @@
     BAND_F_CHAIN = 2048,
     BAND_F_CHECK = 4096,
     BAND_F_COOP = 1024,
+    BAND_F_AHEAD = 8192,
 };
 
 struct BandParams {
@@ -47,6 +48,8 @@
     int32_t chained = 0;
     int32_t sum_restart = 1;
     int32_t spec_in = 0;
+    int32_t ahead_in = 0;
+    int32_t ahead_expect = 0;
 };
 
 struct BandRec {
diff --git a/iridium-sniffer_amd/csrc/create.cpp b/iridium-sniffer_amd/csrc/create.cpp
--- a/iridium-sniffer_amd/csrc/create.cpp
+++ b/iridium-sniffer_amd/csrc/create.cpp
@@ -14,7 +14,8 @@
                      p->d_fir_off, p->d_mag2, p->d_mag3, p->k1_pre[1], p->k1_pre[2], p->k1_counts[1], p->k1_counts[2], p->k1_entries[1], p->k1_entries[2],
                      p->k1_pre[0] != p->d_pre ? p->k1_pre[0] : nullptr, p->k1_counts[0] != p->d_counts ? p->k1_counts[0] : nullptr,
                      p->k1_entries[0] != p->d_entries ? p->k1_entries[0] : nullptr, p->d_counts, p->d_entries, p->d_goff, p->d_compact, p->d_pre, p->d_sum_bak, p->d_hist_bak, p->d_state_bak,
-                     p->d_status, p->d_mc_ops, p->d_mc_done, p->d_band, p->d_smin, p->d_kclk, p->d_state_spec };
+                     p->d_status, p->d_mc_ops, p->d_mc_done, p->d_band, p->d_smin, p->d_kclk, p->d_state_spec,
+                     p->d_band_b, p->d_smin_b };
     for (void *q : ptrs)
         if (q) (void)hipFree(q);
     for (int s = 0; s < 2; s++) {
@@ -87,6 +88,25 @@
 }
 
 extern "C" void irdm_destroy(irdm_pipeline_t *p) { pipeline_free(p); }
+
+int band_ws_b_alloc(irdm_pipeline *p)
+{
+    if (p->d_band_b) return 0;
+    if (!p->band_ok || !p->depth || !p->d_band) return -1;
+    if (hipMalloc(&p->d_band_b, band_work_bytes(p->P.n, p->max_chunk)) != hipSuccess) {
+        p->d_band_b = nullptr;
+        return -1;
+    }
+    band_work_carve(&p->band_ws[1], p->d_band_b, p->P.n, p->max_chunk, false, p->band.bar);
+    p->d_smin_b = dev_alloc<float>((size_t)p->P.n);
+    if (!p->d_smin_b) {
+        (void)hipFree(p->d_band_b);
+        p->d_band_b = nullptr;
+        return -1;
+    }
+    p->band_ws[1].smin = p->d_smin_b;
+    return 0;
+}
 
 
 bool chain_stream_create(irdm_pipeline *, hipStream_t *out, int prio)
@@ -367,6 +387,8 @@
         if (ok) ok = hipMalloc(&p->d_band, band_work_bytes(P.n, p->max_chunk)) == hipSuccess;
         if (ok) band_work_carve(&p->band, p->d_band, P.n, p->max_chunk);
         if (ok) ok = hipMemset(p->band.bar, 0, 256) == hipSuccess;
+        p->band.smin = p->d_smin;
+        p->band_ws[0] = p->band;
         if (ok && p->depth) {
             const size_t sb = band_work_bytes(P.n, p->max_chunk, true);
             ok = hipMalloc(&p->d_band_spec, sb) == hipSuccess;
@@ -375,6 +397,7 @@
                          hipMemset(p->band_spec.rec_count, 0, 4 * 64) == hipSuccess && hipMemset(p->band_spec.flags, 0, 256) == hipSuccess;
             AL(p->d_state_spec, DetState, 1);
             if (ok) ok = hipMemset(p->d_state_spec, 0, sizeof(DetState)) == hipSuccess;
+            if (ok && p->spec_round1_opt) ok = band_ws_b_alloc(p) == 0;
             ok = ok && hipStreamCreateWithPriority(&p->stream_spec, hipStreamNonBlocking, prio_hi) == hipSuccess &&
                  hipEventCreateWithFlags(&p->ev_sums1, hipEventDisableTiming) == hipSuccess &&
                  hipEventCreateWithFlags(&p->ev_spec_done, hipEventDisableTiming) == hipSuccess;
diff --git a/iridium-sniffer_amd/csrc/kernels.hpp b/iridium-sniffer_amd/csrc/kernels.hpp
--- a/iridium-sniffer_amd/csrc/kernels.hpp
+++ b/iridium-sniffer_amd/csrc/kernels.hpp
@@ -62,6 +62,7 @@
     uint32_t *rank;
     unsigned long long *tl;
     unsigned *bar;
+    float *smin;
 };
 struct BandTune {
     int selfcheck = 0;
@@ -71,7 +72,7 @@
 int band_list_cap(int n);
 int band_scan_supported(const DetParams &D, BandParams *out, int n_frames, uint64_t idx0);
 size_t band_work_bytes(int n, size_t max_chunk, bool spec = false);
-int band_work_carve(BandWork *W, void *base, int n, size_t max_chunk, bool spec = false);
+int band_work_carve(BandWork *W, void *base, int n, size_t max_chunk, bool spec = false, unsigned *shared_bar = nullptr);
 int launch_band_spec(const DetParams &D, BandWork S, DetState *st_spec, const float *sum_src, int n_frames, uint64_t idx0,
                      const unsigned *counts, const ListEntry *entries, int have_prev, hipStream_t stream, const BandTune &tune);
 int launch_band_scan(const DetParams &D, BandWork W, DetState *st, float *sum, float *hist, const float *mag,
@@ -80,7 +81,11 @@
                      uint32_t *hp_hdr, void *hp_ctl, int hp_cap, int chained, int tl_sel, hipStream_t stream,
                      const BandTune &tune, const uint32_t *gate_flag = nullptr, uint32_t gate_seq = 0, uint32_t *gate_err = nullptr,
                      const void *gate_src = nullptr, size_t gate_bytes = 0,
-                     const BandWork *spec = nullptr, hipEvent_t sums_done = nullptr);
+                     const BandWork *spec = nullptr, hipEvent_t sums_done = nullptr, int32_t ahead_expect = 0,
+                     int32_t *serial_out = nullptr);
+int launch_band_ahead(const DetParams &D, BandWork W, const BandWork &S, const BandWork &prev, const float *prev_mag, int prev_frames,
+                      const float *mag, const float *hist, int n_frames, uint64_t idx0, const unsigned *counts, const float *pre,
+                      hipStream_t stream, const BandTune &tune);
 constexpr int kBandTlSlots = 32;
 int launch_prefilter_lists(const float *sum, float thr, float *pre, const float *smin, const float *mag, int n,
                            unsigned *counts, ListEntry *entries, int n_frames, int cap, hipStream_t stream);
diff --git a/iridium-sniffer_amd/csrc/pipeline.hpp b/iridium-sniffer_amd/csrc/pipeline.hpp
--- a/iridium-sniffer_amd/csrc/pipeline.hpp
+++ b/iridium-sniffer_amd/csrc/pipeline.hpp
@@ -131,6 +131,19 @@
     uint64_t spec_for_no = ~0ull;
     int spec_frames = 0;
     uint64_t stat_spec_passes = 0, stat_spec_scans = 0, stat_sum_restarts = 0;
+    int spec_round1_opt = 1;
+    void *d_band_b = nullptr;
+    float *d_smin_b = nullptr;
+    BandWork band_ws[2] = {};
+    int last_ws = 0;
+    int fl_ws = 0, chain_ws = 0;
+    uint64_t sums1_no = ~0ull;
+    int sums1_ws = 0;
+    int32_t sums1_serial = 0;
+    uint64_t ahead_for_no = ~0ull;
+    int ahead_ws = 0;
+    int32_t ahead_expect = 0;
+    uint64_t stat_ahead_passes = 0, stat_ahead_used = 0, stat_ahead_refused = 0;
     uint32_t seq_counter = 0;
     uint32_t fl_seq = 0;
     uint32_t chain_seq = 0;
@@ -347,7 +360,9 @@
 int scan_restore(irdm_pipeline *p);
 int scan_band_enqueue_at(irdm_pipeline *p, const float *mag, int n_frames, int done, int retry, bool more_rounds,
                                 uint64_t c0, const irdm_pipeline::FeedSlot *feed, int sel, int first, int chained,
-                                uint32_t seq, uint64_t chunk_no, bool use_spec = false);
+                                uint32_t seq, uint64_t chunk_no, bool use_spec, int ws, bool use_ahead);
+int scan_ws_for(const irdm_pipeline *p, uint64_t no);
+int band_ws_b_alloc(irdm_pipeline *p);
 int scan_band_enqueue(irdm_pipeline *p, const float *mag, int n_frames, int done, int retry, bool more_rounds = false);
 int scan_legacy_enqueue(irdm_pipeline *p, const float *mag, int n_frames, int done, bool sparse);
 int scan_export(irdm_pipeline *p);
diff --git a/iridium-sniffer_amd/csrc/scan_band.hip b/iridium-sniffer_amd/csrc/scan_band.hip
--- a/iridium-sniffer_amd/csrc/scan_band.hip
+++ b/iridium-sniffer_amd/csrc/scan_band.hip
@@ -164,6 +164,18 @@
     s.pad = 0;
     return s;
 }
+__device__ __forceinline__ SumStep plan_step(const BandParams &P, const BandWork &W, int h0, int k, int uf_k, int slot,
+                                             int n_prev, const int32_t *prev_upd)
+{
+    if (k >= kHistory) return make_step(P, uf_k, W.upd_frame[k - kHistory], slot);
+    const int j = n_prev + k - kHistory;
+    if (prev_upd != nullptr && j >= 0) {
+        SumStep s = make_step(P, uf_k, prev_upd[j], slot);
+        s.pad = 1;
+        return s;
+    }
+    return make_step(P, uf_k, -(((h0 + k) % kHistory) + 1), slot);
+}
 __device__ __forceinline__ SumStep noop_step()
 {
     SumStep s;
@@ -176,7 +188,7 @@
 
 struct PlanShared {
     int32_t part[kPlanThreads / 64 + 1];
-    int mismatch, first, status, agree_fail;
+    int mismatch, first, status, agree_fail, n_prev;
     unsigned flags;
     int kstar;
 };
@@ -188,9 +200,12 @@
 template <int NT>
 __device__ void band_plan_body(const BandParams &P, const BandWork &W, const unsigned *__restrict__ counts,
                                DetState *__restrict__ st, int round, PlanShared &sh, uint8_t *lds,
-                               const uint64_t *u_busy = nullptr, const uint64_t *u_forced = nullptr)
+                               const uint64_t *u_busy = nullptr, const uint64_t *u_forced = nullptr,
+                               const BandCtl *prev_ctl = nullptr, const int32_t *prev_upd = nullptr)
 {
     const bool first = round == 0 || (P.spec_in && round == 1);
+    const bool ahead = first && round == 1 && prev_ctl != nullptr;
+    if (!ahead) prev_upd = nullptr;
     if (!(P.spec_in && round == 1) || u_busy == nullptr) {
         u_busy = W.busy;
         u_forced = W.forced;
@@ -201,7 +216,7 @@
     unsigned &s_flags = sh.flags;
     const int tid = threadIdx.x;
     BandCtl *ctl = W.ctl;
-    if (first) {
+    if (first && !ahead) {
         if (tid == 0) {
             const unsigned prev = W.bar[4];
             s_status = (P.chained && prev != 1u) ? 1 : 0;
@@ -218,11 +233,21 @@
         if (tid < (int)(sizeof(BandCtl) / 4)) reinterpret_cast<uint32_t *>(ctl)[tid] = 0;
         if (tid == 0) {
             *W.flags = 0;
-            st->n_gone = 0;
-        }
-        __syncthreads();
-        if (round != 0 && tid == 0) ctl->h0 = st->hist_idx;
-    }
+            if (!ahead) st->n_gone = 0;
+        }
+        __syncthreads();
+        if (round != 0 && tid == 0) {
+            if (ahead) {
+                const int h0p = prev_ctl->h0, np = prev_ctl->n_upd;
+                sh.n_prev = np;
+                ctl->h0 = ((h0p + np) % kHistory + kHistory) % kHistory;
+            } else {
+                ctl->h0 = st->hist_idx;
+            }
+        }
+        __syncthreads();
+    }
+    const int n_prev = ahead ? sh.n_prev : 0;
     if (ctl->status != 0) return;
     const int F = P.n_frames;
     const uint64_t t_begin = wall_clock64();
@@ -462,11 +487,7 @@
         stamp(5);
         const int h0 = ctl->h0;
         for (int k = n_upd + tid; k < n_upd + 2 * kSumDepth + 1; k += kPlanThreads) W.steps[k] = noop_step();
-        for (int k = tid; k < n_upd; k += kPlanThreads) {
-            const int uf_k = W.upd_frame[k];
-            const int old = k < kHistory ? -(((h0 + k) % kHistory) + 1) : W.upd_frame[k - kHistory];
-            W.steps[k] = make_step(P, uf_k, old, s_slot[k + 1]);
-        }
+        for (int k = tid; k < n_upd; k += kPlanThreads) W.steps[k] = plan_step(P, W, h0, k, W.upd_frame[k], s_slot[k + 1], n_prev, prev_upd);
         {
             int k = base;
 #pragma unroll
@@ -536,8 +557,7 @@
     for (int k = n_upd + tid; k < n_upd + 2 * kSumDepth + 1; k += kPlanThreads) W.steps[k] = noop_step();
     for (int k = tid; k < n_upd; k += kPlanThreads) {
         W.snap_after[k] = W.snap_slot[k + 1];
-        W.old_row[k] = k < kHistory ? -(((h0 + k) % kHistory) + 1) : W.upd_frame[k - kHistory];
-        W.steps[k] = make_step(P, W.upd_frame[k], W.old_row[k], W.snap_after[k]);
+        W.steps[k] = plan_step(P, W, h0, k, W.upd_frame[k], W.snap_after[k], n_prev, prev_upd);
     }
     for (int f = tid; f < F; f += kPlanThreads) {
         const int k = W.cnt_before[f];
@@ -564,14 +584,14 @@
                                                        DetState *__restrict__ st, int round, float *__restrict__ sum,
                                                        GoneBurst *__restrict__ gone, int gone_cap, const float *__restrict__ pre,
                                                        float *__restrict__ smin_out, const uint64_t *u_busy,
-                                                       const uint64_t *u_forced)
+                                                       const uint64_t *u_forced, const BandCtl *prev_ctl, const int32_t *prev_upd)
 {
     IRDM_DETECTOR_PRIO();
     TlScope tl(P, W, 4 * round);
     __shared__ PlanShared sh;
     extern __shared__ __attribute__((aligned(16))) unsigned char plan_lds[];
     static_assert(kPlanLdsBytes >= (size_t)kBandMaxTotal * 10, "the fused commit sorts in the plan pass's LDS");
-    band_plan_body<NT>(P, W, counts, st, round, sh, (P.selfcheck & 16) ? nullptr : plan_lds, u_busy, u_forced);
+    band_plan_body<NT>(P, W, counts, st, round, sh, (P.selfcheck & 16) ? nullptr : plan_lds, u_busy, u_forced, prev_ctl, prev_upd);
     if (round == 0 && pre != nullptr) {
         __syncthreads();
         if (!band_void(P, W) && W.ctl->status == 0) {
@@ -597,10 +617,12 @@
     return __builtin_amdgcn_make_buffer_rsrc(const_cast<void *>(p), 0, (int)(bytes > 0x7fffffffu ? 0x7fffffffu : bytes), 0x00020000);
 }
 
+template <bool kAhead = false>
 __device__ __forceinline__ void band_sum_body(const BandParams &P, const BandWork &W, const float *__restrict__ mag,
                                               const float *__restrict__ hist, const float *__restrict__ sum,
                                               const float *__restrict__ pre, float *__restrict__ smin_out,
-                                              const SumStep *steps, float *snap, int b)
+                                              const SumStep *steps, float *snap, int b,
+                                              const float *__restrict__ prev = nullptr, int prev_frames = 0)
 {
     const BandCtl *ctl = W.ctl;
     const int N = P.n;
@@ -618,6 +640,7 @@
     const __amdgpu_buffer_rsrc_t r_mag = band_rsrc(mag, (size_t)P.n_frames * row);
     const __amdgpu_buffer_rsrc_t r_hist = band_rsrc(hist, (size_t)kHistory * row);
     const __amdgpu_buffer_rsrc_t r_snap = band_rsrc(snap, (size_t)W.snap_cap * row);
+    const __amdgpu_buffer_rsrc_t r_prev = kAhead ? band_rsrc(prev, (size_t)prev_frames * row) : r_hist;
     const int boff = b * 4;
 
     static_assert(kHistory % kSumDepth == 0, "a batch of steps must not straddle the history ring's length");
@@ -632,8 +655,10 @@
         _Pragma("unroll") for (int j = 0; j < kSumDepth; j++) {                                         \
             const int o_nw = __builtin_amdgcn_readlane((int)D.x, (half) * kSumDepth + j);               \
             const int o_ol = __builtin_amdgcn_readlane((int)D.y, (half) * kSumDepth + j);               \
+            const __amdgpu_buffer_rsrc_t r_o = kAhead && (k0) < kHistory &&                              \
+                __builtin_amdgcn_readlane((int)D.w, (half) * kSumDepth + j) != 0 ? r_prev : r_old;      \
             NWv[j] = __builtin_bit_cast(float, __builtin_amdgcn_raw_buffer_load_b32(r_mag, boff, o_nw, 0)); \
-            OLv[j] = __builtin_bit_cast(float, __builtin_amdgcn_raw_buffer_load_b32(r_old, boff, o_ol, 0)); \
+            OLv[j] = __builtin_bit_cast(float, __builtin_amdgcn_raw_buffer_load_b32(r_o, boff, o_ol, 0));   \
         }                                                                                               \
     }
 #define IRDM_SUM_STEP(NWv, OLv, D, half)                                                                \
@@ -686,6 +711,17 @@
     band_sum_body(P, W, mag, hist, sum, pre, smin_out, steps, snap, (int)blockIdx.x * 64 + (int)threadIdx.x);
 }
 
+__global__ __launch_bounds__(64) void band_sum_ahead_kernel(BandParams P, BandWork W, const float *__restrict__ mag,
+                                                            const float *__restrict__ hist, const float *__restrict__ sum,
+                                                            const float *__restrict__ pre, float *__restrict__ smin_out,
+                                                            const SumStep *__restrict__ steps, float *__restrict__ snap,
+                                                            const float *__restrict__ prev, int prev_frames)
+{
+    IRDM_DETECTOR_PRIO();
+    if (W.ctl->status != 0) return;
+    band_sum_body<true>(P, W, mag, hist, sum, pre, smin_out, steps, snap, (int)blockIdx.x * 64 + (int)threadIdx.x, prev, prev_frames);
+}
+
 constexpr int kWalkWaveGroups = 256;
 
 template <int NW>
@@ -693,7 +729,9 @@
 {
     IRDM_DETECTOR_PRIO();
     TlScope tl(P, W, 4 * (W.ctl->rounds - 1) + 3);
-    if (band_void(P, W) || W.ctl->status != 0) return;
+    if (band_void(P, W)) return;
+    if (P.ahead_in && blockIdx.x == 0 && threadIdx.x == 0) W.bar[4] = 0;
+    if (W.ctl->status != 0) return;
     io.act_in = st->act;
     io.n_act_in = (int32_t)wv_first((uint32_t)st->n_act);
     const int lane = threadIdx.x & 63;
@@ -788,11 +826,27 @@
 constexpr int kCrossGroups = 256;
 
 __global__ __launch_bounds__(256) void band_cross_w_kernel(BandParams P, BandWork W, const unsigned *__restrict__ counts,
-                                                           const ListEntry *__restrict__ entries)
+                                                           const ListEntry *__restrict__ entries, DetState *__restrict__ st)
 {
     IRDM_DETECTOR_PRIO();
     TlScope tl(P, W, 4 * (W.ctl->rounds - 1) + 2);
     __shared__ uint32_t s_bits_all[4][16384 / 32];
+    if (P.ahead_in) {
+        const bool lead = blockIdx.x == 0 && threadIdx.x == 0;
+        if (__hip_atomic_load(W.bar + 4, __ATOMIC_RELAXED, __HIP_MEMORY_SCOPE_AGENT) != 1u) {
+            if (lead) __hip_atomic_store(W.bar + 5, (unsigned)P.serial, __ATOMIC_RELAXED, __HIP_MEMORY_SCOPE_AGENT);
+            return;
+        }
+        const bool same = W.bar[6] == (unsigned)P.ahead_expect && W.bar[7] <= 2u && st->hist_idx == W.ctl->h0;
+        if (lead) {
+            st->n_gone = 0;
+            if (!same) {
+                W.ctl->flags = BAND_F_AHEAD;
+                W.ctl->status = 2;
+            }
+        }
+        if (!same) return;
+    }
     if (band_void(P, W) || W.ctl->status != 0) return;
     const int lane = threadIdx.x & 63, wave = threadIdx.x >> 6;
     const int gw = (int)blockIdx.x * 4 + wave, n_waves = (int)gridDim.x * 4;
@@ -989,6 +1043,8 @@
         ctl->n_gone = n_gone;
         ctl->n_total = n;
         ctl->committed = 1;
+        W.bar[6] = (unsigned)P.serial;
+        W.bar[7] = (unsigned)ctl->rounds;
         W.bar[4] = 1;
     }
 }
@@ -1096,7 +1152,7 @@
     return b;
 }
 
-int band_work_carve(BandWork *W, void *base, int n, size_t max_chunk, bool spec)
+int band_work_carve(BandWork *W, void *base, int n, size_t max_chunk, bool spec, unsigned *shared_bar)
 {
     const size_t F = max_chunk / (size_t)n + 2;
     unsigned char *p = static_cast<unsigned char *>(base);
@@ -1131,6 +1187,8 @@
     W->bar = static_cast<unsigned *>(take(256));
     W->rank = static_cast<uint32_t *>(take(4 * kBandMaxTotal));
     W->tl = static_cast<unsigned long long *>(take(8 * 4 * kBandTlSlots));
+    if (shared_bar) W->bar = shared_bar;
+    W->smin = nullptr;
     return 0;
 }
 
@@ -1164,7 +1222,7 @@
     io.conc = S.conc;
     io.flags = S.flags;
     hipLaunchKernelGGL(band_spec_prep_kernel, dim3(1), dim3(256), 0, stream, P, S, counts, sum_src, st_spec, have_prev);
-    hipLaunchKernelGGL(band_cross_w_kernel, dim3(kCrossGroups), dim3(256), 0, stream, P, S, counts, entries);
+    hipLaunchKernelGGL(band_cross_w_kernel, dim3(kCrossGroups), dim3(256), 0, stream, P, S, counts, entries, st_spec);
     if (P.band_w == 128)
         hipLaunchKernelGGL((band_walk_wave_kernel<4>), dim3(kWalkWaveGroups), dim3(256), 0, stream, P, S, io, st_spec);
     else
@@ -1172,25 +1230,49 @@
     return hipGetLastError() == hipSuccess ? 0 : -1;
 }
 
+int launch_band_ahead(const DetParams &D, BandWork W, const BandWork &S, const BandWork &prev, const float *prev_mag, int prev_frames,
+                      const float *mag, const float *hist, int n_frames, uint64_t idx0, const unsigned *counts, const float *pre,
+                      hipStream_t stream, const BandTune &tune)
+{
+    BandParams P;
+    if (!band_scan_supported(D, &P, n_frames, idx0) || n_frames < 1 || prev_frames < 1) return -1;
+    P.serial = (int32_t)next_launch_serial();
+    P.spec_in = 1;
+    P.sum_restart = tune.sum_restart;
+    P.selfcheck = tune.selfcheck;
+    const size_t plan_lds = (P.selfcheck & 16) ? 0 : kPlanLdsBytes;
+    (void)hipFuncSetAttribute((const void *)band_plan_kernel<kPlanThreads>, hipFuncAttributeMaxDynamicSharedMemorySize, (int)kPlanLdsBytes);
+    hipLaunchKernelGGL(band_plan_kernel<kPlanThreads>, dim3(1), dim3(kPlanThreads), plan_lds, stream, P, W, counts,
+                       (DetState *)nullptr, 1, (float *)nullptr, (GoneBurst *)nullptr, 0, (const float *)nullptr, (float *)nullptr,
+                       (const uint64_t *)S.busy, (const uint64_t *)S.forced, (const BandCtl *)prev.ctl, (const int32_t *)prev.upd_frame);
+    hipLaunchKernelGGL(band_sum_ahead_kernel, dim3(P.n / 64), dim3(64), 0, stream, P, W, mag, hist, (const float *)prev.sum_new, pre,
+                       W.smin, (const SumStep *)W.steps, W.snap, prev_mag, prev_frames);
+    return hipGetLastError() == hipSuccess ? 0 : -1;
+}
+
 int launch_band_scan(const DetParams &D, BandWork W, DetState *st, float *sum, float *hist, const float *mag,
                      int n_frames, uint64_t idx0, const unsigned *counts, const ListEntry *entries, const float *pre,
                      float *smin, GoneBurst *gone, int gone_cap, int round_begin, int round_end, GoneBurst *hp_gone,
                      uint32_t *hp_hdr, void *hp_ctl, int hp_cap, int chained, int tl_sel, hipStream_t stream,
                      const BandTune &tune, const uint32_t *gate_flag, uint32_t gate_seq, uint32_t *gate_err, const void *gate_src,
-                     size_t gate_bytes, const BandWork *spec, hipEvent_t sums_done)
-{
-    if (spec && round_begin != 1) return -1;
+                     size_t gate_bytes, const BandWork *spec, hipEvent_t sums_done, int32_t ahead_expect, int32_t *serial_out)
+{
+    const bool ahead = ahead_expect != 0;
+    if ((spec || ahead) && round_begin != 1) return -1;
+    if (ahead && (spec || gate_flag)) return -1;
     const uint64_t *ub = spec ? spec->busy : nullptr, *uf = spec ? spec->forced : nullptr;
     bool sums_noted = sums_done == nullptr;
     BandParams P;
     if (!band_scan_supported(D, &P, n_frames, idx0) || n_frames < 1) return -1;
     P.serial = (int32_t)next_launch_serial();
+    if (serial_out) *serial_out = P.serial;
     P.chained = chained;
     P.spec_in = spec ? 1 : 0;
+    P.ahead_expect = ahead_expect;
     P.sum_restart = tune.sum_restart;
     P.selfcheck = tune.selfcheck;
     P.tl_sel = tune.timeline && tl_sel >= 0 && tl_sel < 2 ? tl_sel : -1;
-    if (P.tl_sel >= 0 && (round_begin == 0 || spec)) {
+    if (P.tl_sel >= 0 && (round_begin == 0 || spec || ahead)) {
         unsigned long long *half = W.tl + (size_t)P.tl_sel * 2 * kBandTlSlots;
         (void)hipMemsetAsync(half, 0xff, 8 * kBandTlSlots, stream);
         (void)hipMemsetAsync(half + kBandTlSlots, 0, 8 * kBandTlSlots, stream);
@@ -1217,24 +1299,26 @@
             const size_t plan_lds = (P.selfcheck & 16) ? 0 : kPlanLdsBytes;
             const float *pre0 = round == 0 ? pre : nullptr;
             hipLaunchKernelGGL(band_plan_kernel<kPlanThreads>, dim3(1), dim3(kPlanThreads), plan_lds, stream, P, W, counts, st, round, sum,
-                               gone, gone_cap, pre0, smin, ub, uf);
+                               gone, gone_cap, pre0, smin, ub, uf, (const BandCtl *)nullptr, (const int32_t *)nullptr);
         }
         if (round == round_end) break;
         if (gate_flag && round == (round_begin > 1 ? round_begin : 1)) {
             if (launch_wait_host_flag(gate_flag, gate_seq, gate_err, stream) != 0) return -1;
             if (hipMemcpyAsync(hist, gate_src, gate_bytes, hipMemcpyDeviceToDevice, stream) != hipSuccess) return -1;
         }
-        if (round >= 1)
+        if (round >= 1 && !(ahead && round == 1))
             hipLaunchKernelGGL(band_sum_kernel, dim3(P.n / 64), dim3(64), 0, stream, P, W, mag, hist, sum, pre, smin, W.steps, W.snap);
-        if (!sums_noted && round >= 1) {
+        if (!sums_noted && round >= 1 && !(ahead && round == 1)) {
             if (hipEventRecord(sums_done, stream) != hipSuccess) return -1;
             sums_noted = true;
         }
-        hipLaunchKernelGGL(band_cross_w_kernel, dim3(kCrossGroups), dim3(256), 0, stream, P, W, counts, entries);
+        BandParams Pr = P;
+        Pr.ahead_in = ahead && round == 1 ? 1 : 0;
+        hipLaunchKernelGGL(band_cross_w_kernel, dim3(kCrossGroups), dim3(256), 0, stream, Pr, W, counts, entries, st);
         if (P.band_w == 128)
-            hipLaunchKernelGGL((band_walk_wave_kernel<4>), dim3(kWalkWaveGroups), dim3(256), 0, stream, P, W, io, st);
+            hipLaunchKernelGGL((band_walk_wave_kernel<4>), dim3(kWalkWaveGroups), dim3(256), 0, stream, Pr, W, io, st);
         else
-            hipLaunchKernelGGL((band_walk_wave_kernel<8>), dim3(kWalkWaveGroups), dim3(256), 0, stream, P, W, io, st);
+            hipLaunchKernelGGL((band_walk_wave_kernel<8>), dim3(kWalkWaveGroups), dim3(256), 0, stream, Pr, W, io, st);
     }
     if (P.selfcheck & 16)
         hipLaunchKernelGGL(band_commit_kernel, dim3(1), dim3(kPlanThreads), commit_lds, stream, P, W, st, sum, gone, gone_cap);
diff --git a/iridium-sniffer_amd/csrc/scan_host.cpp b/iridium-sniffer_amd/csrc/scan_host.cpp
--- a/iridium-sniffer_amd/csrc/scan_host.cpp
+++ b/iridium-sniffer_amd/csrc/scan_host.cpp
@@ -68,12 +68,20 @@
     return 0;
 }
 
+int scan_ws_for(const irdm_pipeline *p, uint64_t no)
+{
+    return p->ahead_for_no == no ? p->ahead_ws : p->last_ws;
+}
+
 int scan_band_enqueue_at(irdm_pipeline *p, const float *mag, int n_frames, int done, int retry, bool more_rounds,
                                 uint64_t c0, const irdm_pipeline::FeedSlot *feed, int sel, int first, int chained,
-                                uint32_t seq, uint64_t chunk_no, bool use_spec)
-{
-    (void)seq; (void)chunk_no;
+                                uint32_t seq, uint64_t chunk_no, bool use_spec, int ws, bool use_ahead)
+{
+    (void)seq;
     const DetParams &P = p->P;
+    const BandWork &W = p->band_ws[ws];
+    if (p->ahead_for_no != ~0ull && ws == p->ahead_ws) IRDM_HIP_CHECK(hipStreamWaitEvent(p->stream, p->ev_spec_done, 0));
+    p->last_ws = ws;
     const float *mag_rest = mag + (size_t)done * P.n;
     const uint64_t idx0 = c0 + (uint64_t)done * (uint64_t)P.n;
     const bool from_k1 = feed && feed->lists && done == 0;
@@ -84,12 +92,12 @@
     int *pin = p->h_pin_set[sel];
     GoneBurst *hpg = p->hp_gone_set[sel];
     if (more_rounds) {
-        return launch_band_scan(P, p->band, p->d_state, p->d_sum, p->d_hist, mag_rest, n_frames - done, idx0, counts, entries, pre,
-                                p->d_smin, p->d_gone, p->gone_cap, first, kBandRounds, hpg,
+        return launch_band_scan(P, W, p->d_state, p->d_sum, p->d_hist, mag_rest, n_frames - done, idx0, counts, entries, pre,
+                                W.smin, p->d_gone, p->gone_cap, first, kBandRounds, hpg,
                                 reinterpret_cast<uint32_t *>(pin + 64), pin + 96, p->hp_gone_cap, 0, sel, p->stream, p->band_tune);
     }
     if (!from_k1 || retry) {
-        if (launch_prefilter_lists(p->d_sum, P.threshold, pre, retry ? p->d_smin : nullptr, mag_rest, P.n, counts,
+        if (launch_prefilter_lists(p->d_sum, P.threshold, pre, retry ? W.smin : nullptr, mag_rest, P.n, counts,
                                    entries, n_frames - done, band_list_cap(P.n), p->stream) != 0)
             return -1;
     } else {
@@ -101,14 +109,25 @@
         p->gate_armed = false;
         p->gate_open_pending = true;
     }
-    if (launch_band_scan(P, p->band, p->d_state, p->d_sum, p->d_hist, mag_rest, n_frames - done, idx0, counts,
-                         entries, pre, p->d_smin, p->d_gone, p->gone_cap, use_spec ? 1 : 0, first, hpg,
+    const bool ahead = use_spec && use_ahead;
+    int32_t serial = 0;
+    if (launch_band_scan(P, W, p->d_state, p->d_sum, p->d_hist, mag_rest, n_frames - done, idx0, counts,
+                         entries, pre, W.smin, p->d_gone, p->gone_cap, use_spec ? 1 : 0, first, hpg,
                          reinterpret_cast<uint32_t *>(pin + 64), pin + 96, p->hp_gone_cap, chained, sel, p->stream, p->band_tune,
                          gate ? p->hp_gate_dev : nullptr, p->gate_seq, gate ? p->hp_gate_dev + 1 : nullptr,
                          p->gate_src, sizeof(float) * (size_t)kHistory * P.n,
-                         use_spec ? &p->band_spec : nullptr, p->ev_sums1) != 0)
+                         use_spec && !ahead ? &p->band_spec : nullptr, ahead ? nullptr : p->ev_sums1,
+                         ahead ? p->ahead_expect : 0, &serial) != 0)
         return -1;
     if (use_spec) p->stat_spec_scans++;
+    if (ahead) {
+        p->stat_ahead_used++;
+        p->sums1_serial = p->sums1_no == chunk_no && p->sums1_ws == ws ? serial : 0;
+    } else {
+        p->sums1_no = chunk_no;
+        p->sums1_ws = ws;
+        p->sums1_serial = serial;
+    }
     IRDM_HIP_CHECK(hipEventRecord(p->ev_sk_set[sel][1], p->stream));
     return 0;
 }
@@ -117,7 +136,7 @@
 {
     if (!more_rounds && !retry) p->fl_band_first = p->band_first ? p->band_first : p->band_auto;
     return scan_band_enqueue_at(p, mag, n_frames, done, retry, more_rounds, p->fl_c0, p->fl_feed, p->out_sel, p->fl_band_first, 0,
-                                p->fl_seq, p->fl_no);
+                                p->fl_seq, p->fl_no, false, p->fl_ws, false);
 }
 
 int scan_legacy_enqueue(irdm_pipeline *p, const float *mag, int n_frames, int done, bool sparse)
@@ -158,7 +177,7 @@
 {
     const bool band = p->fl_mode == 2 && p->fl_band_ran;
     return launch_gone_export(p->d_state, p->d_gone, std::min(p->gone_cap, p->hp_gone_cap), p->hp_gone,
-                              reinterpret_cast<uint32_t *>(p->h_pin + 64), band ? p->band.ctl : nullptr, p->h_pin + 96,
+                              reinterpret_cast<uint32_t *>(p->h_pin + 64), band ? p->band_ws[p->fl_ws].ctl : nullptr, p->h_pin + 96,
                               (int)sizeof(BandCtl), p->stream);
 }
 
@@ -186,7 +205,11 @@
     const bool use_spec = p->band_spec_opt && p->d_band_spec && p->spec_for_no == no && p->chain_band_first >= 2 &&
                           f.frames == p->spec_frames && !p->gate_armed;
     if (use_spec) IRDM_HIP_CHECK(hipStreamWaitEvent(p->stream, p->ev_spec_done, 0));
-    if (scan_band_enqueue_at(p, f.mag, f.frames, 0, 0, false, f.c0, &f, sel, p->chain_band_first, 1, p->chain_seq, no, use_spec) != 0) return -1;
+    const bool use_ahead = use_spec && p->spec_round1_opt && p->ahead_for_no == no;
+    p->chain_ws = scan_ws_for(p, no);
+    if (scan_band_enqueue_at(p, f.mag, f.frames, 0, 0, false, f.c0, &f, sel, p->chain_band_first, 1, p->chain_seq, no, use_spec,
+                             p->chain_ws, use_ahead) != 0)
+        return -1;
     IRDM_HIP_CHECK(hipEventRecord(p->ev_end_set[sel], p->stream));
     p->chain_pending = true;
     p->chain_no = no;
@@ -202,9 +225,26 @@
     IRDM_HIP_CHECK(hipStreamWaitEvent(p->stream_spec, nx.ev_k1, 0));
     IRDM_HIP_CHECK(hipStreamWaitEvent(p->stream_spec, p->ev_sums1, 0));
     const int have_prev = p->spec_for_no != ~0ull && p->spec_for_no + 1 == no;
-    if (launch_band_spec(p->P, p->band_spec, p->d_state_spec, p->band.sum_new, nx.frames, nx.c0, p->k1_counts[ls], p->k1_entries[ls],
-                         have_prev, p->stream_spec, p->band_tune) != 0)
+    if (launch_band_spec(p->P, p->band_spec, p->d_state_spec, p->band_ws[p->sums1_ws].sum_new, nx.frames, nx.c0, p->k1_counts[ls],
+                         p->k1_entries[ls], have_prev, p->stream_spec, p->band_tune) != 0)
         return -1;
+    const bool ahead = p->spec_round1_opt && p->d_band_b && p->fl_active && p->fl_mode == 2 && p->fl_band_ran && p->fl_done == 0 &&
+                       p->fl_no + 1 == no && p->sums1_no == p->fl_no && p->sums1_ws == p->fl_ws && p->sums1_serial != 0 &&
+                       !p->gate_armed && !p->gate_open_pending;
+    if (ahead) {
+        const int ws = p->fl_ws ^ 1;
+        if (launch_band_ahead(p->P, p->band_ws[ws], p->band_spec, p->band_ws[p->fl_ws], p->fl_mag, p->fl_frames, nx.mag, p->d_hist,
+                              nx.frames, nx.c0, p->k1_counts[ls], p->k1_pre[ls], p->stream_spec, p->band_tune) != 0)
+            return -1;
+        IRDM_HIP_CHECK(hipEventRecord(p->ev_sums1, p->stream_spec));
+        p->ahead_for_no = no;
+        p->ahead_ws = ws;
+        p->ahead_expect = p->sums1_serial;
+        p->sums1_no = no;
+        p->sums1_ws = ws;
+        p->sums1_serial = 0;
+        p->stat_ahead_passes++;
+    }
     IRDM_HIP_CHECK(hipEventRecord(p->ev_spec_done, p->stream_spec));
     p->spec_for_no = no;
     p->spec_frames = nx.frames;
@@ -227,6 +267,7 @@
         p->fl_band_ran = true;
         p->fl_band_first = p->chain_band_first;
         p->fl_seq = p->chain_seq;
+        p->fl_ws = p->chain_ws;
         scan_select_outputs(p, p->chain_sel);
         p->fl_active = true;
         return 0;
@@ -240,6 +281,7 @@
     p->fl_c0 = p->total_samples;
     p->fl_no = p->chunk_no;
     p->fl_seq = next_scan_seq(p);
+    p->fl_ws = scan_ws_for(p, p->fl_no);
     int done = 0;
     if (!p->host_primed && p->fl_mode != 0) {
         done = std::min(n_frames, kHistory - p->host_hist_idx);
@@ -299,6 +341,13 @@
             IRDM_HIP_CHECK(hipStreamSynchronize(p->stream));
             return 0;
         };
+        if (ctl->status == 2 && ctl->flags == BAND_F_AHEAD && p->fl_band_ran) {
+            redone = true;
+            p->stat_ahead_refused++;
+            if (scan_band_enqueue(p, p->fl_mag, p->fl_frames, p->fl_done, 0) != 0) return -1;
+            if (scan_export(p) != 0) return -1;
+            IRDM_HIP_CHECK(hipStreamSynchronize(p->stream));
+        }
         if (more_rounds() != 0) return -1;
         while (ctl->status != 1 && ctl->flags == BAND_F_STALE && tries < 2) {
             tries++;
@@ -313,7 +362,7 @@
         p->stat_band_steps += (uint64_t)(ctl->n_upd > 0 ? ctl->n_upd : 0);
         if (p->band_tune.timeline && p->fl_band_ran) {
             unsigned long long tl[2 * kBandTlSlots];
-            IRDM_HIP_CHECK(hipMemcpy(tl, p->band.tl + (size_t)p->out_sel * 2 * kBandTlSlots, sizeof(tl), hipMemcpyDeviceToHost));
+            IRDM_HIP_CHECK(hipMemcpy(tl, p->band_ws[p->fl_ws].tl + (size_t)p->out_sel * 2 * kBandTlSlots, sizeof(tl), hipMemcpyDeviceToHost));
             for (int i = 26; i < 32; i++) p->stat_tl_dur[i] += tl[kBandTlSlots + i];
             unsigned long long prev_end = 0;
             for (int i = 0; i < 26; i++) {
```

Result: no change. 77330 (median of 6 runs) (+1.8%).
